# weiwei-ww/ML-VAE

Measured on AMD Instinct MI355X. Metric: spectrogram frames/sec + ELBO; 80-d log-mel B=256 at 1/2/4/8 MI355X, higher is better.
Workload: dtype bf16

## Files before the change

### include/mlvae.h

```cpp
#ifndef MLVAE_H
#define MLVAE_H
#include <stddef.h>
#ifdef __cplusplus
extern "C" {
#endif

const char* mlvae_last_error(void);
int mlvae_abi_version(void);
int mlvae_device_check(char* arch_out, int len);

size_t mlvae_gemm_workspace_size(int M, int N, int K);
int mlvae_gemm(int prec, int trans_a, int trans_b, int M, int N, int K, float alpha,
               const float* A, int lda, const float* B, int ldb, float beta, float* C, int ldc,
               const float* bias1, const float* bias2, int epi, const float* aux, int ldaux,
               int kshift_T, int kshift, float* ws, size_t ws_bytes, void* stream);

size_t mlvae_gemm_ex_workspace_size(int M, int N, int K);
int mlvae_gemm_ex(int trans_a, int trans_b, int M, int N, int K, float alpha, const void* A,
                  int a_bf16, int lda, const void* B, int b_bf16, int ldb, float beta, float* C,
                  int ldc, const float* bias1, const float* bias2, int epi, const float* aux,
                  int ldaux, int kshift_T, int kshift, float* ws, size_t ws_bytes, void* stream);
int mlvae_gemm_ex_drop(int trans_a, int trans_b, int M, int N, int K, float alpha,
                       const void* A, int a_bf16, int lda, const void* B, int b_bf16, int ldb,
                       float beta, float* C, int ldc, const float* bias1, const float* bias2,
                       int epi, const float* aux, int ldaux, int kshift_T, int kshift,
                       unsigned long long drop_seed, unsigned long long drop_offset, float drop_p,
                       float* ws, size_t ws_bytes, void* stream);
size_t mlvae_gemm_bf16_workspace_size(int M, int N, int K, int batch);
int mlvae_gemm_bf16_set_split_target(int workgroups);
int mlvae_gemm_bf16_set_variant(int var);
int mlvae_gemm_bf16(int trans_a, int trans_b, int M, int N, int K, int batch, const void* A,
                    int lda, long long a_bstride, const void* B, int ldb, long long b_bstride,
                    float* C, int ldc, long long c_bstride, float beta, const float* bias1,
                    const float* bias2, int epi, const float* aux, int ldaux, int kshift_T,
                    int kshift, int kshift_bstep, unsigned long long drop_seed,
                    unsigned long long drop_offset, float drop_p, float* ws, size_t ws_bytes,
                    void* stream);
int mlvae_cast_bf16(size_t n, const float* x, void* y, void* stream);
int mlvae_cast_bf16_t(int rows, int cols, const float* x, void* y, void* stream);

int mlvae_lstm_workspace_size(int B, int H, int prec, size_t* xbytes);
int mlvae_lstm_fwd(int prec, int B, int T, int H, const float* w_hh_fwd, const float* w_hh_rev,
                   float* gates, float* cells, float* y, void* xbuf, size_t xbytes, int* err,
                   void* stream);
int mlvae_lstm_bwd(int prec, int B, int T, int H, const float* w_hh_fwd, const float* w_hh_rev,
                   float* gates, const float* cells, const float* dy, void* xbuf, size_t xbytes,
                   int* err, void* stream);
int mlvae_lstm_fwd_ex(int prec, int B, int T, int H, const float* w_hh_fwd, const float* w_hh_rev,
                      float* gates, float* cells, float* y, void* y_bf16, void* xbuf,
                      size_t xbytes, int* err, void* stream);
int mlvae_lstm_bwd_ex(int prec, int B, int T, int H, const float* w_hh_fwd, const float* w_hh_rev,
                      float* gates, const float* cells, const float* dy, void* dg_bf16,
                      void* xbuf, size_t xbytes, int* err, void* stream);
int mlvae_lstm1_fwd(int prec, int B, int T, int H, const float* w_hh, float* gates, float* cells,
                    float* y, void* y_bf16, void* xbuf, size_t xbytes, int* err, void* stream);
int mlvae_lstm1_bwd(int prec, int B, int T, int H, const float* w_hh, float* gates,
                    const float* cells, const float* dy, void* dg_bf16, void* xbuf, size_t xbytes,
                    int* err, void* stream);
int mlvae_lstm_gates_fp16(int B, int H, int prec);
int mlvae_lstm_gates_fp16_t(int B, int T, int H, int prec);
int mlvae_lstm_fwd_ex2(int prec, int B, int T, int H, const float* w_hh_fwd, const float* w_hh_rev,
                       void* gates, int gates_fp16, float* cells, float* y, void* y_bf16,
                       void* y_drop_bf16, unsigned long long drop_seed,
                       unsigned long long drop_offset, float drop_p, void* xbuf, size_t xbytes,
                       int* err, void* stream);
int mlvae_lstm_bwd_ex2(int prec, int B, int T, int H, const float* w_hh_fwd, const float* w_hh_rev,
                       void* gates, int gates_fp16, const float* cells, const float* dy,
                       void* dg_bf16, float* dbias_rows, void* xbuf, size_t xbytes, int* err,
                       void* stream);
int mlvae_lstm_bwd_ex3(int prec, int B, int T, int H, const float* w_hh_fwd, const float* w_hh_rev,
                       void* gates, int gates_fp16, const float* cells, const void* dy, int dy_bf16,
                       void* dg_bf16, float* dbias_rows, void* xbuf, size_t xbytes, int* err,
                       void* stream);
int mlvae_lstm_fwd_fp8(int B, int T, int H, const float* w_hh_fwd, const float* w_hh_rev, void* gates,
                       float* cells, void* y_bf16, void* y_drop_bf16, void* y_drop_fp8, float x8_scale,
                       unsigned long long drop_seed, unsigned long long drop_offset, float drop_p,
                       void* xbuf, size_t xbytes, int* err, void* stream);
int mlvae_lstm_fwd_z(int B, int T, int H, const float* w_hh_fwd, const float* w_hh_rev, const void* z_bf16,
                     int ldz, int Z, const float* w_ih_fwd, const float* w_ih_rev, const float* b_ih_fwd,
                     const float* b_hh_fwd, const float* b_ih_rev, const float* b_hh_rev, void* gates,
                     float* cells, float* y, void* y_bf16, void* y_drop_bf16, void* y_drop_fp8, float x8_scale,
                     unsigned long long drop_seed, unsigned long long drop_offset, float drop_p, void* xbuf,
                     size_t xbytes, int* err, void* stream);
int mlvae_lstm_fwd_z2(int B, int T, int H, const float* w_hh_fwd, const float* w_hh_rev, const void* z_bf16,
                      int ldz, int Z, const float* w_ih_fwd, const float* w_ih_rev, const float* b_ih_fwd,
                      const float* b_hh_fwd, const float* b_ih_rev, const float* b_hh_rev, void* gates,
                      float* cells, float* y, void* y_bf16, int y_bf16_prev, void* y_drop_bf16, void* y_drop_fp8,
                      float x8_scale, unsigned long long drop_seed, unsigned long long drop_offset, float drop_p,
                      void* xbuf, size_t xbytes, int* err, void* stream);
int mlvae_lstm_bwd_fp8(int B, int T, int H, const float* w_hh_fwd, const float* w_hh_rev, void* gates,
                       const float* cells, const float* dy, void* dg_bf16, float* dbias_rows,
                       void* dg_fp8, const float* dg8_scale, unsigned* dg_amax, void* xbuf,
                       size_t xbytes, int* err, void* stream);
int mlvae_lstm_bwd_fp8_ex(int B, int T, int H, const float* w_hh_fwd, const float* w_hh_rev, void* gates,
                          const float* cells, const void* dy, int dy_bf16, void* dg_bf16,
                          float* dbias_rows, void* dg_fp8, const float* dg8_scale, unsigned* dg_amax,
                          void* xbuf, size_t xbytes, int* err, void* stream);
int mlvae_lstm_launch_workgroups(int B, int H, int prec, int fwd);
int mlvae_lstm_set_debug(void* buf);

int mlvae_phn_bce(int B, int T, int C, const float* logits, int ldl, const float* feat_lens,
                  const long long* phn, int L, const float* phn_lens, const float* boundary,
                  float* loss, const float* dloss, float* dlogits, int* err, void* stream);
int mlvae_boundary_fwd(size_t n, const float* za, const float* zb, const float* y, const float* u,
                       unsigned long long seed, unsigned long long offset, float* v, float* bce,
                       float* kld, void* stream);
int mlvae_boundary_bwd(size_t n, const float* za, const float* zb, const float* y, const float* u,
                       unsigned long long seed, unsigned long long offset, const float* dv,
                       const float* dbce, const float* dkld, float* dza, float* dzb, void* stream);

int mlvae_pi_sample(size_t n, const float* logits, const float* u, unsigned long long seed,
                    unsigned long long offset, int train, float* sampled_pi, void* stream);
int mlvae_pi_nll_fwd(size_t n, const float* logits, const int* labels, float* nll, int* err,
                     void* stream);
int mlvae_pi_nll_bwd(size_t n, const float* logits, const int* labels, const float* dnll,
                     float* dlogits, void* stream);

int mlvae_pi_sample_k(size_t n, int K, const float* logits, const float* u, unsigned long long seed,
                      unsigned long long offset, int train, float* sampled_pi, void* stream);
int mlvae_sfl_fwd(size_t n, int K, int F, int Z, const float* logits, const float* sampled_pi,
                  const float* recon, const float* kld, const float* pi_nll, const float* baseline,
                  float w_recon, float w_kld, float w_nll, float* reward, float* rif,
                  float* neg_entropy, float* baseline_loss, void* stream);
int mlvae_sfl_bwd(size_t n, int K, const float* logits, const float* sampled_pi, const float* reward,
// ... 73 lines not shown
                         float* partials, float* bias_ws, size_t bias_ws_bytes, float* db3m,
                         float* db3v, float* db2m, float* db2v, float* db1, int saved_bf16,
                         void* stream);
size_t mlvae_heads_wgrad_workspace_size(int B, int T, int F, int C);
int mlvae_heads_set_nt_mode(int mode);
int mlvae_heads_fused_ex2(int B, int T, int F, int C, int H2, int loss_type, int train,
                          const void* y_bf16, const void* w1_bf16, const void* w1t_bf16, const float* b1,
                          const float* w2m, const float* b2m, const float* w3m, const float* b3m,
                          const float* w2v, const float* b2v, const float* w3v, const float* b3v,
                          const float* x, const float* lens, const int* count, float rec_scale,
                          float* p1, float* p2m, float* p2v, float* mux, float* lvx, float* dmux,
                          float* dlvx, float* dp2m, float* dp2v, float* dp1, float* dy,
                          float* partials, float* bias_ws, size_t bias_ws_bytes, float* db3m,
                          float* db3v, float* db2m, float* db2v, float* db1, int saved_bf16,
                          float* wg_ws, size_t wg_ws_bytes, float* dw3m, float* dw3v, float* dw2m,
                          float* dw2v, void* stream);
int mlvae_heads_fused_ex3(int B, int T, int F, int C, int H2, int loss_type, int train,
                          const void* y_bf16, const void* w1_bf16, const void* w1t_bf16, const float* b1,
                          const float* w2m, const float* b2m, const float* w3m, const float* b3m,
                          const float* w2v, const float* b2v, const float* w3v, const float* b3v,
                          const float* x, const float* lens, const int* count, float rec_scale,
                          float* p1, float* p2m, float* p2v, float* mux, float* lvx, float* dmux,
                          float* dlvx, float* dp2m, float* dp2v, float* dp1, float* dy,
                          float* partials, float* bias_ws, size_t bias_ws_bytes, float* db3m,
                          float* db3v, float* db2m, float* db2v, float* db1, int saved_bf16,
                          float* wg_ws, size_t wg_ws_bytes, float* dw3m, float* dw3v, float* dw2m,
                          float* dw2v, const void* w1_split, void* stream);
int mlvae_bf16_split_rows(const float* src, int rows, int cols, int chunk, void* dst, void* stream);
int mlvae_skinny_proj(int M, int N, int K, const void* A, int lda, const void* B, int ldb,
                      const float* bias1, const float* bias2, float* C, int ldc, void* stream);
int mlvae_skinny_proj_ex(int M, int N, int K, const void* A, int lda, const void* B, int ldb,
                         const float* bias1, const float* bias2, void* C, int ldc, int c_fp16,
                         void* stream);
int mlvae_skinny_nt(int M, int N, int K, const void* A, int lda, const void* Bt, int ldb,
                    float* C, int ldc, void* stream);
size_t mlvae_skinny_tn_workspace_size(int M, int NB, int K);
int mlvae_skinny_tn(int M, int NB, int K, const void* A, int lda, const void* B, int ldb, int nw,
                    float* W, float* bias1, float* bias2, float* ws, size_t ws_bytes, void* stream);
int mlvae_skinny_nt_fp8(int M, int N, int K, const void* A8, int lda, const void* Bt, int ldb, float* C, int ldc,
                        const float* alpha, void* stream);
int mlvae_skinny_tn_fp8(int M, int NB, int K, const void* A8, int lda, const void* B, int ldb, int nw, float* W,
                        float* bias1, float* bias2, const float* alpha, float* ws, size_t ws_bytes, void* stream);
size_t mlvae_skinny_dzw_workspace_size(int M, int K8);
int mlvae_skinny_dzw(int M, int K8, const void* A, int lda, const void* Wt, int ldw, const void* zb, int ldz, int Z,
                     float* dZ, int lddz, float* W, float* bias1, float* bias2, float* ws, size_t ws_bytes,
                     void* stream);
int mlvae_encoder_supported(int F, int E, int Z);
int mlvae_encoder_partials_count(int B, int T);
size_t mlvae_encoder_workspace_size(int B, int T, int F, int E, int Z);
int mlvae_encoder_fwd(int B, int T, int F, int E, int Z, const float* x, const float* w0,
                      const float* b0, const float* w1, const float* b1, const float* wml,
                      const float* bml, const float* eps_in, unsigned long long seed,
                      unsigned long long offset, const float* lens, void* e1_bf16, void* e2_bf16,
                      float* ml, float* z, void* z_bf16, int z_ld, float* eps_out,
                      float* kl_partials, void* stream);
int mlvae_encoder_fwd_ex(int B, int T, int F, int E, int Z, const float* x, const float* w0,
                         const float* b0, const float* w1, const float* b1, const float* wml,
                         const float* bml, const float* eps_in, unsigned long long seed,
                         unsigned long long offset, const float* lens, void* e1_bf16, void* e2_bf16,
                         float* ml, float* z, void* z_bf16, int z_ld, float* eps_out,
                         float* kl_partials, int split, void* stream);
int mlvae_encoder_bwd(int B, int T, int F, int E, int Z, const float* dz, const float* ml,
                      const float* eps, const void* e1_bf16, const void* e2_bf16, const float* x,
                      const float* wml, const float* w1, const float* lens, const int* count,
                      float kl_scale, float* dwml, float* dbml, float* dw1, float* db1, float* dw0,
                      float* db0, float* ws, size_t ws_bytes, void* stream);
int mlvae_dp_scalars(int pack, float* hdr, float* loss3, int* err, void* stream);
int mlvae_elbo_finalize(const float* kl_partials, int nk, const float* rec_partials, int nr,
                        const float* lens, const int* count, int B, int T, int Z, int F,
                        float w_kl, float w_rec, float* out, void* stream);
int mlvae_count_frames(const float* lens, int B, int T, int* out, void* stream);
int mlvae_randn(size_t n, unsigned long long seed, unsigned long long offset, float* out,
                void* stream);
int mlvae_masked_mean(int B, int T, int C, const float* loss, const float* lens, int reduction,
                      float* out, void* stream);

int mlvae_norm_supported(int F);
int mlvae_norm_stats(int B, int T, int F, const float* x, const float* rel_lens, float* utt_stats,
                     float* sums, float eps, void* stream);
int mlvae_norm_update(int F, const float* sums, float* glob_mean, float* glob_std, int mode,
                      float w_old, float w_new, void* stream);
int mlvae_norm_apply(size_t rows, int F, const float* x, const float* glob_mean, const float* glob_std,
                     float* out, void* stream);

int mlvae_sumsq_partials_count(size_t n);
int mlvae_grad_sumsq(const float* grads, size_t n, double* partials, void* stream);
int mlvae_adam_step(float* params, float* exp_avg, float* exp_avg_sq, const float* grads,
                    size_t n, const double* partials, int nparts, const float* loss, int* step,
                    int* nonfinite, float lr, float beta1, float beta2, float eps,
                    float max_norm, float* norm_out, float* hyp_scratch, int advance,
                    void* stream);
int mlvae_adam_step_ex(float* params, float* exp_avg, float* exp_avg_sq, const float* grads,
                       size_t n, const double* partials, int nparts, const float* loss, int* step,
                       int* nonfinite, const int* err, int* err_skips, float lr, float beta1,
                       float beta2, float eps, float max_norm, float* norm_out, float* hyp_scratch,
                       int advance, void* stream);

int mlvae_clip_scale(float* grads, size_t n, const double* partials, int nparts, float max_norm,
                     float* norm_out, void* stream);

int mlvae_lrelu_bwd(size_t n, const float* dy, const float* y, float* dx, void* stream);
int mlvae_masked_mean_bwd(int B, int T, int C, const float* lens, int reduction, const float* g,
                          float* dloss, void* stream);

size_t mlvae_colsum_workspace_size(int N, int C);
int mlvae_colsum(int N, int C, const float* in, int ld, float* out, float* out2, float beta,
                 float* ws, size_t ws_bytes, void* stream);
int mlvae_colsum_ex(int N, int C, const void* in, int in_bf16, int ld, float* out, float* out2,
                    float beta, float* ws, size_t ws_bytes, void* stream);

int mlvae_dropout(size_t n, const float* x, float* y, const float* mask,
                  unsigned long long seed, float p, void* stream);
int mlvae_dropout_ex(size_t n, const float* x, float* y, void* y_bf16, const float* mask,
                     unsigned long long seed, unsigned long long offset, float p, void* stream);

int mlvae_gmm_latent_fwd(int rows, int N, int Z, const float* P, int ldp, const float* eps,
                         const float* expo, unsigned long long seed, unsigned long long offset,
                         float tau, float* z, float* kl, float* w, float* ysoft, void* stream);
int mlvae_gmm_latent_bwd(int rows, int N, int Z, const float* P, int ldp, const float* eps,
                         const float* ysoft, float tau, const float* dz, const float* dkl,
                         const float* dw, float* dP, int lddp, void* stream);
int mlvae_apply_weight_fwd(int rows, int N, int C, const float* x, int ldx, const float* w,
                           float* y, int ldy, void* stream);
int mlvae_apply_weight_bwd(int rows, int N, int C, const float* x, int ldx, const float* w,
                           const float* dy, int lddy, float* dx, int lddx, float* dw,
                           void* stream);

#ifdef __cplusplus
}
#endif
#endif
```

### ml-vae_amd/csrc/gemm_bf16.hip

```cpp
#include "common.h"

namespace {

constexpr int BM = 128, BN = 128, BK = 64, LDK = BK + 8;
constexpr int TILE_ELEMS = BM * LDK;
constexpr size_t LDS_BYTES = (size_t)2 * 2 * TILE_ELEMS * sizeof(short);

struct G2Args {
  int M, N, K;
  const void* A; int lda;
  const void* B; int ldb;
  float* C; int ldc;
  float alpha, beta;
  const float* bias1; const float* bias2;
  int epi;
  const float* aux; int ldaux;
  int kshiftT, kshift;
  int splits, kchunk;
  float* ws;
  unsigned long long dseed;
  unsigned long long doff;
  float dkeep, dscale;
};

// ... 317 lines not shown
  kc = (kc + BK - 1) / BK * BK;
  s = kc > 0 ? (K + kc - 1) / kc : 1;
  *splits = s < 1 ? 1 : s;
  *kchunk = kc > 0 ? kc : BK;
}

extern "C" size_t mlvae_gemm_ex_workspace_size(int M, int N, int K) {
  int s, kc;
  gemm2_plan(M, N, K, &s, &kc);
  return s > 1 ? (size_t)s * M * N * sizeof(float) : 0;
}

extern "C" int mlvae_gemm_ex_drop(int trans_a, int trans_b, int M, int N, int K, float alpha,
                                  const void* A, int a_bf16, int lda, const void* B, int b_bf16,
                                  int ldb, float beta, float* C, int ldc, const float* bias1,
                                  const float* bias2, int epi, const float* aux, int ldaux,
                                  int kshift_T, int kshift, unsigned long long drop_seed,
                                  unsigned long long drop_offset, float drop_p, float* ws,
                                  size_t ws_bytes, void* stream) {
  if (M < 0 || N < 0 || K < 0 || !C || (K > 0 && (!A || !B))) {
    mlvae_set_error("mlvae_gemm_ex: bad shape/ptr");
    return 1;
  }
  if (M == 0 || N == 0) return 0;
  if (epi == EPI_DLRELU && !aux) { mlvae_set_error("mlvae_gemm_ex: DLRELU needs aux"); return 1; }
  if (epi == EPI_DROPOUT && !(drop_p >= 0.f && drop_p < 1.f)) {
    mlvae_set_error("mlvae_gemm_ex: dropout p=%f out of range", drop_p);
    return 1;
  }
  if (epi < EPI_NONE || epi > EPI_DROPOUT) { mlvae_set_error("mlvae_gemm_ex: bad epilogue %d", epi); return 1; }
  if (kshift != 0 && (trans_b || kshift_T <= 0)) {
    mlvae_set_error("mlvae_gemm_ex: kshift needs trans_b = 0, T > 0");
    return 1;
  }
  const size_t ea = a_bf16 ? 2 : 4, eb = b_bf16 ? 2 : 4;
  const int va = (int)(16 / ea), vb = (int)(16 / eb);
  if (((uintptr_t)A % 16) || (lda % va) || ((uintptr_t)B % 16) || (ldb % vb)) {
    mlvae_set_error("mlvae_gemm_ex: operands need 16-byte aligned rows (lda %% %d, ldb %% %d)", va, vb);
    return 1;
  }
  G2Args g;
  g.M = M; g.N = N; g.K = K; g.A = A; g.lda = lda; g.B = B; g.ldb = ldb; g.C = C; g.ldc = ldc;
  g.alpha = alpha; g.beta = beta; g.bias1 = bias1; g.bias2 = bias2; g.epi = epi; g.aux = aux;
  g.ldaux = ldaux; g.kshiftT = kshift_T; g.kshift = kshift; g.ws = ws;
  g.dseed = drop_seed; g.doff = drop_offset; g.dkeep = 1.f - drop_p; g.dscale = 1.f / (1.f - drop_p);
  int s, kc;
  gemm2_plan(M, N, K, &s, &kc);
  if (s > 1 && (!ws || ws_bytes < (size_t)s * M * N * sizeof(float))) {
    s = 1;
    kc = ((K + BK - 1) / BK) * BK;
  }
  if (K == 0) { s = 1; kc = BK; }
  g.splits = s; g.kchunk = kc;
  hipStream_t st = (hipStream_t)stream;
  dim3 grid(((N + BN - 1) / BN) * ((M + BM - 1) / BM), 1, s);
  int rc;
  if (!trans_a && trans_b) rc = launch2<false, true>(g, grid, a_bf16, b_bf16, st);
  else if (!trans_a && !trans_b) rc = launch2<false, false>(g, grid, a_bf16, b_bf16, st);
  else if (trans_a && !trans_b) rc = launch2<true, false>(g, grid, a_bf16, b_bf16, st);
  else rc = launch2<true, true>(g, grid, a_bf16, b_bf16, st);
  if (rc) return rc;
  MLVAE_CHECK_LAUNCH();
  if (s > 1) {
    size_t MN = (size_t)M * N;
    int blocks = (int)((MN + 63) / 64);
    if (blocks > 4096) blocks = 4096;
    splitk_reduce2<<<blocks, 256, 0, st>>>(g);
    MLVAE_CHECK_LAUNCH();
  }
  return 0;
}

extern "C" int mlvae_gemm_ex(int trans_a, int trans_b, int M, int N, int K, float alpha,
                             const void* A, int a_bf16, int lda, const void* B, int b_bf16,
                             int ldb, float beta, float* C, int ldc, const float* bias1,
                             const float* bias2, int epi, const float* aux, int ldaux,
                             int kshift_T, int kshift, float* ws, size_t ws_bytes, void* stream) {
  if (epi == EPI_DROPOUT) { mlvae_set_error("mlvae_gemm_ex: dropout epilogue needs mlvae_gemm_ex_drop"); return 1; }
  return mlvae_gemm_ex_drop(trans_a, trans_b, M, N, K, alpha, A, a_bf16, lda, B, b_bf16, ldb, beta,
                            C, ldc, bias1, bias2, epi, aux, ldaux, kshift_T, kshift, 0ull, 0ull, 0.f, ws,
                            ws_bytes, stream);
}

__global__ __launch_bounds__(256) void cast_bf16_kernel(size_t n, const float* __restrict__ x,
                                                        unsigned short* __restrict__ y) {
  const size_t n4 = n / 4;
  for (size_t i = (size_t)blockIdx.x * 256 + threadIdx.x; i < n4; i += (size_t)gridDim.x * 256) {
    const f32x4 v = reinterpret_cast<const f32x4*>(x)[i];
    u32x2 o = {(unsigned)bf_bits(v[0]) | ((unsigned)bf_bits(v[1]) << 16),
               (unsigned)bf_bits(v[2]) | ((unsigned)bf_bits(v[3]) << 16)};
    reinterpret_cast<u32x2*>(y)[i] = o;
  }
  for (size_t i = n4 * 4 + (size_t)blockIdx.x * 256 + threadIdx.x; i < n; i += (size_t)gridDim.x * 256)
    y[i] = bf_bits(x[i]);
}

extern "C" int mlvae_cast_bf16(size_t n, const float* x, void* y, void* stream) {
  if (n == 0) return 0;
  if (!x || !y || ((uintptr_t)x % 16) || ((uintptr_t)y % 8)) {
    mlvae_set_error("mlvae_cast_bf16: needs 16-byte aligned x, 8-byte aligned y");
    return 1;
  }
  size_t blocks = (n / 4 + 255) / 256;
  if (blocks > 4096) blocks = 4096;
  if (blocks < 1) blocks = 1;
  cast_bf16_kernel<<<(unsigned)blocks, 256, 0, (hipStream_t)stream>>>(n, x,
                                                                       static_cast<unsigned short*>(y));
  MLVAE_CHECK_LAUNCH();
  return 0;
}

__global__ __launch_bounds__(256) void cast_bf16_t_kernel(int rows, int cols, const float* __restrict__ x,
                                                          unsigned short* __restrict__ y) {
  __shared__ float t[32][33];
  const int r0 = blockIdx.y * 32, c0 = blockIdx.x * 32;
  const int tx = threadIdx.x & 31, ty = threadIdx.x >> 5;
#pragma unroll
  for (int k = 0; k < 4; ++k) {
    const int r = r0 + ty + 8 * k, c = c0 + tx;
    t[ty + 8 * k][tx] = (r < rows && c < cols) ? x[(size_t)r * cols + c] : 0.f;
  }
  __syncthreads();
#pragma unroll
  for (int k = 0; k < 4; ++k) {
    const int c = c0 + ty + 8 * k, r = r0 + tx;
    if (c < cols && r < rows) y[(size_t)c * rows + r] = bf_bits(t[tx][ty + 8 * k]);
  }
}

extern "C" int mlvae_cast_bf16_t(int rows, int cols, const float* x, void* y, void* stream) {
  if (rows <= 0 || cols <= 0) return 0;
  if (!x || !y) { mlvae_set_error("mlvae_cast_bf16_t: null pointer"); return 1; }
  dim3 grid((cols + 31) / 32, (rows + 31) / 32);
  cast_bf16_t_kernel<<<grid, 256, 0, (hipStream_t)stream>>>(rows, cols, x, static_cast<unsigned short*>(y));
  MLVAE_CHECK_LAUNCH();
  return 0;
}
```

### ml-vae_amd/csrc/lstm.hip

```cpp
#include "common.h"
#include <stdlib.h>
#include <type_traits>

#include "lstm_common.h"

namespace {


template <int PREC, int HJ, int NL>
__global__ __launch_bounds__(320) void lstm_fwd_kernel(LstmArgs a) {
  typedef typename Elt<PREC>::T ET;
  constexpr int ROWS = 4 * HJ, MT = ROWS / 16;
  constexpr int KS = 4;
  constexpr int NRED = PREC == PREC_F32 ? 1 : 2;
  constexpr int KSTEP = PREC == PREC_F32 ? 16 : 32;
  constexpr int EPL = PREC == PREC_F32 ? 4 : 8;
  constexpr int GE = Elt<PREC>::GE;
  constexpr bool IOW = PREC == PREC_BF16 && HJ == 16;
  constexpr int GXS = 16 * 4 + 4, OUS = 16 * 8 + 4;
  extern __shared__ __attribute__((aligned(16))) char smem[];
  f32x4* red0 = reinterpret_cast<f32x4*>(smem);
  float* gxr = reinterpret_cast<float*>(smem + NRED * 4 * MT * 64 * 16);
  float* outr = gxr + 2 * 16 * GXS;
  __shared__ int abort_flag;
// ... 831 lines not shown
  return p;
}

int device_cus() {
  int dev = 0, cus = 256;
  if (hipGetDevice(&dev) != hipSuccess ||
      hipDeviceGetAttribute(&cus, hipDeviceAttributeMultiprocessorCount, dev) != hipSuccess)
    cus = 256;
  return cus;
}

int max_batch_per_launch(int H, bool fwd, int prec) {
  const int cus = device_cus();
  int hj = pick_hj(H, fwd, prec);
  int nj = hj ? H / hj : 1;
  int nb = cus / (2 * nj);
  return nb * BG;
}

template <int PREC, int HJ, int NL>
int launch_nl(bool fwd, const LstmArgs& a, const Plan& p, hipStream_t s) {
  dim3 grid(a.xcd_local ? 8 * a.NJ : a.ndir * a.NB * a.NJ);
  auto k = fwd ? lstm_fwd_kernel<PREC, HJ, NL> : lstm_bwd_kernel<PREC, HJ, NL>;
  const size_t lds = p.lds;
  if (hipFuncSetAttribute((const void*)k, hipFuncAttributeMaxDynamicSharedMemorySize, (int)lds) != hipSuccess) {
    mlvae_set_error("lstm: cannot reserve %zu B LDS", lds);
    return 2;
  }
  const int nthr = (fwd && PREC == PREC_BF16 && HJ == 16) ? 320 : 256;
  k<<<grid, nthr, lds, s>>>(a);
  MLVAE_CHECK_LAUNCH();
  return 0;
}

template <int PREC, int HJ>
int launch(bool fwd, const LstmArgs& a, const Plan& p, hipStream_t s) {
  constexpr int KSTEP = PREC == PREC_F32 ? 16 : 32;
  constexpr int KSF = 4;
  const int nl = fwd ? a.Kp / (KSF * KSTEP) : a.K4p / (4 * KSTEP);
  switch (nl) {
    case 1: return launch_nl<PREC, HJ, 1>(fwd, a, p, s);
    case 2: return launch_nl<PREC, HJ, 2>(fwd, a, p, s);
    case 4: return launch_nl<PREC, HJ, 4>(fwd, a, p, s);
    case 8: return launch_nl<PREC, HJ, 8>(fwd, a, p, s);
    case 16: return launch_nl<PREC, HJ, 16>(fwd, a, p, s);
    case 32: return launch_nl<PREC, HJ, 32>(fwd, a, p, s);
    default:
      mlvae_set_error("lstm: H=%d needs %d operand loads per wave (max 32)", a.H, nl);
      return 1;
  }
}

template <int NTW>
int launch_rs(const LstmArgs& a, const Plan& p, hipStream_t s) {
  dim3 grid(a.xcd_local ? 8 * a.NJ : a.ndir * a.NB * a.NJ);
  auto k = lstm_bwd_rs_kernel<NTW>;
  if (hipFuncSetAttribute((const void*)k, hipFuncAttributeMaxDynamicSharedMemorySize, (int)p.lds) != hipSuccess) {
    mlvae_set_error("lstm: cannot reserve %zu B LDS", p.lds);
    return 2;
  }
  k<<<grid, 256, p.lds, s>>>(a);
  MLVAE_CHECK_LAUNCH();
  return 0;
}

bool use_wide(int B, int H, int prec) {
  if (prec != PREC_BF16 || H <= 0 || H % 4) return false;
  const int bf = max_batch_per_launch(H, true, prec), bb = max_batch_per_launch(H, false, prec);
  (void)bf; (void)bb;
  if (g_dbg_mode & (1 << 20)) return false;
  return lstm_wide_workgroups(B, H, true) > 0 && lstm_wide_workgroups(B, H, false) > 0;
}

struct WideExtra {
  unsigned short* ydb = nullptr;
  float* dbias = nullptr;
  unsigned long long seed = 0, off = 0;
  float p = 0.f;
  WideFp8 f8;
  const unsigned short* dyb = nullptr;
  WideZ wz;
};

int run(bool fwd, int prec, int B, int T, int H, const float* W0, const float* W1, float* G,
        float* Cs, float* Y, void* xbuf, size_t xbytes, int* err, hipStream_t st,
        unsigned short* yb = nullptr, unsigned short* dgb = nullptr, int gates_fp16 = 0,
        const WideExtra& ex = WideExtra(), int ndir = 2) {
  if (B <= 0 || T <= 0) return 0;
  if (H <= 0 || H % 4 != 0) { mlvae_set_error("lstm: H=%d must be a positive multiple of 4", H); return 1; }
  if (prec != PREC_F32 && prec != PREC_BF16) { mlvae_set_error("lstm: bad prec %d", prec); return 1; }
  const bool wide = gates_fp16 != 0;
  if (ndir != 1 && ndir != 2) { mlvae_set_error("lstm: %d directions", ndir); return 1; }
  if (wide && ndir != 2) { mlvae_set_error("lstm: fp16 gates are bidirectional only"); return 1; }
  if (wide && !use_wide(B, H, prec)) {
    mlvae_set_error("lstm: B=%d H=%d prec=%d: fp16 gates only where mlvae_lstm_gates_fp16() = 1", B, H, prec);
    return 1;
  }
  if (wide) {
    if (!fwd && !dgb && !ex.f8.dg8) {
      mlvae_set_error("lstm: the wide-batch backward writes dG to dg_bf16 or (fp8 mode) dg_fp8 (both NULL)");
      return 1;
    }
    if (ex.ydb && !(ex.p >= 0.f && ex.p < 1.f)) { mlvae_set_error("lstm: dropout p=%g", ex.p); return 1; }
    return lstm_wide_run(fwd, B, T, H, W0, W1, G, Cs, Y, xbuf, xbytes, err, st, yb, dgb, ex.dbias, ex.ydb,
                         ex.seed, ex.off, ex.p, g_dbg, g_dbg_mode, ex.f8, ex.dyb, ex.wz);
  }
  if (ex.dyb) { mlvae_set_error("lstm: bf16 dY only on the wide-batch path (fp16 gates)"); return 1; }
  if (ex.ydb || ex.dbias || !Y) {
    mlvae_set_error("lstm: fused dropout / bias-gradient outputs, Y = NULL only on the wide-batch path");
    return 1;
  }
  if (!fwd && use_stepwise_bwd(H, prec)) return run_bwd_stepwise(B, T, H, ndir, W0, W1, G, Cs, Y, xbuf, xbytes, dgb, st);
  const int bmax = max_batch_per_launch(H, fwd, prec);
  if (bmax < BG) { mlvae_set_error("lstm: H=%d too large for one resident launch", H); return 1; }
  Plan full = make_plan(bmax < B ? bmax : B, H, prec, fwd);
  const size_t need_x = fwd ? full.xbytes_fwd : full.xbytes_bwd;
  if (!xbuf || xbytes < need_x || !err) {
    mlvae_set_error("lstm: exchange workspace too small (need %zu B)", need_x);
    return 1;
  }
  for (int b0 = 0; b0 < B; b0 += bmax) {
    const int bc = B - b0 < bmax ? B - b0 : bmax;
    Plan p = make_plan(bc, H, prec, fwd);
    LstmArgs a{};
    a.B = bc; a.T = T; a.H = H; a.NB = p.NB; a.NJ = p.NJ; a.HJ = p.HJ; a.Kp = p.Kp; a.K4p = p.K4p;
    a.W0 = W0; a.W1 = W1;
    const size_t gld = (size_t)4 * H * ndir, yld = (size_t)H * ndir;
    a.ndir = ndir;
    a.G = G + (size_t)b0 * T * gld;
    a.Cs = Cs + (size_t)b0 * T * yld;
    a.Y = Y + (size_t)b0 * T * yld;
    a.xbuf = xbuf; a.err = err; a.dbg = g_dbg; a.dbg_mode = g_dbg_mode;
    a.Yb = yb ? yb + (size_t)b0 * T * yld : nullptr;
    a.dGb = dgb ? dgb + (size_t)b0 * T * gld : nullptr;
    a.xcd_local = p.xcd && device_cus() == 256 && (fwd ? !(g_dbg_mode & 4) : (g_dbg_mode & 2));
    a.xtab = reinterpret_cast<unsigned*>(
        static_cast<char*>(xbuf) + (p.rs ? (size_t)2 * p.NB * NSLOT * p.NJ * p.NJ * 256 * sizeof(short)
                                         : (size_t)2 * p.NB * NSLOT * BG * p.Kp * (prec == PREC_F32 ? 4 : 2)));
    if (hipMemsetAsync(xbuf, 0, fwd ? p.xbytes_fwd : p.xbytes_bwd, st) != hipSuccess) {
      mlvae_set_error("lstm: memset failed");
      return 2;
    }
    int rc;
    if (p.rs) {
      rc = p.NJ == 8 ? launch_rs<2>(a, p, st) : p.NJ == 16 ? launch_rs<4>(a, p, st)
         : p.NJ == 32 ? launch_rs<8>(a, p, st) : launch_rs<16>(a, p, st);
    } else if (prec == PREC_F32) {
      rc = p.HJ == 16 ? launch<PREC_F32, 16>(fwd, a, p, st)
         : p.HJ == 8 ? launch<PREC_F32, 8>(fwd, a, p, st) : launch<PREC_F32, 4>(fwd, a, p, st);
    } else {
      rc = p.HJ == 32 ? launch<PREC_BF16, 32>(fwd, a, p, st)
         : p.HJ == 16 ? launch<PREC_BF16, 16>(fwd, a, p, st)
         : p.HJ == 8 ? launch<PREC_BF16, 8>(fwd, a, p, st) : launch<PREC_BF16, 4>(fwd, a, p, st);
    }
    if (rc) return rc;
  }
  return 0;
}

}

extern "C" int mlvae_lstm_workspace_size(int B, int H, int prec, size_t* xbytes) {
  if (H <= 0 || H % 4 != 0) { mlvae_set_error("lstm: H=%d must be a positive multiple of 4", H); return 1; }
  const int bf = max_batch_per_launch(H, true, prec), bb = max_batch_per_launch(H, false, prec);
  Plan pf = make_plan(bf < B ? bf : B, H, prec, true);
  Plan pb = make_plan(bb < B ? bb : B, H, prec, false);
  *xbytes = pf.xbytes_fwd > pb.xbytes_bwd ? pf.xbytes_fwd : pb.xbytes_bwd;
  if (use_stepwise_bwd(H, prec) && (size_t)2 * B * H * sizeof(float) > *xbytes)
    *xbytes = (size_t)2 * B * H * sizeof(float);
  if (prec == PREC_BF16) {
    const size_t wf = lstm_wide_xbytes(B, H, true), wb = lstm_wide_xbytes(B, H, false);
    if (wf > *xbytes) *xbytes = wf;
    if (wb > *xbytes) *xbytes = wb;
  }
  return 0;
}

extern "C" int mlvae_lstm_launch_workgroups(int B, int H, int prec, int fwd) {
  if (B <= 0 || H <= 0 || H % 4) return 0;
  const int bmax = max_batch_per_launch(H, fwd != 0, prec);
  if (use_wide(B, H, prec)) return lstm_wide_workgroups(B, H, fwd != 0);
  Plan p = make_plan(bmax < B ? bmax : B, H, prec, fwd != 0);
  return 2 * p.NB * p.NJ;
}

extern "C" int mlvae_lstm_gates_fp16(int B, int H, int prec) { return use_wide(B, H, prec) ? 1 : 0; }
extern "C" int mlvae_lstm_gates_fp16_t(int B, int T, int H, int prec) {
  return use_wide(B, H, prec) && lstm_wide_t_ok(T, H) ? 1 : 0;
}

extern "C" int mlvae_lstm_fwd_ex2(int prec, int B, int T, int H, const float* w_hh_fwd,
                                  const float* w_hh_rev, void* gates, int gates_fp16, float* cells,
                                  float* y, void* y_bf16, void* y_drop_bf16,
                                  unsigned long long drop_seed, unsigned long long drop_offset,
                                  float drop_p, void* xbuf, size_t xbytes, int* err, void* stream) {
  WideExtra ex;
  ex.ydb = static_cast<unsigned short*>(y_drop_bf16);
  ex.seed = drop_seed; ex.off = drop_offset; ex.p = drop_p;
  return run(true, prec, B, T, H, w_hh_fwd, w_hh_rev, static_cast<float*>(gates), cells, y, xbuf,
             xbytes, err, (hipStream_t)stream, static_cast<unsigned short*>(y_bf16), nullptr,
             gates_fp16, ex);
}

extern "C" int mlvae_lstm_fwd_fp8(int B, int T, int H, const float* w_hh_fwd, const float* w_hh_rev,
                                  void* gates, float* cells, void* y_bf16, void* y_drop_bf16,
                                  void* y_drop_fp8, float x8_scale, unsigned long long drop_seed,
                                  unsigned long long drop_offset, float drop_p, void* xbuf,
                                  size_t xbytes, int* err, void* stream) {
  if (!use_wide(B, H, PREC_BF16) || !y_drop_fp8 || !(x8_scale > 0.f)) {
    mlvae_set_error("lstm_fwd_fp8: wide-batch shapes with an e4m3 dropout output and a positive scale only");
    return 1;
  }
  WideExtra ex;
  ex.ydb = static_cast<unsigned short*>(y_drop_bf16);
  ex.seed = drop_seed; ex.off = drop_offset; ex.p = drop_p;
  ex.f8.y8 = static_cast<unsigned char*>(y_drop_fp8);
  ex.f8.x8scale = x8_scale;
  return run(true, PREC_BF16, B, T, H, w_hh_fwd, w_hh_rev, static_cast<float*>(gates), cells, nullptr,
             xbuf, xbytes, err, (hipStream_t)stream, static_cast<unsigned short*>(y_bf16), nullptr, 1, ex);
}
extern "C" int mlvae_lstm_fwd_z2(int B, int T, int H, const float* w_hh_fwd, const float* w_hh_rev,
                                 const void* z_bf16, int ldz, int Z, const float* w_ih_fwd,
                                 const float* w_ih_rev, const float* b_ih_fwd, const float* b_hh_fwd,
                                 const float* b_ih_rev, const float* b_hh_rev, void* gates, float* cells,
                                 float* y, void* y_bf16, int y_bf16_prev, void* y_drop_bf16, void* y_drop_fp8,
                                 float x8_scale, unsigned long long drop_seed, unsigned long long drop_offset,
                                 float drop_p, void* xbuf, size_t xbytes, int* err, void* stream) {
  if (Z != 32 || !z_bf16 || !use_wide(B, H, PREC_BF16) || (y_drop_fp8 && !(x8_scale > 0.f))) {
    mlvae_set_error("lstm_fwd_z: Z = 32 on wide-batch shapes; an e4m3 dropout output needs a scale");
    return 1;
  }
  WideExtra ex;
  ex.ydb = static_cast<unsigned short*>(y_drop_bf16);
  ex.seed = drop_seed; ex.off = drop_offset; ex.p = drop_p;
  ex.f8.y8 = static_cast<unsigned char*>(y_drop_fp8);
  ex.f8.x8scale = x8_scale;
  ex.wz.zb = static_cast<const unsigned short*>(z_bf16);
  ex.wz.ldz = ldz;
  ex.wz.w0 = w_ih_fwd; ex.wz.w1 = w_ih_rev;
  ex.wz.b[0] = b_ih_fwd; ex.wz.b[1] = b_hh_fwd; ex.wz.b[2] = b_ih_rev; ex.wz.b[3] = b_hh_rev;
  ex.wz.yb_prev = y_bf16 && y_bf16_prev ? 1 : 0;
  return run(true, PREC_BF16, B, T, H, w_hh_fwd, w_hh_rev, static_cast<float*>(gates), cells, y, xbuf, xbytes,
             err, (hipStream_t)stream, static_cast<unsigned short*>(y_bf16), nullptr, 1, ex);
}
// ... 126 lines not shown
```

### ml-vae_amd/csrc/lstm_common.h

```cpp
#pragma once
#include "common.h"
#include <type_traits>

#ifndef MLVAE_DIAG
#define MLVAE_DIAG 0
#endif
#define DMODE(a) (MLVAE_DIAG ? (a).dbg_mode : 0)
#define DPTR(a) (MLVAE_DIAG ? (a).dbg : (unsigned long long*)nullptr)

namespace {

constexpr int BG = 16;
constexpr int NSLOT = 4;
constexpr unsigned SPIN_LIMIT = 1u << 20;
constexpr int MIN_LDS = 82 * 1024;

struct LstmArgs {
  int B, T, H;
  int NB, NJ, HJ;
  int ndir;
  int Kp;
  int K4p;
  const float* W0;
  const float* W1;
  float* G;
  float* Cs;
  float* Y;
  void* xbuf;
  int* err;
  unsigned long long* dbg;
  int dbg_mode;
  int xcd_local;
  unsigned* xtab;
  unsigned short* Yb;
  unsigned short* dGb;
  float* dbias;
  unsigned short* Ydb;
  unsigned long long dseed, doff;
  float dkeep, dscale;
  unsigned char* Y8;
  float x8scale;
  unsigned char* dG8;
  const float* g8scale;
  unsigned* g8amax;
  const unsigned short* dYb;
  const unsigned short* Zb;
  int ldz;
  const float* Wz0;
  const float* Wz1;
  const float* bz[4];
  int yb_prev;
};

__device__ __forceinline__ unsigned xcc_id() {
  return __builtin_amdgcn_s_getreg((3 << 11) | (0 << 6) | 20) & 0xf;
}

__device__ bool group_on_one_xcd(unsigned* tab, int members, int me, int* scratch) {
  const int tid = threadIdx.x;
  const unsigned mine = xcc_id() + 1;
  if (tid == 0) { *scratch = 0; st_flag(tab + me, mine); }
  __syncthreads();
  if (tid < members) {
    unsigned v = 0, spins = 0;
    while ((v = ld_flag(tab + tid)) == 0 && ++spins < (1u << 16)) __builtin_amdgcn_s_sleep(2);
    if (v != mine) atomicOr(scratch, 1);
  }
  __syncthreads();
  return *scratch == 0;
}

#define STAMP(ph)                                                              \
  do {                                                                         \
    if (DPTR(a) && blockIdx.x == 0 && threadIdx.x == 0)                          \
      a.dbg[(size_t)s * 16 + (ph)] = __builtin_amdgcn_s_memtime();             \
  } while (0)
#define WSTAMP(slot)                                                           \
  do {                                                                         \
    if (DPTR(a) && blockIdx.x == 0 && (threadIdx.x & 63) == 0)                   \
      a.dbg[(size_t)s * 16 + (slot) + (threadIdx.x >> 6)] = __builtin_amdgcn_s_memtime(); \
  } while (0)

#define IOSTAMP(k)                                                             \
  do {                                                                         \
    if (DBG && DPTR(a) && (DMODE(a) & 16) && blockIdx.x == 0 && threadIdx.x == 256 && \
        (unsigned)(s - STW0) < (unsigned)STWN)                                 \
      stamp_lds[(s - STW0) * 16 + 8 + (k)] = __builtin_amdgcn_s_memtime();     \
  } while (0)
constexpr int STW0 = 64, STWN = 32;
#define LSTAMP_DECL                                                            \
  __shared__ unsigned long long stamp_lds[DBG ? STWN * 16 : 1];                \
  if (DBG && DPTR(a) && blockIdx.x == 0 && threadIdx.x == 0)                     \
    for (int i_ = 0; i_ < STWN * 16; ++i_) stamp_lds[i_] = 0
#define LSTAMP(ph)                                                             \
  do {                                                                         \
    if (DBG && DPTR(a) && blockIdx.x == 0 && threadIdx.x == 0 &&                        \
        (unsigned)(s - STW0) < (unsigned)STWN)                                 \
      stamp_lds[(s - STW0) * 16 + (ph)] = __builtin_amdgcn_s_memtime();        \
  } while (0)
#define LWSTAMP()                                                              \
  do {                                                                         \
    if (DBG && DPTR(a) && !(DMODE(a) & 16) && blockIdx.x == 0 && (threadIdx.x & 63) == 0 && \
        (unsigned)(s - STW0) < (unsigned)STWN)                                 \
      stamp_lds[(s - STW0) * 16 + 8 + (threadIdx.x >> 6)] = __builtin_amdgcn_s_memtime(); \
  } while (0)
#define LSTAMP_FLUSH()                                                         \
  do {                                                                         \
    if (DBG) __syncthreads();                                                  \
    if (DBG && DPTR(a) && blockIdx.x == 0 && threadIdx.x == 0)                   \
      for (int i_ = 0; i_ < STWN * 16; ++i_)                                   \
        a.dbg[(size_t)STW0 * 16 + i_] = stamp_lds[i_];                         \
  } while (0)

#define RTS_DECL                                                               \
  __shared__ unsigned long long rts_lds[DBG ? STWN * 16 : 1];                  \
  const bool rts_on = DBG && DPTR(a) && (DMODE(a) & 8);                        \
  if (rts_on)                                                                  \
    for (int i_ = threadIdx.x; i_ < STWN * 16; i_ += blockDim.x) rts_lds[i_] = 0
#define RTS(slot)                                                              \
  do {                                                                         \
    if (rts_on && (threadIdx.x & 63) == 0 && (unsigned)(s - STW0) < (unsigned)STWN) \
      rts_lds[(s - STW0) * 16 + (slot)] = __builtin_amdgcn_s_memrealtime();    \
  } while (0)
#define RTS_FLUSH()                                                            \
  do {                                                                         \
    if (DBG) __syncthreads();                                                  \
    if (rts_on)                                                                \
      for (int i_ = threadIdx.x; i_ < STWN * 16; i_ += blockDim.x)             \
        a.dbg[(size_t)a.T * 16 + (size_t)blockIdx.x * STWN * 16 + i_] = rts_lds[i_]; \
  } while (0)

__device__ __forceinline__ void stagger_start(int gid, int mode) {
  if (!(mode & (1 << 29)) || !((gid ^ (gid >> 3)) & 1)) return;
  for (int i = 0; i < ((mode >> 5) & 7); ++i) __builtin_amdgcn_s_sleep(16);
}

template <int PREC> struct Elt;
template <> struct Elt<PREC_F32> { typedef float T; static constexpr int GE = 2; };
template <> struct Elt<PREC_BF16> { typedef short T; static constexpr int GE = 4; };

__device__ __forceinline__ unsigned step_tag(int s) { return (unsigned)(((s >> 2) + 1) & 1); }
__device__ __forceinline__ unsigned step_tag_lg(int s, int lg) { return (unsigned)(((s >> lg) + 1) & 1); }

__device__ __forceinline__ unsigned long long pack_bf16(float v0, float v1, float v2, float v3,
                                                        unsigned tag) {
  const unsigned e0 = ((unsigned)(unsigned short)f2bf(v0) & ~1u) | tag;
  const unsigned lo = e0 | ((unsigned)(unsigned short)f2bf(v1) << 16);
  const unsigned hi = (unsigned)(unsigned short)f2bf(v2) | ((unsigned)(unsigned short)f2bf(v3) << 16);
  return ((unsigned long long)hi << 32) | lo;
}
__device__ __forceinline__ unsigned long long pack_f32(float v0, float v1, unsigned tag) {
  const unsigned e0 = (__float_as_uint(v0) & ~1u) | tag;
  return ((unsigned long long)__float_as_uint(v1) << 32) | e0;
}
__device__ __forceinline__ void st_granule(__amdgpu_buffer_rsrc_t r, unsigned byte_off,
                                           unsigned long long v) {
  u32x2 w = {(unsigned)v, (unsigned)(v >> 32)};
  __builtin_amdgcn_raw_buffer_store_b64(w, r, byte_off, 0, 16 );
}
__device__ __forceinline__ bool tags_ok(u32x4 v, unsigned tag, bool g0, bool g1) {
  return (!g0 || (v[0] & 1u) == tag) && (!g1 || (v[2] & 1u) == tag);
}

}

struct WideFp8 {
  unsigned char* y8 = nullptr;
  float x8scale = 0.f;
  unsigned char* dg8 = nullptr;
  const float* g8scale = nullptr;
  unsigned* g8amax = nullptr;
};
struct WideZ {
  const unsigned short* zb = nullptr;
  int ldz = 0;
  const float* w0 = nullptr;
  const float* w1 = nullptr;
  const float* b[4] = {nullptr, nullptr, nullptr, nullptr};
  int yb_prev = 0;
};
int lstm_wide_run(bool fwd, int B, int T, int H, const float* W0, const float* W1, float* G,
                  float* Cs, float* Y, void* xbuf, size_t xbytes, int* err, hipStream_t st,
                  unsigned short* yb, unsigned short* dgb, float* dbias, unsigned short* ydb,
                  unsigned long long dseed, unsigned long long doff, float dp,
                  unsigned long long* dbg, int dbg_mode, const WideFp8& f8 = WideFp8(),
                  const unsigned short* dyb = nullptr, const WideZ& wz = WideZ());
size_t lstm_wide_xbytes(int B, int H, bool fwd);
bool lstm_wide_t_ok(int T, int H);
int lstm_wide_workgroups(int B, int H, bool fwd);
```

### ml-vae_amd/csrc/lstm_wide.hip

```cpp
#include "lstm_common.h"
#include <stdlib.h>
#include <type_traits>

namespace {

constexpr int WW = 8;
constexpr int FWD_KLF = 4;
template <int TPW> constexpr int bptt_groups() { return 2; }
#ifndef NT_AUX
#define NT_AUX 2
#endif

__device__ __forceinline__ void publish(__amdgpu_buffer_rsrc_t r, unsigned byte_off,
                                        unsigned long long v, bool plain) {
  if (plain) {
    u32x2 w = {(unsigned)v, (unsigned)(v >> 32)};
    __builtin_amdgcn_raw_buffer_store_b64(w, r, byte_off, 0, 0);
  } else {
    st_granule(r, byte_off, v);
  }
}

__device__ __forceinline__ int swz(int utt, int slot) { return slot ^ (utt & 15); }

template <int TPW, int NKC, int OCC, bool DBG = false, bool AS = false, bool ZP = false, int NT = 1,
          bool W12 = false>
__global__ __launch_bounds__(W12 ? 768 : 512, W12 ? 1 : OCC) void lstm_fwd_wide_kernel(LstmArgs a) {
  static_assert(NT == 1 || (NT == 2 && AS && TPW == 1), "two N-tiles: the asymmetric TPW-1 split");
  static_assert(!W12 || (AS && TPW == 1), "12 waves: the asymmetric TPW-1 split");
  constexpr int NWV = W12 ? 12 : 8;
  constexpr int NPOLL = W12 ? 8 : 4;
  constexpr int IO0 = NWV - 4;
  constexpr int BGW = BG * NT;
  constexpr int HJ = WW * TPW * 4;
  constexpr int H = NKC * 32;
  constexpr int PL = NKC / NPOLL;
  constexpr int ROWB = H * 2;
  constexpr int HIMG = BGW * ROWB;
  constexpr int GXU = 4 * HJ + 8;
  constexpr int OUB = 4 * HJ * 2 + 2 * HJ * 4 + 16;
  constexpr int NC8 = BGW * HJ / 8;
  constexpr int KLF = ((TPW == 1 && !AS) || W12) ? 0 : FWD_KLF;
  constexpr int KR = NKC - KLF;
  constexpr int HB = 4;
  constexpr int NQ = 16 * 4 * HJ / 4;
  constexpr int QPT = NQ / 256;
  static_assert(NQ % 256 == 0, "io split");
  extern __shared__ __attribute__((aligned(16))) char smem[];
  LSTAMP_DECL;
  RTS_DECL;
  char* himg = smem;
  unsigned short* gxr = reinterpret_cast<unsigned short*>(smem + 2 * HIMG);
  char* outr = reinterpret_cast<char*>(gxr + 2 * BGW * GXU);
  bf16x8* wlds = reinterpret_cast<bf16x8*>(outr + 2 * BGW * OUB);
  unsigned* dbl = reinterpret_cast<unsigned*>(wlds + 8 * TPW * KLF * 64);
  __shared__ int abort_flag;

  const int ngroups = 2 * a.NB, gstride = (ngroups + 7) & ~7;
  const int gid = blockIdx.x % gstride, js = blockIdx.x / gstride;
  if (gid >= ngroups) return;
  const int dir = gid / a.NB, grp = gid % a.NB;
  const int T = a.T, j0 = js * HJ;
  const int tid = threadIdx.x, lane = tid & 63;
  const int nlg = (DMODE(a) & (1 << 24)) ? 2 : 1, nmask = (1 << nlg) - 1;
  const int wave = __builtin_amdgcn_readfirstlane(tid >> 6);
  const float* W = dir ? a.W1 : a.W0;
  const int bi = lane & 15, q = lane >> 4;
  bool valid[NT];
#pragma unroll
  for (int n = 0; n < NT; ++n) valid[n] = grp * BGW + 16 * n + bi < a.B;

  static_assert(!AS || TPW == 1, "asymmetric split: TPW 1 only");
  constexpr int TPP = W12 ? 1 : AS ? 2 : TPW;
  constexpr int TPI = AS ? 0 : TPW;
  static_assert(NPOLL * TPP + 4 * TPI == WW * TPW, "every tile owned once");
  auto load_w = [&](auto* wreg, int m0, int mt) {
    for (int t = 0; t < mt; ++t) {
      const int m = m0 + t;
      const float* wrow = W + (size_t)((bi & 3) * H + j0 + 4 * m + (bi >> 2)) * H;
#pragma unroll
      for (int kc = 0; kc < NKC; ++kc) {
        const f32x4 w0 = *reinterpret_cast<const f32x4*>(wrow + kc * 32 + 8 * q);
        const f32x4 w1 = *reinterpret_cast<const f32x4*>(wrow + kc * 32 + 8 * q + 4);
        bf16x8 v;
#pragma unroll
        for (int e = 0; e < 4; ++e) { v[e] = f2bf(w0[e]); v[4 + e] = f2bf(w1[e]); }
        if (kc < KR) wreg[t][kc < KR ? kc : 0] = v;
        else wlds[(m * KLF + (kc - KR)) * 64 + lane] = v;
      }
    }
  };
  __shared__ int placement;
  const bool same_xcd = group_on_one_xcd(a.xtab + gid * a.NJ, a.NJ, js, &placement) &&
                        !(DMODE(a) & 32768);
  if (tid == 0) abort_flag = 0;

  const size_t xslot = (size_t)BGW * H;
  short* xb = reinterpret_cast<short*>(a.xbuf) + (size_t)(dir * a.NB + grp) * NSLOT * xslot;
  auto xr = make_rsrc(xb, (unsigned)(NSLOT * xslot * sizeof(short)));

  const int iot = tid - 64 * IO0;
  const bool io = wave >= IO0;
  const int iow = wave - IO0;
  typedef __attribute__((address_space(3))) void* lds_ptr_t;
  unsigned short* G16 = reinterpret_cast<unsigned short*>(a.G);
  const auto rgx = make_rsrc(G16 + (size_t)grp * BGW * T * 8 * H, 0xffffffffu);
  const bool tmaj = (DMODE(a) & 1024) != 0;
  auto rowof = [&](int b_, int t_) -> size_t { return tmaj ? (size_t)t_ * a.B + b_ : (size_t)b_ * T + t_; };
  const auto rgx_abs = make_rsrc(G16, (unsigned)min((size_t)a.B * T * 8 * H * 2, (size_t)0xffffffffu));
  unsigned short* zr = gxr;
  const auto rz = make_rsrc(a.Zb, (unsigned)min((size_t)a.B * T * a.ldz * 2, (size_t)0x7fffffff));
  auto io_load = [&](int s_) {
    if (s_ >= T || (s_ > 0 && (DMODE(a) & 8192))) return;
    const int t_ = dir ? T - 1 - s_ : s_;
    if constexpr (ZP) {
      if (iow < NT) {
        const int u = iow * 16 + (lane >> 2), b = grp * BGW + u;
        const unsigned off = b < a.B ? (unsigned)((((size_t)b * T + t_) * a.ldz + 8 * (lane & 3)) * 2) : 0x80000000u;
        __builtin_amdgcn_raw_ptr_buffer_load_lds(rz, (lds_ptr_t)(zr + ((s_ & 1) * BGW + iow * 16) * 32), 16,
                                                 off, 0, 0, NT_AUX);
      }
      return;
    }
    constexpr int UPW = BGW / 4;
#pragma unroll
    for (int i = 0; i < UPW; ++i) {
      const int u = iow * UPW + i, b = grp * BGW + u;
      if (b >= a.B) continue;
      const int g = lane / (HJ / 8), uu = (lane % (HJ / 8)) * 8;
      const unsigned off = tmaj ? (unsigned)((((size_t)t_ * a.B + b) * 8 * H + dir * 4 * H + g * H + j0 + uu) * 2)
                                : (unsigned)((((size_t)u * T + t_) * 8 * H + dir * 4 * H + g * H + j0 + uu) * 2);
      const auto rs = tmaj ? rgx_abs : rgx;
      unsigned short* dst = gxr + (s_ & 1) * BGW * GXU + u * GXU;
      if (lane < HJ / 2) __builtin_amdgcn_raw_ptr_buffer_load_lds(rs, (lds_ptr_t)dst, 16, off, 0, 0, NT_AUX);
    }
  };
  auto drop_bits = [&](int s_, int c8) -> unsigned {
    const int u = c8 / (HJ / 8), uu = (c8 % (HJ / 8)) * 8;
    const int t_ = dir ? T - 1 - s_ : s_;
    const size_t o = ((size_t)(grp * BGW + u) * T + t_) * 2 * H + dir * H + j0 + uu;
// ... 303 lines not shown
              for (int t = 0; t < MT; ++t) {
                const int u0 = j0 + 4 * (m0 + t);
                publish(xr, ((unsigned)((s & nmask) * xslot) + ((u0 >> 3) * BGW + 16 * n + bi) * 8 + (u0 & 7)) * sizeof(short),
                        gr[t][n], same_xcd);
              }
          }
        } else if (q == 0) {
          const int u0 = j0 + 4 * TPW * wave;
          const unsigned cell = (unsigned)((s & nmask) * xslot) + ((u0 >> 3) * 16 + bi) * 8 + (u0 & 7);
          if constexpr (TPW == 2) {
            const u32x4 v = {(unsigned)gr[0][0], (unsigned)(gr[0][0] >> 32), (unsigned)gr[1][0], (unsigned)(gr[1][0] >> 32)};
            if (same_xcd) __builtin_amdgcn_raw_buffer_store_b128(v, xr, cell * sizeof(short), 0, 0);
            else st_sc1_b128(xr, cell * sizeof(short), v);
          } else {
            publish(xr, cell * sizeof(short), gr[0][0], same_xcd);
          }
        }
      }
      LSTAMP(4);
      RTS(wave);
      IOSTAMP(5);
      if (!IO && (DMODE(a) & (1 << 23))) {
        asm volatile("s_waitcnt vmcnt(0)" ::: "memory");
        LSTAMP(5);
      }
      if (IO && !PURE_IO && late_dma_s) io_load(s + 1);
      if (IO && !PURE_IO && s > 0) io_store(s - 1);
      IOSTAMP(6);
#pragma unroll
      for (int n = 0; n < NT; ++n) {
        char* ob = outr + ((s & 1) * BGW + 16 * n + bi) * OUB;
        unsigned short* og = reinterpret_cast<unsigned short*>(ob);
        float* of = reinterpret_cast<float*>(ob + 8 * HJ);
#pragma unroll
        for (int t = 0; t < MT; ++t) {
          const int u = 4 * (m0 + t) + q;
          og[u] = f2h(gates[t][n][0]); og[HJ + u] = f2h(gates[t][n][1]);
          og[2 * HJ + u] = f2h(gates[t][n][2]); og[3 * HJ + u] = f2h(gates[t][n][3]);
          of[u] = c[t][n]; of[HJ + u] = hvals[t][n];
        }
      }
      LSTAMP(6);
      if (!IO && want_drop && tid < NC8 && (!late_bits || s + 1 == T)) dbl[(s & 1) * NC8 + tid] = drop_bits(s, tid);
      LSTAMP(7);
    }
    __syncthreads();
    if (IO) io_store(T - 1);
  };
  if (io) run(std::true_type{});
  else run(std::false_type{});
  LSTAMP_FLUSH();
  RTS_FLUSH();
}

template <int TPW, int NKC, int OCC, bool F8 = false, bool DYB = false, bool DBG = false>
__global__ __launch_bounds__(512, OCC) void lstm_bwd_wide_kernel(LstmArgs a) {
  constexpr int HJ = 32 * TPW;
  constexpr int H = NKC * 32;
  constexpr int NJ = H / HJ;
  constexpr int NTW = NKC / 4;
  constexpr int KC = 4 * HJ / 32;
  constexpr int KLB = TPW == 1 ? 0 : KC / 4;
  constexpr int KR = KC - KLB;
  constexpr int BKB = TPW == 1 ? 4 : 1;
  constexpr int ROWB = 4 * HJ * 2;
  constexpr int AIMG = 16 * ROWB;
  constexpr int NPL = NJ / 8;
  constexpr int CPG = 2 * HJ / 64;
  static_assert(NPL >= 1 && CPG >= 1 && NPL * CPG == 2, "two 16-byte partial loads per lane");
  extern __shared__ __attribute__((aligned(16))) char smem[];
  LSTAMP_DECL;
  RTS_DECL;
  char* aimg = smem;
  bf16x8* wlds = reinterpret_cast<bf16x8*>(smem + 2 * AIMG);
  constexpr int CG_B = 4 * HJ * 2 + 16;
  constexpr int CF_B = HJ * 4 + 32;
  constexpr int CD_B = DYB ? HJ * 2 + 32 : CF_B;
  static_assert(((CG_B + CF_B + CD_B) / 4) % 8 == 4 || ((CG_B + CF_B + CD_B) / 4) % 64 == 20,
                "conflict-free staged rows");
  constexpr int CUTT = CG_B + CF_B + CD_B;
  char* cst = smem + 2 * AIMG + (size_t)8 * NTW * KLB * 64 * 16;
  __shared__ int abort_flag;

  const int ngroups = 2 * a.NB, gstride = (ngroups + 7) & ~7;
  const int gid = blockIdx.x % gstride, js = blockIdx.x / gstride;
  if (gid >= ngroups) return;
  const int dir = gid / a.NB, grp = gid % a.NB;
  const int T = a.T, j0 = js * HJ;
  const int tid = threadIdx.x, lane = tid & 63;
  const int nlg = (DMODE(a) & (1 << 24)) ? 2 : 1, nmask = (1 << nlg) - 1;
  const int wave = __builtin_amdgcn_readfirstlane(tid >> 6);
  const float* W = dir ? a.W1 : a.W0;
  const int bi = lane & 15, q = lane >> 4;

  bf16x8 wreg[NTW][KR];
  static_assert(KLB > 0 || KR == KC, "");
#pragma unroll
  for (int nt = 0; nt < NTW; ++nt) {
    const int n = (wave * NTW + nt) * 16 + bi;
#pragma unroll
    for (int kc = 0; kc < KC; ++kc) {
      bf16x8 v;
#pragma unroll
      for (int e = 0; e < 8; ++e) {
        const int k = kc * 32 + 8 * q + e;
        v[e] = f2bf(W[(size_t)((k / HJ) * H + j0 + (k % HJ)) * H + n]);
      }
      if (kc < KR) wreg[nt][kc < KR ? kc : 0] = v;
      else wlds[((wave * NTW + nt) * KLB + (kc - KR)) * 64 + lane] = v;
    }
  }
  __shared__ int placement;
  const bool same_xcd = group_on_one_xcd(a.xtab + gid * NJ, NJ, js, &placement) &&
                        !(DMODE(a) & 32768);
  if (tid == 0) abort_flag = 0;
  if (DBG && DPTR(a) && (DMODE(a) & 8) && tid == 0) a.dbg[blockIdx.x] = same_xcd ? 1 : 2;
  __syncthreads();

  const size_t xslot = (size_t)NJ * NJ * HJ * 16;
  short* xb = reinterpret_cast<short*>(a.xbuf) + (size_t)(dir * a.NB + grp) * NSLOT * xslot;
  auto xr = make_rsrc(xb, (unsigned)(NSLOT * xslot * sizeof(short)));

  auto rs_perm = [](int g) { return g ^ ((g & 4) ? 3 : 0); };
  const int arow = rs_perm(js / NPL);
  const int gq = tid >> 3, pg = lane & 7;
  int uc[CPG], cu[CPG];
  bool bv[CPG];
#pragma unroll
  for (int ci = 0; ci < CPG; ++ci) {
    const int cb = gq * CPG + ci;
    uc[ci] = cb >> 1;
    cu[ci] = (cb & 1) * 8 + rs_perm(pg);
    bv[ci] = grp * BG + cu[ci] < a.B;
  }
  constexpr int NGC = 16 * 4 * HJ / 8, NFC = 16 * HJ / 4, NDC = DYB ? 16 * HJ / 8 : NFC;
  constexpr int NCH = NGC + NFC + NDC;
  constexpr int CPT = (NCH + 511) / 512;
  static_assert(DYB || NCH % 512 == 0, "whole chunks per thread");
  static_assert(NGC % 64 == 0 && NFC % 64 == 0 && NDC % 64 == 0, "chunk kinds change at whole waves");
  const size_t gbase = (size_t)grp * BG * T;
  const auto rG = make_rsrc(reinterpret_cast<const unsigned short*>(a.G) + gbase * 8 * H, 0xffffffffu);
  const auto rC = make_rsrc(a.Cs + gbase * 2 * H, 0xffffffffu);
  const auto rY = DYB ? make_rsrc(a.dYb + gbase * 2 * H, 0xffffffffu) : make_rsrc(a.Y + gbase * 2 * H, 0xffffffffu);
  u32x4 creg[CPT];
  auto chunk_lds = [&](int c) -> int {
    if (c < NGC) {
      const int u = c / (4 * HJ / 8), k = c % (4 * HJ / 8);
      return u * CUTT + k * 16;
    }
    const int f = c - NGC;
    if (f < NFC) {
      const int u = f / (HJ / 4), k = f % (HJ / 4);
      return u * CUTT + CG_B + k * 16;
    }
    const int r = f - NFC, upr = DYB ? HJ / 8 : HJ / 4;
    return (r / upr) * CUTT + CG_B + CF_B + (r % upr) * 16;
  };
  const int ulast = a.B - 1 - grp * BG;
  auto load_cell = [&](int s_) {
    const int sc = s_ < T ? s_ : T - 1;
    const int t_ = dir ? sc : T - 1 - sc;
    const int tp_ = dir ? t_ + 1 : t_ - 1;
    const int tpc = tp_ < 0 ? 0 : (tp_ >= T ? T - 1 : tp_);
#pragma unroll
    for (int i = 0; i < CPT; ++i) {
      const int cw0 = wave * 64 + 512 * i;
// ... 340 lines not shown
    if (2 * nb2 * (H / 32) <= cus) {
      p.nt = 2; p.tpw = 1; p.HJ = 32; p.NJ = H / 32; p.NB = nb2; p.ok = true;
    }
  }
  if (!p.ok)
  for (int tpw = 1; tpw <= 2; ++tpw) {
    if (fwd && tpw * p.nkc * 4 > 128) break;
    p.NB = (B + BG - 1) / BG;
    const int hj = 32 * tpw, nj = H / hj;
    if (!fwd && (nj < 8 || nj % 8)) continue;
    if (2 * p.NB * nj <= cus) {
      p.tpw = tpw; p.HJ = hj; p.NJ = nj; p.ok = true;
      break;
    }
  }
  if (!p.ok) return p;
  if (fwd && p.tpw == 1) p.w12 = !(mode & 2048);
  p.lds = wide_lds(H, p.HJ, fwd, p.nt);
  if (fwd) p.xbytes = (size_t)2 * p.NB * NSLOT * BG * p.nt * H * 2;
  else p.xbytes = (size_t)2 * p.NB * NSLOT * p.NJ * p.NJ * p.HJ * 16 * 2;
  if (p.lds < (size_t)MIN_LDS) p.lds = MIN_LDS;
  p.xtab_off = p.xbytes;
  p.xbytes += (size_t)2 * p.NB * p.NJ * sizeof(unsigned);
  return p;
}

template <int TPW, int NKC, int OCC>
int launch_wide(bool fwd, const LstmArgs& a, const WidePlan& p, hipStream_t s) {
  const bool dbg = a.dbg != nullptr;
  constexpr bool AS1 = TPW == 1;
  const bool zp = a.Zb != nullptr;
  auto k = (fwd && p.w12)
               ? (p.nt == 2 ? (dbg ? lstm_fwd_wide_kernel<1, NKC, OCC, true, true, false, 2, true>
                                   : zp ? lstm_fwd_wide_kernel<1, NKC, OCC, false, true, true, 2, true>
                                        : lstm_fwd_wide_kernel<1, NKC, OCC, false, true, false, 2, true>)
                            : (dbg ? lstm_fwd_wide_kernel<1, NKC, OCC, true, true, false, 1, true>
                                   : zp ? lstm_fwd_wide_kernel<1, NKC, OCC, false, true, true, 1, true>
                                        : lstm_fwd_wide_kernel<1, NKC, OCC, false, true, false, 1, true>))
         : (fwd && p.nt == 2)
               ? (dbg ? lstm_fwd_wide_kernel<1, NKC, OCC, true, true, false, 2>
                      : zp ? lstm_fwd_wide_kernel<1, NKC, OCC, false, true, true, 2>
                           : lstm_fwd_wide_kernel<1, NKC, OCC, false, true, false, 2>)
         : fwd ? (dbg ? lstm_fwd_wide_kernel<TPW, NKC, OCC, true, AS1>
                      : zp ? lstm_fwd_wide_kernel<TPW, NKC, OCC, false, AS1, true>
                           : lstm_fwd_wide_kernel<TPW, NKC, OCC, false, AS1>)
               : (a.g8amax ? (a.dYb ? lstm_bwd_wide_kernel<TPW, NKC, OCC, true, true>
                                    : lstm_bwd_wide_kernel<TPW, NKC, OCC, true, false>)
                           : (a.dYb ? (dbg ? lstm_bwd_wide_kernel<TPW, NKC, OCC, false, true, true>
                                           : lstm_bwd_wide_kernel<TPW, NKC, OCC, false, true>)
                                    : (dbg ? lstm_bwd_wide_kernel<TPW, NKC, OCC, false, false, true>
                                           : lstm_bwd_wide_kernel<TPW, NKC, OCC, false>)));
  if (hipFuncSetAttribute((const void*)k, hipFuncAttributeMaxDynamicSharedMemorySize, (int)p.lds) != hipSuccess) {
    mlvae_set_error("lstm_wide: cannot reserve %zu B LDS", p.lds);
    return 2;
  }
  k<<<dim3(((2 * p.NB + 7) & ~7) * p.NJ), (fwd && p.w12) ? 768 : 512, p.lds, s>>>(a);
  MLVAE_CHECK_LAUNCH();
  return 0;
}

}

bool lstm_wide_t_ok(int T, int H) {
  return (size_t)2 * BG * T * 8 * H * 2 <= 0xffffffffull && (size_t)2 * BG * T * 2 * H * 4 <= 0xffffffffull;
}

int lstm_wide_workgroups(int B, int H, bool fwd) {
  WidePlan p = wide_plan(B, H, fwd);
  if (!p.ok) return 0;
  return 2 * p.NB * p.NJ;
}

size_t lstm_wide_xbytes(int B, int H, bool fwd) {
  WidePlan p = wide_plan(B, H, fwd), q = wide_plan(B, H, fwd, 512);
  if (!p.ok) return 0;
  return p.xbytes > q.xbytes ? p.xbytes : q.xbytes;
}

int lstm_wide_run(bool fwd, int B, int T, int H, const float* W0, const float* W1, float* G,
                  float* Cs, float* Y, void* xbuf, size_t xbytes, int* err, hipStream_t st,
                  unsigned short* yb, unsigned short* dgb, float* dbias, unsigned short* ydb,
                  unsigned long long dseed, unsigned long long doff, float dp,
                  unsigned long long* dbg, int dbg_mode, const WideFp8& f8, const unsigned short* dyb,
                  const WideZ& wz) {
  WidePlan p = wide_plan(B, H, fwd, dbg_mode);
  if (!p.ok) return -1;
  if (!lstm_wide_t_ok(T, H)) {
    mlvae_set_error("lstm_wide: T=%d too long for the wide kernels' 32-bit batch-group addressing at H=%d "
                    "(mlvae_lstm_gates_fp16_t(B, T, H, prec) = 0: pass fp32 gates)", T, H);
    return 1;
  }
  if (!xbuf || xbytes < p.xbytes || !err) {
    mlvae_set_error("lstm_wide: exchange workspace too small (need %zu B)", p.xbytes);
    return 1;
  }
  LstmArgs a{};
  a.ndir = 2;
  a.B = B; a.T = T; a.H = H; a.NB = p.NB; a.NJ = p.NJ; a.HJ = p.HJ; a.Kp = H; a.K4p = 4 * H;
  a.W0 = W0; a.W1 = W1; a.G = G; a.Cs = Cs; a.Y = Y; a.xbuf = xbuf; a.err = err;
  a.dbg = dbg; a.dbg_mode = dbg_mode; a.xcd_local = 0; a.Yb = yb; a.dGb = dgb;
  a.dbias = dbias; a.Ydb = ydb; a.dseed = dseed; a.doff = doff; a.dkeep = 1.f - dp;
  a.Y8 = f8.y8; a.x8scale = f8.x8scale; a.dG8 = f8.dg8; a.g8scale = f8.g8scale; a.g8amax = f8.g8amax;
  a.dYb = fwd ? nullptr : dyb;
  if (wz.zb && dbg) a.dbg = dbg = nullptr;
  if (wz.zb) {
    if (!fwd || !wz.w0 || !wz.w1 || !wz.b[0] || !wz.b[1] || !wz.b[2] || !wz.b[3] ||
        wz.ldz < 32 || wz.ldz % 8 || ((uintptr_t)wz.zb % 16)) {
      mlvae_set_error("lstm_wide: the fused z projection needs the forward, "
                      "both W_ih and all four biases, a 16-byte aligned z with ldz >= 32, ldz %% 8 == 0");
      return 1;
    }
    a.Zb = wz.zb; a.ldz = wz.ldz; a.Wz0 = wz.w0; a.Wz1 = wz.w1; a.yb_prev = wz.yb_prev;
    for (int i = 0; i < 4; ++i) a.bz[i] = wz.b[i];
  }
  if (a.Y8 && (!fwd || !(a.x8scale > 0.f) || !(dp >= 0.f && dp < 1.f))) {
    mlvae_set_error("lstm_wide: the e4m3 dropout(h) output needs the forward, a positive scale and 0 <= p < 1");
    return 1;
  }
  if (a.dG8 && (!a.g8scale || !a.g8amax)) {
    mlvae_set_error("lstm_wide: the fp8 dG copy needs its scale and amax words");
    return 1;
  }
  a.dscale = dp < 1.f ? 1.f / (1.f - dp) : 0.f;
  a.xtab = reinterpret_cast<unsigned*>(static_cast<char*>(xbuf) + p.xtab_off);
  if (hipMemsetAsync(xbuf, 0, p.xbytes, st) != hipSuccess) {
    mlvae_set_error("lstm_wide: memset failed");
    return 2;
  }
  return p.tpw == 2 ? launch_wide<2, 16, 2>(fwd, a, p, st) : launch_wide<1, 16, 2>(fwd, a, p, st);
}
```

### ml-vae_amd/csrc/norm.hip

```cpp
#include "common.h"

namespace {

constexpr int NT = 256;

__device__ __forceinline__ int norm_frames(float rel, int T) {
  const float n = rintf(rel * (float)T);
  return n <= 0.f ? 0 : (n >= (float)T ? T : (int)n);
}

__global__ __launch_bounds__(NT) void norm_stats_kernel(int T, int F, const float* __restrict__ x,
                                                        const float* __restrict__ lens,
                                                        float* __restrict__ stats, float eps) {
  extern __shared__ f32x4 red[];
  const int b = blockIdx.x, FQ = F / 4, RL = NT / FQ;
  const int q = threadIdx.x % FQ, rl = threadIdx.x / FQ;
  const int n = norm_frames(lens[b], T);
  const f32x4* xb = reinterpret_cast<const f32x4*>(x + (size_t)b * T * F);
  const bool act = rl < RL;
  f32x4 s = {0.f, 0.f, 0.f, 0.f};
  if (act) {
    int r = rl;
    for (; r + 3 * RL < n; r += 4 * RL) {
      const f32x4 a0 = xb[(size_t)r * FQ + q], a1 = xb[(size_t)(r + RL) * FQ + q];
      const f32x4 a2 = xb[(size_t)(r + 2 * RL) * FQ + q], a3 = xb[(size_t)(r + 3 * RL) * FQ + q];
      s += a0; s += a1; s += a2; s += a3;
    }
    for (; r < n; r += RL) s += xb[(size_t)r * FQ + q];
    red[rl * FQ + q] = s;
  }
  __syncthreads();
  f32x4 mean = {0.f, 0.f, 0.f, 0.f};
  if (n > 0) {
    f32x4 t = red[q];
    for (int i = 1; i < RL; ++i) t += red[i * FQ + q];
    mean = t / (float)n;
  }
  __syncthreads();
  f32x4 v = {0.f, 0.f, 0.f, 0.f};
  if (act) {
    int r = rl;
    for (; r + 3 * RL < n; r += 4 * RL) {
      const f32x4 d0 = xb[(size_t)r * FQ + q] - mean, d1 = xb[(size_t)(r + RL) * FQ + q] - mean;
      const f32x4 d2 = xb[(size_t)(r + 2 * RL) * FQ + q] - mean, d3 = xb[(size_t)(r + 3 * RL) * FQ + q] - mean;
      v += d0 * d0; v += d1 * d1; v += d2 * d2; v += d3 * d3;
    }
    for (; r < n; r += RL) {
      const f32x4 d = xb[(size_t)r * FQ + q] - mean;
      v += d * d;
    }
    red[rl * FQ + q] = v;
  }
  __syncthreads();
  if (rl == 0) {
    f32x4 t = red[q];
    for (int i = 1; i < RL; ++i) t += red[i * FQ + q];
    f32x4 sd;
#pragma unroll
    for (int e = 0; e < 4; ++e) {
      const float var = t[e] / (float)(n - 1);
      const float st = sqrtf(var);
      sd[e] = n > 0 ? (st < eps ? eps : st) : 0.f;
    }
    float* o = stats + (size_t)b * 2 * F;
    *reinterpret_cast<f32x4*>(o + 4 * q) = mean;
    *reinterpret_cast<f32x4*>(o + F + 4 * q) = sd;
  }
}

__global__ __launch_bounds__(NT) void norm_sums_kernel(int B, int T, int F, const float* __restrict__ lens,
                                                       const float* __restrict__ stats,
                                                       float* __restrict__ sums) {
  __shared__ float red[4][64];
  const int c = threadIdx.x & 63, lb = threadIdx.x >> 6, f = blockIdx.x * 64 + c;
  float s = 0.f;
  if (f <= 2 * F) {
    int b = lb;
    for (; b + 12 < B; b += 16) {
      float v[4], m[4];
#pragma unroll
      for (int i = 0; i < 4; ++i) {
        m[i] = norm_frames(lens[b + 4 * i], T) > 0 ? 1.f : 0.f;
        v[i] = f < 2 * F ? stats[(size_t)(b + 4 * i) * 2 * F + f] : 1.f;
      }
#pragma unroll
      for (int i = 0; i < 4; ++i) s += m[i] * v[i];
    }
    for (; b < B; b += 4)
      if (norm_frames(lens[b], T) > 0) s += f < 2 * F ? stats[(size_t)b * 2 * F + f] : 1.f;
  }
  red[lb][c] = s;
  __syncthreads();
  if (lb == 0 && f <= 2 * F) sums[f] = ((red[0][c] + red[1][c]) + red[2][c]) + red[3][c];
}

__global__ __launch_bounds__(NT) void norm_update_kernel(int F, const float* __restrict__ sums,
                                                         float* __restrict__ gmean, float* __restrict__ gstd,
                                                         int mode, float w1, float w) {
  const float cnt = sums[2 * F] > 0.f ? sums[2 * F] : 1.f;
  for (int f = threadIdx.x; f < F; f += NT) {
    const float cm = sums[f] / cnt, cs = sums[F + f] / cnt;
    if (mode == 1) { gmean[f] = cm; gstd[f] = cs; }
    else if (mode == 2) { gmean[f] = w1 * gmean[f] + w * cm; gstd[f] = w1 * gstd[f] + w * cs; }
  }
}

__global__ __launch_bounds__(NT) void norm_apply_kernel(size_t nq, int FQ, const f32x4* __restrict__ x,
                                                        const float* __restrict__ gmean,
                                                        const float* __restrict__ gstd,
                                                        f32x4* __restrict__ out) {
  for (size_t i = (size_t)blockIdx.x * NT + threadIdx.x; i < nq; i += (size_t)gridDim.x * NT) {
    const int q = (int)(i % FQ);
    const f32x4 m = *reinterpret_cast<const f32x4*>(gmean + 4 * q);
    const f32x4 s = *reinterpret_cast<const f32x4*>(gstd + 4 * q);
    out[i] = (x[i] - m) / s;
  }
}

}

extern "C" int mlvae_norm_supported(int F) { return F > 0 && F % 4 == 0 && F / 4 <= NT; }

extern "C" int mlvae_norm_stats(int B, int T, int F, const float* x, const float* rel_lens,
                                float* utt_stats, float* sums, float eps, void* stream) {
  if (!mlvae_norm_supported(F) || B <= 0 || T <= 0) {
    mlvae_set_error("norm_stats: B=%d T=%d F=%d unsupported (F %% 4 == 0, F <= 1024)", B, T, F);
    return 1;
  }
  if (((uintptr_t)x | (uintptr_t)utt_stats) & 15) {
    mlvae_set_error("norm_stats: x / utt_stats must be 16-byte aligned");
    return 1;
  }
  hipStream_t s = (hipStream_t)stream;
  const int FQ = F / 4, RL = NT / FQ;
  norm_stats_kernel<<<B, NT, (size_t)RL * FQ * sizeof(f32x4), s>>>(T, F, x, rel_lens, utt_stats, eps);
  norm_sums_kernel<<<(2 * F + 1 + 63) / 64, NT, 0, s>>>(B, T, F, rel_lens, utt_stats, sums);
  MLVAE_CHECK_LAUNCH();
  return 0;
}

extern "C" int mlvae_norm_update(int F, const float* sums, float* glob_mean, float* glob_std, int mode,
                                 float w_old, float w_new, void* stream) {
  if (mode < 0 || mode > 2) { mlvae_set_error("norm_update: mode %d", mode); return 1; }
  if (mode == 0) return 0;
  norm_update_kernel<<<1, NT, 0, (hipStream_t)stream>>>(F, sums, glob_mean, glob_std, mode, w_old, w_new);
  MLVAE_CHECK_LAUNCH();
  return 0;
}

extern "C" int mlvae_norm_apply(size_t rows, int F, const float* x, const float* glob_mean,
                                const float* glob_std, float* out, void* stream) {
  if (!mlvae_norm_supported(F)) { mlvae_set_error("norm_apply: F=%d unsupported", F); return 1; }
  if (((uintptr_t)x | (uintptr_t)out | (uintptr_t)glob_mean | (uintptr_t)glob_std) & 15) {
    mlvae_set_error("norm_apply: buffers must be 16-byte aligned");
    return 1;
  }
  const size_t nq = rows * (size_t)(F / 4);
  size_t g = (nq + NT - 1) / NT;
  if (g > 4096) g = 4096;
  if (g < 1) g = 1;
  norm_apply_kernel<<<(unsigned)g, NT, 0, (hipStream_t)stream>>>(
      nq, F / 4, reinterpret_cast<const f32x4*>(x), glob_mean, glob_std, reinterpret_cast<f32x4*>(out));
  MLVAE_CHECK_LAUNCH();
  return 0;
}
```

### ml-vae_amd/csrc/optim.hip

```cpp
#include "common.h"

namespace {

__global__ __launch_bounds__(256) void sumsq_kernel(const float* __restrict__ g, size_t n,
                                                    double* __restrict__ partials) {
  __shared__ double sm[4];
  double acc = 0.0;
  const size_t n4 = n / 4;
  const f32x4* g4 = reinterpret_cast<const f32x4*>(g);
  for (size_t i = (size_t)blockIdx.x * 256 + threadIdx.x; i < n4; i += (size_t)gridDim.x * 256) {
    f32x4 v = g4[i];
    acc += (double)v[0] * v[0] + (double)v[1] * v[1] + (double)v[2] * v[2] + (double)v[3] * v[3];
  }
  if (blockIdx.x == 0)
    for (size_t i = n4 * 4 + threadIdx.x; i < n; i += 256) acc += (double)g[i] * g[i];
  acc = wave_sum_d(acc);
  if ((threadIdx.x & 63) == 0) sm[threadIdx.x >> 6] = acc;
  __syncthreads();
  if (threadIdx.x == 0) partials[blockIdx.x] = sm[0] + sm[1] + sm[2] + sm[3];
}

struct AdamArgs {
  float* p; float* m; float* v; const float* g;
  size_t n;
  const float* hyp;
  float b1, b2, eps;
};

__global__ __launch_bounds__(256) void adam_prologue(const double* partials, int nparts,
                                                     const float* loss, const int* step, float lr,
                                                     float b1, float b2, float max_norm,
                                                     float* hyp, float* norm_out, const int* err) {
  __shared__ double red[256];
  double a = 0.0;
  for (int i = threadIdx.x; i < nparts; i += 256) a += partials[i];
  red[threadIdx.x] = a;
  __syncthreads();
  for (int o = 128; o > 0; o >>= 1) {
    if ((int)threadIdx.x < o) red[threadIdx.x] += red[threadIdx.x + o];
    __syncthreads();
  }
  if (threadIdx.x != 0) return;
  const float total = (float)sqrt(red[0]);
  float coef = max_norm / (total + 1e-6f);
  coef = coef < 1.f ? coef : 1.f;
  if (!(total == total)) coef = total;
  const int t = *step + 1;
  const double bc1 = 1.0 - pow((double)b1, (double)t);
  const double bc2 = 1.0 - pow((double)b2, (double)t);
  hyp[0] = coef;
  hyp[1] = ((loss && !isfinite(*loss)) || (err && *err != 0)) ? 1.f : 0.f;
  hyp[2] = (float)((double)lr / bc1);
  hyp[3] = (float)sqrt(bc2);
  if (norm_out) *norm_out = total;
}

__global__ __launch_bounds__(256) void adam_kernel(AdamArgs a) {
  if (a.hyp[1] != 0.f) return;
  const float coef = a.hyp[0], step_size = a.hyp[2], bc2s = a.hyp[3];
  const float w1 = 1.f - a.b1, w2 = 1.f - a.b2;
  const size_t n4 = a.n / 4;
  f32x4* p4 = reinterpret_cast<f32x4*>(a.p);
  f32x4* m4 = reinterpret_cast<f32x4*>(a.m);
  f32x4* v4 = reinterpret_cast<f32x4*>(a.v);
  const f32x4* g4 = reinterpret_cast<const f32x4*>(a.g);
  for (size_t i = (size_t)blockIdx.x * 256 + threadIdx.x; i < n4; i += (size_t)gridDim.x * 256) {
    f32x4 g = g4[i] * coef, m = m4[i], v = v4[i], p = p4[i];
#pragma unroll
    for (int e = 0; e < 4; ++e) {
      m[e] = m[e] + w1 * (g[e] - m[e]);
      v[e] = v[e] * a.b2 + w2 * g[e] * g[e];
      const float denom = sqrtf(v[e]) / bc2s + a.eps;
      p[e] = p[e] + (-step_size) * (m[e] / denom);
    }
    p4[i] = p; m4[i] = m; v4[i] = v;
  }
  if (blockIdx.x == 0) {
    for (size_t i = n4 * 4 + threadIdx.x; i < a.n; i += 256) {
      const float g = a.g[i] * coef;
      float m = a.m[i], v = a.v[i];
      m = m + w1 * (g - m);
      v = v * a.b2 + w2 * g * g;
      a.p[i] = a.p[i] + (-step_size) * (m / (sqrtf(v) / bc2s + a.eps));
      a.m[i] = m; a.v[i] = v;
    }
  }
}

__global__ void step_counter_kernel(const float* loss, int* step, int* nonfinite, const int* err,
                                    int* err_skips) {
  if (threadIdx.x || blockIdx.x) return;
  if (err && *err != 0) { if (err_skips) *err_skips += 1; }
  else if (loss && !isfinite(*loss)) { if (nonfinite) *nonfinite += 1; }
  else *step += 1;
}

__global__ __launch_bounds__(256) void clip_scale_kernel(float* __restrict__ g, size_t n,
                                                         const double* __restrict__ partials,
                                                         int nparts, float max_norm,
                                                         float* norm_out) {
  __shared__ double red[256];
  double a = 0.0;
  for (int i = threadIdx.x; i < nparts; i += 256) a += partials[i];
  red[threadIdx.x] = a;
  __syncthreads();
  for (int o = 128; o > 0; o >>= 1) {
    if ((int)threadIdx.x < o) red[threadIdx.x] += red[threadIdx.x + o];
    __syncthreads();
  }
  const float total = (float)sqrt(red[0]);
  float coef = max_norm / (total + 1e-6f);
  coef = coef < 1.f ? coef : 1.f;
  if (!(total == total)) coef = total;
  if (blockIdx.x == 0 && threadIdx.x == 0 && norm_out) *norm_out = total;
  for (size_t i = (size_t)blockIdx.x * 256 + threadIdx.x; i < n; i += (size_t)gridDim.x * 256)
    g[i] *= coef;
}

template <bool BF>
__device__ __forceinline__ f32x4 load4(const void* in, size_t off) {
  if constexpr (BF) {
    const u32x2 v = *reinterpret_cast<const u32x2*>(static_cast<const unsigned short*>(in) + off);
    return f32x4{__uint_as_float(v[0] << 16), __uint_as_float(v[0] & 0xffff0000u),
                 __uint_as_float(v[1] << 16), __uint_as_float(v[1] & 0xffff0000u)};
  } else {
    return *reinterpret_cast<const f32x4*>(static_cast<const float*>(in) + off);
  }
}
template <bool BF>
__device__ __forceinline__ float load1(const void* in, size_t off) {
  if constexpr (BF) return __uint_as_float((unsigned)static_cast<const unsigned short*>(in)[off] << 16);
  else return static_cast<const float*>(in)[off];
}

template <bool BF>
__global__ __launch_bounds__(256) void colsum_partial(int N, int C, const void* __restrict__ in,
                                                      int ld, int rows_per, int vec,
                                                      float* __restrict__ part) {
  __shared__ f32x4 red[16][16];
  const int cq = threadIdx.x & 15, rl = threadIdx.x >> 4;
  const int c = blockIdx.x * 64 + cq * 4;
  const int r0 = blockIdx.y * rows_per, r1 = min(N, r0 + rows_per);
  f32x4 acc = {0.f, 0.f, 0.f, 0.f};
  if (c < C) {
    if (vec && c + 3 < C) {
      for (int rb = r0 + rl; rb < r1; rb += 256) {
        f32x4 blk = {0.f, 0.f, 0.f, 0.f};
        const int re = min(r1, rb + 256);
        for (int r = rb; r < re; r += 16) blk += load4<BF>(in, (size_t)r * ld + c);
        acc += blk;
      }
    } else {
      for (int r = r0 + rl; r < r1; r += 16)
        for (int e = 0; e < 4; ++e)
          if (c + e < C) acc[e] += load1<BF>(in, (size_t)r * ld + c + e);
    }
  }
  red[rl][cq] = acc;
  __syncthreads();
  if (threadIdx.x < 64) {
    const int q = threadIdx.x >> 2, e = threadIdx.x & 3;
    float s = 0.f;
    for (int i = 0; i < 16; ++i) s += red[i][q][e];
    const int cc = blockIdx.x * 64 + threadIdx.x;
    if (cc < C) part[(size_t)blockIdx.y * C + cc] = s;
  }
}

__global__ __launch_bounds__(256) void colsum_final(int C, int R, const float* __restrict__ part,
                                                    float* __restrict__ out, float* __restrict__ out2,
                                                    float beta) {
  const int c = blockIdx.x * 256 + threadIdx.x;
  if (c >= C) return;
  float s = 0.f;
  for (int r0 = 0; r0 < R; r0 += 16) {
    float b = 0.f;
    const int r1 = min(R, r0 + 16);
// ... 7 lines not shown
static int colsum_chunks(int N, int C) {
  const int cb = (C + 63) / 64;
  int R = (1024 + cb - 1) / cb;
  const int rmax = (N + 63) / 64;
  if (R > rmax) R = rmax;
  if (R > 256) R = 256;
  if (R < 1) R = 1;
  return R;
}

__global__ __launch_bounds__(256) void dropout_kernel(size_t n, const float* __restrict__ x,
                                                      float* __restrict__ y,
                                                      unsigned short* __restrict__ ybf,
                                                      const float* __restrict__ mask,
                                                      unsigned long long seed,
                                                      unsigned long long qoff, float p, bool vec) {
  const float keep = 1.f - p, scale = 1.f / keep;
  const size_t nq = (n + 3) / 4;
  const unsigned long long dk = drop_key(seed);
  for (size_t q = (size_t)blockIdx.x * 256 + threadIdx.x; q < nq; q += (size_t)gridDim.x * 256) {
    unsigned long long r = 0;
    if (!mask) r = drop_quad(dk, qoff + q);
    if (vec && q * 4 + 3 < n) {
      const f32x4 xv = *reinterpret_cast<const f32x4*>(x + q * 4);
      f32x4 v;
#pragma unroll
      for (int e = 0; e < 4; ++e) v[e] = xv[e] * (mask ? mask[q * 4 + e] : drop_elem_scale(r, e, keep, scale));
      if (y) *reinterpret_cast<f32x4*>(y + q * 4) = v;
      if (ybf) *reinterpret_cast<bf16x4*>(ybf + q * 4) = bf16x4{f2bf(v[0]), f2bf(v[1]), f2bf(v[2]), f2bf(v[3])};
      continue;
    }
#pragma unroll
    for (int e = 0; e < 4; ++e) {
      const size_t i = q * 4 + e;
      if (i >= n) break;
      const float m = mask ? mask[i] : drop_elem_scale(r, e, keep, scale);
      const float v = x[i] * m;
      if (y) y[i] = v;
      if (ybf) ybf[i] = (unsigned short)f2bf(v);
    }
  }
}

int grid_for(size_t total, int cap) {
  size_t g = (total + 255) / 256;
  if (g > (size_t)cap) g = cap;
  if (g < 1) g = 1;
  return (int)g;
}

}

extern "C" int mlvae_sumsq_partials_count(size_t n) { return grid_for(n / 4 + 1, 1024); }

extern "C" int mlvae_grad_sumsq(const float* g, size_t n, double* partials, void* stream) {
  if (((uintptr_t)g & 15) != 0) { mlvae_set_error("grad_sumsq: grads must be 16-byte aligned"); return 1; }
  sumsq_kernel<<<mlvae_sumsq_partials_count(n), 256, 0, (hipStream_t)stream>>>(g, n, partials);
  MLVAE_CHECK_LAUNCH();
  return 0;
}

extern "C" int mlvae_adam_step_ex(float* params, float* exp_avg, float* exp_avg_sq, const float* grads,
                                  size_t n, const double* partials, int nparts, const float* loss,
                                  int* step, int* nonfinite, const int* err, int* err_skips, float lr,
                                  float beta1, float beta2, float eps, float max_norm, float* norm_out,
                                  float* hyp, int advance, void* stream) {
  if (!hyp || (((uintptr_t)params | (uintptr_t)exp_avg | (uintptr_t)exp_avg_sq | (uintptr_t)grads) & 15)) {
    mlvae_set_error("adam_step: needs hyp scratch and 16-byte aligned buffers");
    return 1;
  }
  hipStream_t s = (hipStream_t)stream;
  if (advance >= 0)
    adam_prologue<<<1, 256, 0, s>>>(partials, nparts, loss, step, lr, beta1, beta2, max_norm, hyp,
                                    norm_out, err);
  AdamArgs a;
  a.p = params; a.m = exp_avg; a.v = exp_avg_sq; a.g = grads; a.n = n; a.hyp = hyp;
  a.b1 = beta1; a.b2 = beta2; a.eps = eps;
  adam_kernel<<<grid_for(n / 4 + 1, 2048), 256, 0, s>>>(a);
  if (advance > 0) step_counter_kernel<<<1, 64, 0, s>>>(loss, step, nonfinite, err, err_skips);
  MLVAE_CHECK_LAUNCH();
  return 0;
}

extern "C" int mlvae_adam_step(float* params, float* exp_avg, float* exp_avg_sq, const float* grads,
                               size_t n, const double* partials, int nparts, const float* loss,
                               int* step, int* nonfinite, float lr, float beta1, float beta2,
                               float eps, float max_norm, float* norm_out, float* hyp,
                               int advance, void* stream) {
  return mlvae_adam_step_ex(params, exp_avg, exp_avg_sq, grads, n, partials, nparts, loss, step,
                            nonfinite, nullptr, nullptr, lr, beta1, beta2, eps, max_norm, norm_out,
                            hyp, advance, stream);
}

extern "C" int mlvae_clip_scale(float* g, size_t n, const double* partials, int nparts,
                                float max_norm, float* norm_out, void* stream) {
  if (n == 0) return 0;
  clip_scale_kernel<<<grid_for(n, 512), 256, 0, (hipStream_t)stream>>>(g, n, partials, nparts,
                                                                       max_norm, norm_out);
  MLVAE_CHECK_LAUNCH();
  return 0;
}

extern "C" size_t mlvae_colsum_workspace_size(int N, int C) {
  return (size_t)colsum_chunks(N, C) * C * sizeof(float);
}

extern "C" int mlvae_colsum_ex(int N, int C, const void* in, int in_bf16, int ld, float* out,
                               float* out2, float beta, float* ws, size_t ws_bytes, void* stream) {
  if (C == 0) return 0;
  const int R = colsum_chunks(N, C);
  if (!ws || ws_bytes < (size_t)R * C * sizeof(float)) { mlvae_set_error("colsum: workspace too small"); return 1; }
  const int rows_per = (N + R - 1) / R;
  const int vec = in_bf16 ? ((((uintptr_t)in & 7) == 0) && (ld % 4 == 0))
                          : ((((uintptr_t)in & 15) == 0) && (ld % 4 == 0));
  hipStream_t s = (hipStream_t)stream;
  if (in_bf16) colsum_partial<true><<<dim3((C + 63) / 64, R), 256, 0, s>>>(N, C, in, ld, rows_per, vec, ws);
  else colsum_partial<false><<<dim3((C + 63) / 64, R), 256, 0, s>>>(N, C, in, ld, rows_per, vec, ws);
  colsum_final<<<(C + 255) / 256, 256, 0, s>>>(C, R, ws, out, out2, beta);
  MLVAE_CHECK_LAUNCH();
  return 0;
}

extern "C" int mlvae_colsum(int N, int C, const float* in, int ld, float* out, float* out2,
                            float beta, float* ws, size_t ws_bytes, void* stream) {
  return mlvae_colsum_ex(N, C, in, 0, ld, out, out2, beta, ws, ws_bytes, stream);
}

extern "C" int mlvae_dropout_ex(size_t n, const float* x, float* y, void* y_bf16,
                                const float* mask, unsigned long long seed,
                                unsigned long long offset, float p, void* stream) {
  if (p < 0.f || p >= 1.f) { mlvae_set_error("dropout: p=%f out of range", p); return 1; }
  if (offset % 4) { mlvae_set_error("dropout: element offset %llu not a multiple of 4", offset); return 1; }
  if (!y && !y_bf16) { mlvae_set_error("dropout: no output"); return 1; }
  const bool vec = ((uintptr_t)x % 16) == 0 && ((uintptr_t)y % 16) == 0 && ((uintptr_t)y_bf16 % 8) == 0;
  dropout_kernel<<<grid_for(n, 2048), 256, 0, (hipStream_t)stream>>>(
      n, x, y, static_cast<unsigned short*>(y_bf16), mask, seed, offset / 4, p, vec);
  MLVAE_CHECK_LAUNCH();
  return 0;
}

extern "C" int mlvae_dropout(size_t n, const float* x, float* y, const float* mask,
                             unsigned long long seed, float p, void* stream) {
  return mlvae_dropout_ex(n, x, y, nullptr, mask, seed, 0ull, p, stream);
}

__global__ void dp_scalars_kernel(int pack, float* hdr, float* loss3, int* err) {
  if (threadIdx.x || blockIdx.x) return;
  if (pack) {
    hdr[0] = loss3[0]; hdr[1] = loss3[1]; hdr[2] = loss3[2];
    hdr[3] = *err != 0 ? 1.f : 0.f;
  } else {
    loss3[0] = hdr[0]; loss3[1] = hdr[1]; loss3[2] = hdr[2];
    if (hdr[3] > 0.f && *err == 0) *err = 1;
  }
}
extern "C" int mlvae_dp_scalars(int pack, float* hdr, float* loss3, int* err, void* stream) {
  if (!hdr || !loss3 || !err) { mlvae_set_error("dp_scalars: null pointer"); return 1; }
  dp_scalars_kernel<<<1, 64, 0, (hipStream_t)stream>>>(pack, hdr, loss3, err);
  MLVAE_CHECK_LAUNCH();
  return 0;
}
```

### ml-vae_amd/mlvae_hip/_lib.py

```python
import ctypes as C
import os

_HERE = os.path.dirname(os.path.abspath(__file__))
LIB_PATH = os.environ.get("MLVAE_LIB_PATH") or os.path.join(_HERE, "libmlvae.so")

P = C.c_void_p
I = C.c_int
F = C.c_float
SZ = C.c_size_t
U64 = C.c_ulonglong

_SIGS = {
    "mlvae_last_error": [],
    "mlvae_abi_version": [],
    "mlvae_device_check": [C.c_char_p, I],
    "mlvae_gemm_workspace_size": [I, I, I],
    "mlvae_gemm": [I, I, I, I, I, I, F, P, I, P, I, F, P, I, P, P, I, P, I, I, I, P, SZ, P],
    "mlvae_gemm_ex_workspace_size": [I, I, I],
    "mlvae_gemm_ex": [I, I, I, I, I, F, P, I, I, P, I, I, F, P, I, P, P, I, P, I, I, I, P, SZ, P],
    "mlvae_gemm_ex_drop": [I, I, I, I, I, F, P, I, I, P, I, I, F, P, I, P, P, I, P, I, I, I, U64, U64,
                           F, P, SZ, P],
    "mlvae_cast_bf16": [SZ, P, P, P],
    "mlvae_cast_bf16_t": [I, I, P, P, P],
    "mlvae_gemm_bf16_workspace_size": [I, I, I, I],
    "mlvae_gemm_bf16_set_split_target": [I],
    "mlvae_gemm_bf16_set_variant": [I],
    "mlvae_gemm_bf16": [I, I, I, I, I, I, P, I, C.c_longlong, P, I, C.c_longlong, P, I, C.c_longlong,
                        F, P, P, I, P, I, I, I, I, U64, U64, F, P, SZ, P],
    "mlvae_lstm_workspace_size": [I, I, I, C.POINTER(SZ)],
    "mlvae_lstm_fwd": [I, I, I, I, P, P, P, P, P, P, SZ, P, P],
    "mlvae_lstm_bwd": [I, I, I, I, P, P, P, P, P, P, SZ, P, P],
    "mlvae_lstm_fwd_ex": [I, I, I, I, P, P, P, P, P, P, P, SZ, P, P],
    "mlvae_lstm_bwd_ex": [I, I, I, I, P, P, P, P, P, P, P, SZ, P, P],
    "mlvae_viterbi_workspace_size": [I, I, I],
    "mlvae_viterbi_md": [I, I, I, I, P, I, P, P, P, P, P, P, F, P, SZ, P, P, P, P, P, P],
    "mlvae_phn_bce": [I, I, I, P, I, P, P, I, P, P, P, P, P, P, P],
    "mlvae_gemm_fp8": [I, I, I, P, I, P, I, P, I, P, P, P, I, P],
    "mlvae_fp8_scale_workspace_size": [],
    "mlvae_fp8_scale": [SZ, P, F, P, P, SZ, P],
    "mlvae_cast_fp8": [SZ, P, I, P, F, P, P],
    "mlvae_conv1d_supported": [I, I, I],
    "mlvae_conv1d_fwd": [I, I, I, I, I, P, I, P, P, I, P, I, P],
    "mlvae_conv1d_dgrad": [I, I, I, I, I, P, I, P, P, I, P, I, P],
    "mlvae_conv1d_wgrad_workspace_size": [I, I, I, I, I],
    "mlvae_conv1d_wgrad": [I, I, I, I, I, P, I, P, I, P, P, P, SZ, P],
    "mlvae_boundary_fwd": [SZ, P, P, P, P, U64, U64, P, P, P, P],
    "mlvae_boundary_bwd": [SZ, P, P, P, P, U64, U64, P, P, P, P, P, P],
    "mlvae_pi_sample": [SZ, P, P, U64, U64, I, P, P],
    "mlvae_pi_nll_fwd": [SZ, P, P, P, P, P],
    "mlvae_pi_nll_bwd": [SZ, P, P, P, P, P],
    "mlvae_pi_sample_k": [SZ, I, P, P, U64, U64, I, P, P],
    "mlvae_sfl_fwd": [SZ, I, I, I, P, P, P, P, P, P, F, F, F, P, P, P, P, P],
    "mlvae_sfl_bwd": [SZ, I, P, P, P, P, P, P, P, P, P, P],
    "mlvae_lstm1_fwd": [I, I, I, I, P, P, P, P, P, P, SZ, P, P],
    "mlvae_lstm1_bwd": [I, I, I, I, P, P, P, P, P, P, SZ, P, P],
    "mlvae_lstm_gates_fp16": [I, I, I],
    "mlvae_lstm_gates_fp16_t": [I, I, I, I],
    "mlvae_lstm_fwd_ex2": [I, I, I, I, P, P, P, I, P, P, P, P, U64, U64, F, P, SZ, P, P],
    "mlvae_lstm_bwd_ex2": [I, I, I, I, P, P, P, I, P, P, P, P, P, SZ, P, P],
    "mlvae_lstm_bwd_ex3": [I, I, I, I, P, P, P, I, P, P, I, P, P, P, SZ, P, P],
    "mlvae_elbo_partials_count": [I, I, I],
    "mlvae_heads_partials_count": [I, I],
    "mlvae_heads_supported": [I, I, I],
    "mlvae_heads_fused": [I, I, I, I, I, I, I, P, P, P, P, P, P, P, P, P, P, P, P, P, P, P, F,
                          P, P, P, P, P, P, P, P, P, P, P, P, P],
    "mlvae_heads_bias_workspace_size": [I, I, I, I],
    "mlvae_heads_fused_ex": [I, I, I, I, I, I, I, P, P, P, P, P, P, P, P, P, P, P, P, P, P, P, F,
                             P, P, P, P, P, P, P, P, P, P, P, P, P, SZ, P, P, P, P, P, I, P],
    "mlvae_heads_fused_ex2": [I, I, I, I, I, I, I, P, P, P, P, P, P, P, P, P, P, P, P, P, P, P, F,
                              P, P, P, P, P, P, P, P, P, P, P, P, P, SZ, P, P, P, P, P, I,
                              P, SZ, P, P, P, P, P],
    "mlvae_heads_fused_ex3": [I, I, I, I, I, I, I, P, P, P, P, P, P, P, P, P, P, P, P, P, P, P, F,
                              P, P, P, P, P, P, P, P, P, P, P, P, P, SZ, P, P, P, P, P, I,
                              P, SZ, P, P, P, P, P, P],
    "mlvae_bf16_split_rows": [P, I, I, I, P, P],
    "mlvae_dp_scalars": [I, P, P, P, P],
    "mlvae_heads_wgrad_workspace_size": [I, I, I, I],
    "mlvae_heads_set_nt_mode": [I],
    "mlvae_skinny_proj": [I, I, I, P, I, P, I, P, P, P, I, P],
    "mlvae_skinny_proj_ex": [I, I, I, P, I, P, I, P, P, P, I, I, P],
    "mlvae_skinny_nt": [I, I, I, P, I, P, I, P, I, P],
    "mlvae_skinny_tn_workspace_size": [I, I, I],
    "mlvae_skinny_tn": [I, I, I, P, I, P, I, I, P, P, P, P, SZ, P],
    "mlvae_skinny_nt_fp8": [I, I, I, P, I, P, I, P, I, P, P],
    "mlvae_skinny_tn_fp8": [I, I, I, P, I, P, I, I, P, P, P, P, P, SZ, P],
    "mlvae_skinny_dzw": [I, I, P, I, P, I, P, I, I, P, I, P, P, P, P, SZ, P],
    "mlvae_skinny_dzw_workspace_size": [I, I],
    "mlvae_encoder_supported": [I, I, I],
    "mlvae_encoder_partials_count": [I, I],
    "mlvae_encoder_workspace_size": [I, I, I, I, I],
    "mlvae_encoder_fwd": [I, I, I, I, I, P, P, P, P, P, P, P, P, U64, U64, P, P, P, P, P, P, I, P, P, P],
    "mlvae_encoder_fwd_ex": [I, I, I, I, I, P, P, P, P, P, P, P, P, U64, U64, P, P, P, P, P, P, I, P, P, I, P],
    "mlvae_encoder_bwd": [I, I, I, I, I, P, P, P, P, P, P, P, P, P, P, F, P, P, P, P, P, P, P, SZ, P],
    "mlvae_reparam_kl_fwd": [I, I, I, P, I, P, P, P, P, P, P],
    "mlvae_reparam_kl_bwd": [I, I, I, P, I, P, P, P, P, P, F, P, I, P],
    "mlvae_recon": [I, I, I, I, P, I, P, I, P, I, P, P, P, P, P, F, P, P, P],
    "mlvae_elbo_finalize": [P, I, P, I, P, P, I, I, I, I, F, F, P, P],
    "mlvae_masked_mean": [I, I, I, P, P, I, P, P],
    "mlvae_count_frames": [P, I, I, P, P],
    "mlvae_randn": [SZ, U64, U64, P, P],
    "mlvae_sumsq_partials_count": [SZ],
    "mlvae_grad_sumsq": [P, SZ, P, P],
    "mlvae_adam_step": [P, P, P, P, SZ, P, I, P, P, P, F, F, F, F, F, P, P, I, P],
    "mlvae_adam_step_ex": [P, P, P, P, SZ, P, I, P, P, P, P, P, F, F, F, F, F, P, P, I, P],
    "mlvae_colsum_workspace_size": [I, I],
    "mlvae_colsum": [I, I, P, I, P, P, F, P, SZ, P],
    "mlvae_colsum_ex": [I, I, P, I, I, P, P, F, P, SZ, P],
    "mlvae_dropout": [SZ, P, P, P, U64, F, P],
    "mlvae_dropout_ex": [SZ, P, P, P, P, U64, U64, F, P],
    "mlvae_lrelu_bwd": [SZ, P, P, P, P],
    "mlvae_clip_scale": [P, SZ, P, I, F, P, P],
    "mlvae_masked_mean_bwd": [I, I, I, P, I, P, P, P],
    "mlvae_gmm_latent_fwd": [I, I, I, P, I, P, P, U64, U64, F, P, P, P, P, P],
    "mlvae_gmm_latent_bwd": [I, I, I, P, I, P, P, F, P, P, P, P, I, P],
    "mlvae_apply_weight_fwd": [I, I, I, P, I, P, P, I, P],
    "mlvae_apply_weight_bwd": [I, I, I, P, I, P, P, I, P, I, P, P],
    "mlvae_lstm_launch_workgroups": [I, I, I, I],
    "mlvae_lstm_set_debug": [P],
    "mlvae_lstm_set_debug_mode": [I],
    "mlvae_lstm_fwd_fp8": [I, I, I, P, P, P, P, P, P, P, F, U64, U64, F, P, SZ, P, P],
    "mlvae_lstm_fwd_z": [I, I, I, P, P, P, I, I, P, P, P, P, P, P, P, P, P, P, P, P, F, U64, U64, F, P, SZ, P, P],
    "mlvae_lstm_fwd_z2": [I, I, I, P, P, P, I, I, P, P, P, P, P, P, P, P, P, P, I, P, P, F, U64, U64, F, P, SZ, P, P],
    "mlvae_lstm_bwd_fp8": [I, I, I, P, P, P, P, P, P, P, P, P, P, P, SZ, P, P],
    "mlvae_lstm_bwd_fp8_ex": [I, I, I, P, P, P, P, P, I, P, P, P, P, P, P, SZ, P, P],
    "mlvae_fp8_delayed_scale": [P, P, P, F, P, P],
    "mlvae_gemm_fp8_ex": [I, I, I, P, I, P, I, P, I, P, P, P, I, U64, U64, F, P],
    "mlvae_gemm_fp8_tn_workspace_size": [I, I, I],
    "mlvae_gemm_fp8_tn": [I, I, I, P, I, P, I, P, I, P, P, SZ, P],
    "mlvae_gemm_fp8_tn_ex_workspace_size": [I, I, I, I],
    "mlvae_gemm_fp8_tn_ex": [I, I, I, I, P, I, C.c_longlong, P, I, C.c_longlong, P, I, C.c_longlong, P, I, I, I,
                             P, SZ, P],
    "mlvae_norm_supported": [I],
    "mlvae_norm_stats": [I, I, I, P, P, P, P, F, P],
    "mlvae_norm_update": [I, P, P, P, I, F, F, P],
    "mlvae_norm_apply": [SZ, I, P, P, P, P, P],
}
_RESTYPE = {
    "mlvae_last_error": C.c_char_p,
    "mlvae_conv1d_wgrad_workspace_size": SZ,
    "mlvae_skinny_dzw_workspace_size": SZ,
    "mlvae_fp8_scale_workspace_size": SZ,
    "mlvae_gemm_fp8_tn_workspace_size": SZ,
    "mlvae_gemm_fp8_tn_ex_workspace_size": SZ,
    "mlvae_gemm_workspace_size": SZ,
    "mlvae_gemm_ex_workspace_size": SZ,
    "mlvae_colsum_workspace_size": SZ,
    "mlvae_gemm_bf16_workspace_size": SZ,
    "mlvae_skinny_tn_workspace_size": SZ,
    "mlvae_encoder_workspace_size": SZ,
    "mlvae_viterbi_workspace_size": SZ,
    "mlvae_heads_bias_workspace_size": SZ,
    "mlvae_heads_wgrad_workspace_size": SZ,
}

_lib = None


class MlvaeError(RuntimeError):
    pass


def lib():
    global _lib
    if _lib is None:
        import torch
        if not os.path.exists(LIB_PATH):
            raise MlvaeError(
                f"{LIB_PATH} is missing: build it with `python -m mlvae_hip.build` "
                "(or __graft_entry__.build()); there is no CPU fallback")
        h = C.CDLL(LIB_PATH)
        ab = "MLVAE_LIB_PATH" in os.environ
        for name, args in _SIGS.items():
            if ab and not hasattr(h, name):
                continue
            fn = getattr(h, name)
            fn.argtypes = args
            fn.restype = _RESTYPE.get(name, I)
        _lib = h
        mode = os.environ.get("MLVAE_LSTM_DEBUG_MODE")
        if mode:
            h.mlvae_lstm_set_debug_mode(int(mode))
    return _lib


def exported_symbols():
    return list(_SIGS.keys())


def last_error():
    return lib().mlvae_last_error().decode(errors="replace")


def check(rc, what=""):
    if rc != 0:
        raise MlvaeError(f"{what or 'mlvae'} failed (status {rc}): {last_error()}")
    return rc


def device_check():
    buf = C.create_string_buffer(64)
    rc = lib().mlvae_device_check(buf, 64)
    return rc, buf.value.decode()


_cus = None


def device_cus():
    global _cus
    if _cus is None:
        import torch
        _cus = torch.cuda.get_device_properties(torch.cuda.current_device()).multi_processor_count
    return _cus
```

### ml-vae_amd/mlvae_hip/engine.py

```python
import contextlib
import math
from collections import OrderedDict
from dataclasses import dataclass
from functools import partial

import torch

from . import _lib
from ._lib import check, lib

PREC = {"fp32": 0, "bf16": 1}
LOSS = {"likelihood": 0, "mse": 1}
EPI_NONE, EPI_LRELU, EPI_DLRELU, EPI_DROPOUT = 0, 1, 2, 3
EPI_OUT_F16 = 16
EPI_OUT_BF16 = 32
G8_MARGIN = 2.0


def x8_scale(p):
    s, lim = 1.0, 448.0 * (1.0 - p)
    while s * 2.0 <= lim:
        s *= 2.0
    return s

# ... 157 lines not shown
        self.E1 = empty(N, E, **f)
        self.E2 = empty(N, E, **f)
        self.ML = empty(N, 2 * Z, **f)
        self.Zs = empty(N, Z, **f)
        self.eps = empty(N, Z, **f)
        self.g16 = bool(lib().mlvae_lstm_gates_fp16_t(B, T, H, PREC[cfg.prec]))
        self.G = [empty(N, 8 * H, dtype=torch.float16 if self.g16 else torch.float32) for _ in range(L)]
        self.NBG = (B + 15) // 16
        self.dbias_rows = [empty(self.NBG, 8 * H, **f) if self.g16 else None for _ in range(L)]
        self.Cs = [empty(N, 2 * H, **f) for _ in range(L)]
        self.Y = [empty(N, 2 * H, **f) for _ in range(L)]
        self.Yd = [empty(N, 2 * H, **f) if cfg.dropout > 0 else None for _ in range(L - 1)]
        self.bf = cfg.prec == "bf16"
        b16 = dict(dtype=torch.bfloat16)
        self.Yb = [empty(N, 2 * H, **b16) for _ in range(L)] if self.bf else None
        self.Ydb = ([empty(N, 2 * H, **b16) if cfg.dropout > 0 else None for _ in range(L - 1)]
                    if self.bf else None)
        self.dGb = [empty(N, 8 * H, **b16) for _ in range(L)] if self.bf else None
        self.enc_fused = self.bf and enc_fused
        self.ZA = Z + 16 if self.enc_fused else Z
        self.Zb = empty(N, self.ZA, **b16) if self.bf else None
        f8 = self.bf and cfg.fp8
        self.X8 = {li: empty(N, 2 * H, dtype=torch.uint8) for li in range(1, L)} if f8 else None
        self.dG8 = {li: empty(N, 8 * H, dtype=torch.uint8) for li in range(0 if f8_l0 else 1, L)} if f8 else None
        self.H8 = {li: empty(N, 2 * H, dtype=torch.uint8) for li in range(0 if f8_l0 else 1, L)} if f8 else None
        self.E1b = empty(N, E, **b16) if self.enc_fused else None
        self.E2b = empty(N, E, **b16) if self.enc_fused else None
        if self.bf:
            self.Yd = [None] * (L - 1)
        self.P1 = empty(N, 2 * C, **f)
        self.P2m = empty(N, C, **f)
        self.P2v = empty(N, C, **f)
        self.MUX = empty(N, F, **f)
        self.LVX = empty(N, F, **f)
        self.dMUX = empty(N, F, **f)
        self.dLVX = empty(N, F, **f)
        self.dP2m = empty(N, C, **f)
        self.dP2v = empty(N, C, **f)
        self.dP1 = empty(N, 2 * C, **f)
        self.heads_bws = empty(lib().mlvae_heads_bias_workspace_size(B, T, F, C) // 4 + 1, **f) \
            if self.bf else None
        nwg = lib().mlvae_heads_wgrad_workspace_size(B, T, F, C) if self.bf else 0
        self.heads_wgws = empty(nwg // 4 + 1, **f) if nwg else None
        self.dY = [empty(N, 2 * H, **f) for _ in range(L)]
        self.dZs = empty(N, Z, **f)
        self.dML = empty(N, 2 * Z, **f)
        self.dE2 = empty(N, E, **f)
        self.dE1 = empty(N, E, **f)
        l = lib()
        self.nk = l.mlvae_elbo_partials_count(B, T, Z)
        self.nr = l.mlvae_elbo_partials_count(B, T, F)
        self.pk = empty(self.nk, **f)
        self.pr = empty(self.nr, **f)
        self.nh = l.mlvae_heads_partials_count(B, T)
        self.ph = empty(self.nh, **f)
        self.nke = l.mlvae_encoder_partials_count(B, T) if self.enc_fused else 0
        self.pke = empty(max(self.nke, 1), **f)
        ewb = l.mlvae_encoder_workspace_size(B, T, F, E, Z) if self.enc_fused else 0
        self.enc_ws = empty(ewb // 4 + 1, **f)
        self.conv_ws = ([empty(l.mlvae_conv1d_wgrad_workspace_size(B, T, cin, E, cfg.enc_conv) // 4 + 1, **f)
                         for cin in (F, E)] if cfg.enc_conv else None)
        self.loss = torch.zeros(3, device=device, dtype=torch.float32)
        self.count = torch.zeros(1, device=device, dtype=torch.int32)
        shapes = [(N, E, F), (N, E, E), (N, 2 * Z, E), (N, 2 * C, 2 * H), (N, C, C), (N, F, C),
                  (F, C, N), (C, C, N), (2 * C, 2 * H, N), (2 * Z, E, N), (E, E, N), (E, F, N),
                  (N, 2 * H, 8 * H), (N, Z, 8 * H), (4 * H, H, N)]
        for li in range(L):
            din = Z if li == 0 else 2 * H
            shapes += [(N, 8 * H, din), (8 * H, din, N)]
        ws = max(max(l.mlvae_gemm_workspace_size(m, n, k), l.mlvae_gemm_ex_workspace_size(m, n, k),
                     l.mlvae_gemm_bf16_workspace_size(m, n, k, 1))
                 for m, n, k in shapes)
        ws = max(ws, l.mlvae_gemm_bf16_workspace_size(4 * H, H, N, 2))
        if self.enc_fused:
            ws = max(ws, l.mlvae_skinny_tn_workspace_size(8 * H, self.ZA, N))
            if Z == 32 and (8 * H) % 256 == 0:
                ws = max(ws, l.mlvae_skinny_dzw_workspace_size(N, 8 * H))
        cs = max(l.mlvae_colsum_workspace_size(N, c) for c in (F, C, 2 * C, 8 * H, 2 * Z, E))
        self.gws = empty(max(ws, cs, 16) // 4 + 1, **f)
        self.gws_side = empty(max(ws, cs, 16) // 4 + 1, **f)
        self.gws_bytes = self.gws.numel() * 4
        xb = _lib.SZ()
        check(l.mlvae_lstm_workspace_size(B, H, PREC[cfg.prec], _lib.C.byref(xb)), "lstm_workspace_size")
        self.xbuf = empty(max(xb.value, 16), dtype=torch.uint8)
        self.reset_step()

    def reset_step(self):
        self.x = self.lens = None
        self.eps_used = None
        self.kl_parts = None
        self.layer_in = []
        self.rnn_out = self.rnn_out_bf = None
        self.heads_fused = False
        self.heads_bias = False
        self.heads_wgrad = False
        self.dy_bf16 = {li: False for li in range(self.L)}
        self.x8_fused = {}
        self.ydb_skipped = {}
        self.yb_prev = {}
        self.f8hh = {}
        self.drop_seed = {}
        self.masks = {}


def _aligned(ptr, ld, bf):
    return ptr is not None and ptr % 16 == 0 and ld % (8 if bf else 4) == 0


def _pb(t, off=0):
    return t.data_ptr() + 2 * off


def _p(t, off=0):
    return t.data_ptr() + 4 * off


def _pg(t, off=0):
    return None if t is None else _p(t, off)


def _pgb(t, off=0):
    return None if t is None else _pb(t, off)


class VAEEngine:

    def __init__(self, cfg, device="cuda", params=None, seed=123456):
        self.cfg = cfg.check()
        self.device = torch.device(device)
        if self.device.type != "cuda":
            raise RuntimeError("VAEEngine runs on the HIP device only (no CPU fallback)")
        lib()
        self.layout = ParamLayout(cfg)
        n = self.layout.total
        f = dict(device=self.device, dtype=torch.float32)
        self.flat = torch.zeros(n, **f)
        self._grad_ext = torch.zeros(4 + n, **f)
        self.grad = self._grad_ext[4:]
        self.exp_avg = torch.zeros(n, **f)
        self.exp_avg_sq = torch.zeros(n, **f)
        self.step_ctr = torch.zeros(1, device=self.device, dtype=torch.int32)
        self.nonfinite_ctr = torch.zeros(1, device=self.device, dtype=torch.int32)
        self.grad_norm = torch.zeros(1, **f)
        self.hyp = torch.zeros(4, **f)
        self.err = torch.zeros(1, device=self.device, dtype=torch.int32)
        self.err_skips = torch.zeros(1, device=self.device, dtype=torch.int32)
        self._nonfinite_seen = 0
        self.flat_bf = torch.empty(n, device=self.device, dtype=torch.bfloat16) if cfg.prec == "bf16" else None
        self.wih_t = {}
        self.fused_heads = (cfg.prec == "bf16" and bool(lib().mlvae_heads_supported(cfg.C, cfg.F, 2 * cfg.H)))
        self.w1_t = (torch.empty(2 * cfg.C * 2 * cfg.H, device=self.device, dtype=torch.bfloat16)
                     if self.fused_heads else None)
        self.w1_split = (torch.empty(2 * cfg.C * 4 * cfg.H, device=self.device, dtype=torch.bfloat16)
                         if self.fused_heads else None)
        self.fused_encoder = (cfg.prec == "bf16" and not cfg.enc_conv and
                              bool(lib().mlvae_encoder_supported(cfg.F, cfg.E, cfg.Z)))
        if cfg.prec == "bf16":
            for li in range(1, cfg.L):
                self.wih_t[li] = torch.empty(2 * cfg.H * 8 * cfg.H, device=self.device, dtype=torch.bfloat16)
            if self.fused_encoder:
                self.wih_t[0] = torch.empty(cfg.Z * 8 * cfg.H, device=self.device, dtype=torch.bfloat16)
        up, every = (range(1, cfg.L), range(cfg.L)) if cfg.fp8 else ((), ())
        self.w8 = {li: torch.empty(8 * cfg.H * 2 * cfg.H, device=self.device, dtype=torch.uint8) for li in up}
        self.w8s = {li: torch.zeros(2, device=self.device) for li in up}
        self.w8t = {li: torch.empty(2 * cfg.H * 8 * cfg.H, device=self.device, dtype=torch.uint8) for li in up}
        self.g8 = {li: torch.zeros(2, device=self.device) for li in every}
        self.g8_amax = {li: torch.zeros(2, device=self.device, dtype=torch.int32) for li in every}
        self.g8w = {li: torch.zeros(2, device=self.device) for li in every}
        self.one1 = torch.ones(1, device=self.device) if cfg.fp8 else None
        self.x8s = torch.tensor([x8_scale(cfg.dropout)], device=self.device) if cfg.fp8 else None
        self.f8ws = (torch.empty(lib().mlvae_fp8_scale_workspace_size() // 4 + 1, device=self.device)
                     if cfg.fp8 else None)
        self.g8_ready = False
        self.g8_par = 0
        self.nparts = lib().mlvae_sumsq_partials_count(n)
        self.sq_parts = torch.zeros(self.nparts, device=self.device, dtype=torch.float64)
        self.seed = seed
        self.rng_step = 0
        self._work = {}
        self._T = 0
        self._pool = _Pool(self.device)
        self.force_overlap = None
        self.overlap = True
        self.split_overlap = 128
        self.split_tail = 160
        self.side_stream = torch.cuda.Stream(self.device)
        self._on_side = False
        self.kernel_timers = None
        self.process_group = None
        self.world = 1
        self.rank = 0
        self.global_offset = 0
        self.bucket_allreduce = True
        self.comm_stream = None
        self._ar_pending = False
        self.ar_split = self.layout.offsets[f"decoder.rnn.weight_ih_l{cfg.L - 1}"]
        if params is not None:
            self.load_reference_params(params)

    dy_bf16 = property(lambda self: self.cfg.prec == "bf16")
    zproj = property(lambda self: True)
    heads_wgrad = property(lambda self: True)

    def view(self, name, buf=None):
        buf = self.flat if buf is None else buf
        o = self.layout.offsets[name]
        return buf[o:o + self.layout.numel(name)].view(self.layout.shapes[name])

    def named_parameters(self):
        return OrderedDict((k, self.view(k)) for k in self.layout.shapes)

    def named_grads(self):
        return OrderedDict((k, self.view(k, self.grad)) for k in self.layout.shapes)

    @classmethod
    def from_modules(cls, encoder, decoder, device="cuda", prec="fp32", kld_weight=1e-3,
                     recon_weight=1.0, lr=1e-3, betas=(0.9, 0.999), eps=1e-8,
                     max_grad_norm=5.0, seed=123456, fp8=False):
        heads = decoder.mean_fc.linear_plan()
        if hasattr(encoder, "conv"):
            c0 = encoder.conv[0].conv_plan()[0][0]
            F, E, kconv = c0.in_channels, c0.out_channels, c0.kernel_size[0]
        else:
            lin0 = encoder.fc[0].linear_plan()[0][0]
            F, E, kconv = lin0.in_features, lin0.out_features, 0
        cfg = VAEConfig(F=F, E=E, enc_conv=kconv,
                        Z=encoder.mean_fc.out_features, H=decoder.rnn.hidden_size,
# ... 10 lines not shown
            for n, p in mod.named_parameters():
                p.data = eng.view(pre + n)
                p.grad = eng.view(pre + n, eng.grad)
        return eng

    def init_default(self, seed=None):
        g = torch.Generator(device=self.device).manual_seed(self.seed if seed is None else seed)
        with torch.no_grad():
            for name, shp in self.layout.shapes.items():
                if ".rnn." in name:
                    bound = 1.0 / math.sqrt(self.cfg.H)
                else:
                    wshape = self.layout.shapes[name[:-4] + "weight"] if name.endswith("bias") else shp
                    bound = 1.0 / math.sqrt(math.prod(wshape[1:]))
                v = self.view(name)
                v.uniform_(-bound, bound, generator=g)
        return self

    def load_reference_params(self, params):
        with torch.no_grad():
            for k, v in params.items():
                self.view(k).copy_(torch.as_tensor(v, dtype=torch.float32))

    def _ptr(self, name, buf=None):
        return _p(self.flat if buf is None else buf, self.layout.offsets[name])

    def _gp(self, name):
        return self._ptr(name, self.grad)

    def _wb(self, name):
        if self.flat_bf is None:
            return None
        return _pb(self.flat_bf, self.layout.offsets[name])

    def _fp8_whh(self, w, li, shifted=False):
        H, N, T = self.cfg.H, w.N, w.T
        l = lib()
        st = self._stream()
        check(l.mlvae_cast_fp8(N * 2 * H, _pb(w.Yb[li]), 1, None, x8_scale(self.cfg.dropout), w.H8[li].data_ptr(),
                               st), "cast_fp8")
        check(l.mlvae_gemm_fp8_tn_ex(4 * H, H, N, 2, w.dG8[li].data_ptr(), 8 * H, 4 * H, w.H8[li].data_ptr(), 2 * H, H,
                                     self._gp(f"decoder.rnn.weight_hh_l{li}"), H, 4 * H * H, _p(self.g8w[li], 1),
                                     0 if shifted else T, 0 if shifted else -1, 0 if shifted else 2,
                                     _p(self._ws(w)), w.gws_bytes, st), "gemm_fp8_tn_ex")

    def _whh_bf16(self, w, li, dG_bf, preshifted):
        H, N, T = self.cfg.H, w.N, w.T
        Yb = w.Yb[li]
        ld, lh = 8 * H, 2 * H
        C = self._gp(f"decoder.rnn.weight_hh_l{li}")
        if preshifted:
            self._fast(w, 1, 0, 4 * H, H, N, _pb(dG_bf), ld, _pb(Yb), lh, C, H, batch=2, a_bs=4 * H, b_bs=H,
                       c_bs=4 * H * H)
            return
        nb = N // T
        if nb > 1:
            ca0, cb0 = T * ld, (T - 1) * lh
            self._fast(w, 1, 0, 4 * H, H, nb - 1, _pb(dG_bf, ca0), T * ld, _pb(Yb, cb0), T * lh, C, H, batch=2,
                       a_bs=(T - 1) * ld + 4 * H - ca0, b_bs=T * lh + H - cb0, c_bs=4 * H * H)
        self._fast(w, 1, 0, 4 * H, H, N - 1, _pb(dG_bf, ld), ld, _pb(Yb), lh, C, H, batch=2,
                   a_bs=4 * H - ld, b_bs=lh + H, c_bs=4 * H * H, beta=-1.0 if nb > 1 else 0.0)

    def _dzw_path(self, N):
        cfg = self.cfg
        return bool(cfg.Z == 32 and (8 * cfg.H) % 256 == 0 and N >= 65536)

    def _f8_layer0(self, N):
        cfg = self.cfg
        return bool(cfg.fp8 and self.fused_encoder
                    and not self._dzw_path(N) and N >= 4096 and (8 * cfg.H) % 256 == 0 and cfg.H % 16 == 0)

    def work(self, B, T):
        key = (B, T)
        if key not in self._work:
            self._work = {key: _Work(self.cfg, B, T, self.device,
                                     enc_fused=self.fused_encoder, pool=self._pool, f8_l0=self._f8_layer0(B * T))}
        return self._work[key]

    def _stream(self):
        if self._on_side:
            return self.side_stream.cuda_stream
        return torch.cuda.current_stream(self.device).cuda_stream

    def _ws(self, w):
        return w.gws_side if self._on_side else w.gws

    def _mm(self, w, ta, tb, M, N, K, A, lda, B, ldb, C, ldc, A_bf=None, B_bf=None, bias1=None,
            bias2=None, epi=0, aux=None, ldaux=0, kshift_T=0, kshift=0, beta=0.0, drop_seed=None):
        if self.cfg.prec == "bf16":
            a, abf = (A_bf, 1) if A_bf is not None else (A, 0)
            b, bbf = (B_bf, 1) if B_bf is not None else (B, 0)
            if _aligned(a, lda, abf) and _aligned(b, ldb, bbf):
                ws = self._ws(w)
                if drop_seed is not None:
                    check(lib().mlvae_gemm_ex_drop(ta, tb, M, N, K, 1.0, a, abf, lda, b, bbf, ldb, beta,
                                                   C, ldc, bias1, bias2, EPI_DROPOUT, aux, ldaux,
                                                   kshift_T, kshift, drop_seed, self._drop_off,
                                                   self.cfg.dropout,
                                                   _p(ws), w.gws_bytes, self._stream()),
                          "mlvae_gemm_ex_drop")
                    return True
                check(lib().mlvae_gemm_ex(ta, tb, M, N, K, 1.0, a, abf, lda, b, bbf, ldb, beta, C,
                                          ldc, bias1, bias2, epi, aux, ldaux, kshift_T, kshift,
                                          _p(ws), w.gws_bytes, self._stream()), "mlvae_gemm_ex")
                return False
        if A is None or B is None:
            raise RuntimeError("GEMM operand exists only as bf16 but is not 16-byte aligned")
        check(lib().mlvae_gemm(PREC[self.cfg.prec], ta, tb, M, N, K, 1.0, A, lda, B, ldb, beta, C,
                               ldc, bias1, bias2, epi, aux, ldaux, kshift_T, kshift,
                               _p(self._ws(w)), w.gws_bytes, self._stream()), "mlvae_gemm")
        return False

    def _fast(self, w, ta, tb, M, N, K, A_bf, lda, B_bf, ldb, C, ldc, batch=1, a_bs=0, b_bs=0,
              c_bs=0, bias1=None, bias2=None, drop_seed=None, out_f16=False, out_bf16=False, beta=0.0):
        epi, p = (EPI_DROPOUT, self.cfg.dropout) if drop_seed is not None else (EPI_NONE, 0.0)
        if out_f16:
            epi |= EPI_OUT_F16
        if out_bf16:
            epi |= EPI_OUT_BF16
        check(lib().mlvae_gemm_bf16(ta, tb, M, N, K, batch, A_bf, lda, a_bs, B_bf, ldb, b_bs, C, ldc,
                                    c_bs, beta, bias1, bias2, epi, None, 0, 0, 0, 0,
                                    drop_seed or 0, self._drop_off, p, _p(self._ws(w)), w.gws_bytes,
                                    self._stream()), "mlvae_gemm_bf16")

    def _colsum(self, w, N, Cn, src, ld, out, out2=None):
        check(lib().mlvae_colsum(N, Cn, src, ld, out, out2, 0.0, _p(self._ws(w)), w.gws_bytes,
                                 self._stream()), "mlvae_colsum")

    def _side(self, fn, ev=None):
        if not self.overlap:
            return fn()
        if ev is None:
            ev = self._mark()
        self.side_stream.wait_event(ev)
        self._on_side = True
        try:
            fn()
        finally:
            self._on_side = False

    def _mark(self):
        ev = torch.cuda.Event()
        ev.record(torch.cuda.current_stream(self.device))
        return ev

    def _defer_side(self, pending, fn):
        if not self.overlap:
            return fn()
        pending.append((fn, self._mark()))

    def _flush_side(self, pending):
        for fn, ev in pending:
            self._side(fn, ev)
        pending.clear()

    @contextlib.contextmanager
    def _timed(self, name):
        on = self.kernel_timers is not None and not self._on_side
        if on:
            a = torch.cuda.Event(enable_timing=True)
            a.record(torch.cuda.current_stream(self.device))
        yield
        if on:
            b = torch.cuda.Event(enable_timing=True)
            b.record(torch.cuda.current_stream(self.device))
            self.kernel_timers.setdefault(name, []).append((a, b))

    def _join_side(self):
        if self.overlap:
            ev = torch.cuda.Event()
            ev.record(self.side_stream)
            torch.cuda.current_stream(self.device).wait_event(ev)

    def forward(self, x, lens, eps=None, train=False, dropout_masks=None, need_grad_inputs=False):
        cfg = self.cfg
        B, T, Fdim = x.shape
        if Fdim != cfg.F:
            raise ValueError(f"feature dim {Fdim} != input_size {cfg.F}")
        x = x.contiguous()
        if x.data_ptr() % 16:
            x = x.clone()
        lens = lens.to(device=self.device, dtype=torch.float32).contiguous()
        w = self.work(B, T)
        w.reset_step()
        w.x, w.lens = x, lens
        self._T = T
        if self.world > 1:
            self.global_offset = self.rank * B
        prep_ev = self._prep_weights(B, train)
        count = self._global_count(w) if self.world > 1 else None
        self._encode(w, eps)
        layer_in = (w.Zs, (w.Zb if w.bf else None), cfg.Z, w.ZA)
        for li in range(cfg.L):
            if li == 1 and prep_ev is not None:
                torch.cuda.current_stream(self.device).wait_event(prep_ev)
                prep_ev = None
            w.layer_in.append(layer_in)
            zproj = self._input_projection(w, li)
            layer_in = self._recurrence_fwd(w, li, zproj, train, dropout_masks)
        if prep_ev is not None:
            torch.cuda.current_stream(self.device).wait_event(prep_ev)
        w.rnn_out = w.Y[cfg.L - 1]
        w.rnn_out_bf = w.Yb[cfg.L - 1] if w.bf else None
        w.heads_fused = self.fused_heads and w.bf
        recon_parts, n = (self._heads_fused if w.heads_fused else self._heads_unfused)(w, train, count)
        w_kl, w_rec = self.loss_weights()
        check(lib().mlvae_elbo_finalize(_p(w.kl_parts[0]), w.kl_parts[1], _p(recon_parts), n, _p(lens), count, B, T,
                                        cfg.Z, cfg.F, w_kl, w_rec, _p(w.loss), self._stream()), "elbo_finalize")
        return w

    def _prep_weights(self, B, train):
        if self.flat_bf is None:
            return None
        check(lib().mlvae_cast_bf16(self.layout.total, _p(self.flat), _pb(self.flat_bf), self._stream()), "cast_bf16")
        if self._full_chip(B):
            self._weight_prep(train)
            return None
        self._on_side = True
        self.side_stream.wait_event(self._mark())
        try:
            self._weight_prep(train)
        finally:
            self._on_side = False
        prep_ev = torch.cuda.Event()
        prep_ev.record(self.side_stream)
        return prep_ev

    def _weight_prep(self, train):
        cfg, l, s = self.cfg, lib(), self._stream()
        if train and self.w1_t is not None:
            check(l.mlvae_cast_bf16_t(2 * cfg.C, 2 * cfg.H, self._ptr("decoder.mean_fc.blocks.0.weight"),
                                      _pb(self.w1_t), s), "cast_bf16_t")
        if train:
            for li, dst in self.wih_t.items():
                check(l.mlvae_cast_bf16_t(8 * cfg.H, cfg.Z if li == 0 else 2 * cfg.H,
                                          self._ptr(f"decoder.rnn.weight_ih_l{li}"), _pb(dst), s), "cast_bf16_t")
        n = 8 * cfg.H * 2 * cfg.H
        for li in self.w8:
            wih = self._ptr(f"decoder.rnn.weight_ih_l{li}")
            check(l.mlvae_fp8_scale(n, wih, x8_scale(cfg.dropout), _p(self.w8s[li]), _p(self.f8ws),
                                    self.f8ws.numel() * 4, s), "fp8_scale")
            check(l.mlvae_cast_fp8(n, wih, 0, _p(self.w8s[li]), 0.0, self.w8[li].data_ptr(), s), "cast_fp8")
            if train and li in self.wih_t:
                check(l.mlvae_cast_fp8(n, _pb(self.wih_t[li]), 1, _p(self.w8s[li]), 0.0,
                                       self.w8t[li].data_ptr(), s), "cast_fp8")

    def _encode(self, w, eps):
        cfg = self.cfg
        B, T, N, E, Z, Fd = w.B, w.T, w.N, cfg.E, cfg.Z, cfg.F
        l, s = lib(), self._stream()
        X, lens, wb = _p(w.x), w.lens, self._wb
        eps_off = self._eps_offset(T) + self.rng_step * (1 << 40)
        eps_t = None if eps is None else eps.to(self.device, torch.float32).contiguous().view(N, Z)
        w.eps_used = w.eps if eps_t is None else eps_t
        if w.enc_fused:
            ep = lambda n: self._ptr(f"encoder.{n}")
            with self._timed("encoder_fwd"):
                check(l.mlvae_encoder_fwd_ex(B, T, Fd, E, Z, X, ep("fc.0.blocks.0.weight"), ep("fc.0.blocks.0.bias"),
                                           ep("fc.0.blocks.2.weight"), ep("fc.0.blocks.2.bias"),
                                           ep("mean_fc.weight"), ep("mean_fc.bias"),
                                           None if eps_t is None else _p(eps_t), self.seed, eps_off, _p(lens),
                                           _pb(w.E1b), _pb(w.E2b), _p(w.ML), _p(w.Zs), _pb(w.Zb), w.ZA,
                                           _p(w.eps) if eps_t is None else None, _p(w.pke), 1,
                                           s), "encoder_fwd")
            w.kl_parts = (w.pke, w.nke)
            return
        if eps_t is None:
            check(l.mlvae_randn(N * Z, self.seed, eps_off, _p(w.eps), s), "mlvae_randn")
        ep = cfg.enc_prefix
        if cfg.enc_conv:
            K = cfg.enc_conv
            with self._timed("conv_fwd"):
                check(l.mlvae_conv1d_fwd(B, T, Fd, E, K, X, Fd, self._ptr(f"{ep}.0.weight"),
                                         self._ptr(f"{ep}.0.bias"), 1, _p(w.E1), E, s), "conv1d_fwd")
                check(l.mlvae_conv1d_fwd(B, T, E, E, K, _p(w.E1), E, self._ptr(f"{ep}.2.weight"),
                                         self._ptr(f"{ep}.2.bias"), 1, _p(w.E2), E, s), "conv1d_fwd")
        else:
            self._mm(w, 0, 1, N, E, Fd, X, Fd, self._ptr(f"{ep}.0.weight"), Fd,
                     _p(w.E1), E, B_bf=wb(f"{ep}.0.weight"),
                     bias1=self._ptr(f"{ep}.0.bias"), epi=EPI_LRELU)
            self._mm(w, 0, 1, N, E, E, _p(w.E1), E, self._ptr(f"{ep}.2.weight"), E,
                     _p(w.E2), E, B_bf=wb(f"{ep}.2.weight"),
                     bias1=self._ptr(f"{ep}.2.bias"), epi=EPI_LRELU)
        self._mm(w, 0, 1, N, 2 * Z, E, _p(w.E2), E, self._ptr("encoder.mean_fc.weight"), E,
                 _p(w.ML), 2 * Z, B_bf=wb("encoder.mean_fc.weight"), bias1=self._ptr("encoder.mean_fc.bias"))
        check(l.mlvae_reparam_kl_fwd(B, T, Z, _p(w.ML), 2 * Z, _p(w.eps_used), _p(lens), _p(w.Zs),
                                     None, _p(w.pk), s), "reparam_kl_fwd")
        if w.bf:
            check(l.mlvae_cast_bf16(N * Z, _p(w.Zs), _pb(w.Zb), s), "cast_bf16")
        w.kl_parts = (w.pk, w.nk)

    def _input_projection(self, w, li):
        cfg = self.cfg
        N, H = w.N, cfg.H
        l, s, wb = lib(), self._stream(), self._wb
        xin, xin_bf, din, ldx = w.layer_in[li]
        W, b_ih, b_hh = (self._ptr(f"decoder.rnn.{n}_l{li}") for n in ("weight_ih", "bias_ih", "bias_hh"))
        if li == 0 and w.bf and w.g16 and din == 32 and ldx % 8 == 0 and xin_bf is not None:
            return True
        if w.bf and din <= 32 and din % 8 == 0:
            check(l.mlvae_skinny_proj_ex(N, 8 * H, din, _pb(xin_bf), ldx, wb(f"decoder.rnn.weight_ih_l{li}"), din,
                                         b_ih, b_hh, _p(w.G[li]), 8 * H, int(w.g16), s), "skinny_proj")
        elif w.bf and cfg.fp8 and li > 0 and din % 16 == 0 and ldx == din:
            xs = x8_scale(cfg.dropout)
            with self._timed(f"proj_l{li}"):
                if not w.x8_fused[li]:
                    check(l.mlvae_cast_fp8(N * din, _pb(xin_bf), 1, None, xs, w.X8[li].data_ptr(), s), "cast_fp8")
                check(l.mlvae_gemm_fp8(N, 8 * H, din, w.X8[li].data_ptr(), din, self.w8[li].data_ptr(), din,
                                       _p(w.G[li]), 8 * H, _p(self.w8s[li], 1), b_ih, b_hh,
                                       EPI_OUT_F16 if w.g16 else EPI_NONE, s), "gemm_fp8")
        elif w.bf and din % 8 == 0:
            with self._timed(f"proj_l{li}"):
                self._fast(w, 0, 1, N, 8 * H, din, _pb(xin_bf), ldx, wb(f"decoder.rnn.weight_ih_l{li}"),
                           din, _p(w.G[li]), 8 * H, bias1=b_ih, bias2=b_hh, out_f16=w.g16)
        else:
            if w.g16:
                raise RuntimeError("fp16 gate buffer needs a bf16 layer input with din % 8 == 0")
            self._mm(w, 0, 1, N, 8 * H, din, _pg(xin), din, W, din, _p(w.G[li]), 8 * H,
                     A_bf=_pgb(xin_bf), B_bf=wb(f"decoder.rnn.weight_ih_l{li}"), bias1=b_ih, bias2=b_hh)
        return False

    def _recurrence_fwd(self, w, li, zproj, train, dropout_masks):
        cfg = self.cfg
        B, T, N, H = w.B, w.T, w.N, cfg.H
        l, s = lib(), self._stream()
        _, xin_bf, din, ldx = w.layer_in[li]
        W_hh, W_hh_r = self._ptr(f"decoder.rnn.weight_hh_l{li}"), self._ptr(f"decoder.rnn.weight_hh_l{li}_reverse")
        drop = li < cfg.L - 1 and train and cfg.dropout > 0
        fuse_drop = w.g16 and drop and dropout_masks is None
        need_y = (not w.g16 or (drop and not fuse_drop) or
                  (li == cfg.L - 1 and not (self.fused_heads and w.bf)))
        seed = self._drop_seed(li) if fuse_drop else 0
        x8_fused = bool(cfg.fp8 and fuse_drop and not need_y and (li + 1) in w.X8 and 2 * H % 16 == 0)
        x8_ptr = w.X8[li + 1].data_ptr() if x8_fused else None
        w.x8_fused[li + 1] = x8_fused
        skip_ydb = bool(x8_fused and self.g8_ready
                        and l.mlvae_gemm_fp8_tn_workspace_size(8 * H, 2 * H, N) <= w.gws_bytes)
        w.ydb_skipped[li + 1] = skip_ydb
        ydb_arg = None if skip_ydb else (_pb(w.Ydb[li]) if fuse_drop else None)
        yb_prev = bool(zproj and fuse_drop)
        w.yb_prev[li] = yb_prev
        with self._timed("lstm_fwd"):
            if zproj:
                rp = lambda n: self._ptr(f"decoder.rnn.{n}")
                check(l.mlvae_lstm_fwd_z2(B, T, H, W_hh, W_hh_r, _pb(xin_bf), ldx, din,
                                          rp("weight_ih_l0"), rp("weight_ih_l0_reverse"),
                                          rp("bias_ih_l0"), rp("bias_hh_l0"), rp("bias_ih_l0_reverse"),
                                          rp("bias_hh_l0_reverse"), _p(w.G[li]), _p(w.Cs[li]),
                                          _p(w.Y[li]) if need_y else None, _pb(w.Yb[li]), int(yb_prev),
                                          ydb_arg, x8_ptr, x8_scale(cfg.dropout) if x8_fused else 0.0, seed,
                                          self._drop_off, cfg.dropout if fuse_drop else 0.0,
                                          _p(w.xbuf), w.xbuf.numel(), _p(self.err), s), "lstm_fwd_z2")
            elif x8_fused:
                check(l.mlvae_lstm_fwd_fp8(B, T, H, W_hh, W_hh_r, _p(w.G[li]), _p(w.Cs[li]), _pb(w.Yb[li]),
                                           ydb_arg, x8_ptr, x8_scale(cfg.dropout), seed, self._drop_off, cfg.dropout,
                                           _p(w.xbuf), w.xbuf.numel(), _p(self.err), s), "lstm_fwd_fp8")
            else:
                check(l.mlvae_lstm_fwd_ex2(PREC[cfg.prec], B, T, H, W_hh, W_hh_r, _p(w.G[li]), int(w.g16),
                                           _p(w.Cs[li]), _p(w.Y[li]) if need_y else None, _pgb(w.Yb[li] if w.bf else None),
                                           _pb(w.Ydb[li]) if fuse_drop else None, seed, self._drop_off,
                                           cfg.dropout if fuse_drop else 0.0,
                                           _p(w.xbuf), w.xbuf.numel(), _p(self.err), s), "lstm_fwd")
        if not drop:
            return w.Y[li], (w.Yb[li] if w.bf else None), 2 * H, 2 * H
        if fuse_drop:
            w.drop_seed[li] = (seed, None)
        else:
            self._dropout(w, li, w.Y[li], w.Yd[li], dropout_masks)
        return w.Yd[li], (w.Ydb[li] if w.bf else None), 2 * H, 2 * H

    def _heads_fused(self, w, train, count):
        cfg = self.cfg
        B, T, H, C, Fd = w.B, w.T, cfg.H, cfg.C, cfg.F
        l, s, wb = lib(), self._stream(), self._wb
        lt = LOSS[cfg.loss_type]
        _, w_rec = self.loss_weights()
        hp = lambda name: self._ptr(f"decoder.{name}")
        hg = lambda name: self._gp(f"decoder.{name}")
        w.heads_bias = bool(train)
        w.dy_bf16[cfg.L - 1] = bool(w.heads_bias and w.g16)
        bias_args = (_p(w.heads_bws), w.heads_bws.numel() * 4, hg("mean_fc.blocks.4.bias"),
                     hg("log_var_fc.blocks.4.bias"), hg("mean_fc.blocks.2.bias"),
                     hg("log_var_fc.blocks.2.bias"), hg("mean_fc.blocks.0.bias")) \
            if w.heads_bias else (None, 0, None, None, None, None, None)
        w.heads_wgrad = bool(w.heads_bias and w.heads_wgws is not None)
        mse_h = lt == 1
        wg_args = (_p(w.heads_wgws), w.heads_wgws.numel() * 4, hg("mean_fc.blocks.4.weight"),
                   None if mse_h else hg("log_var_fc.blocks.4.weight"), hg("mean_fc.blocks.2.weight"),
                   None if mse_h else hg("log_var_fc.blocks.2.weight")) \
            if w.heads_wgrad else (None, 0, None, None, None, None)
        if train:
            check(l.mlvae_bf16_split_rows(hp("mean_fc.blocks.0.weight"), 2 * C, 2 * H, 64, _pb(self.w1_split), s),
                  "bf16_split_rows")
        with self._timed("heads"):
            check(l.mlvae_heads_fused_ex3(
              B, T, Fd, C, 2 * H, lt, 1 if train else 0, _pb(w.rnn_out_bf), wb("decoder.mean_fc.blocks.0.weight"),
              _pb(self.w1_t) if train else None, hp("mean_fc.blocks.0.bias"),
              hp("mean_fc.blocks.2.weight"), hp("mean_fc.blocks.2.bias"),
              hp("mean_fc.blocks.4.weight"), hp("mean_fc.blocks.4.bias"),
              hp("log_var_fc.blocks.2.weight"), hp("log_var_fc.blocks.2.bias"),
              hp("log_var_fc.blocks.4.weight"), hp("log_var_fc.blocks.4.bias"),
              _p(w.x), _p(w.lens), count, w_rec, _p(w.P1), _p(w.P2m), _p(w.P2v), _p(w.MUX), _p(w.LVX),
              _p(w.dMUX) if train else None, _p(w.dLVX) if (train and lt == 0) else None,
              _p(w.dP2m) if train else None, _p(w.dP2v) if train else None,
              _p(w.dP1) if train else None, _p(w.dY[cfg.L - 1]) if train else None,
              _p(w.ph), *bias_args, (3 if w.dy_bf16[cfg.L - 1] else 1) if w.heads_bias else 0,
              *wg_args, _pb(self.w1_split) if train else None, s), "heads_fused")
        return w.ph, w.nh

    def _heads_unfused(self, w, train, count):
        cfg = self.cfg
        B, T, N, H, C, Fd = w.B, w.T, w.N, cfg.H, cfg.C, cfg.F
        l, s, wb = lib(), self._stream(), self._wb
        lt = LOSS[cfg.loss_type]
        _, w_rec = self.loss_weights()
        self._mm(w, 0, 1, N, 2 * C, 2 * H, _p(w.rnn_out), 2 * H, self._ptr("decoder.mean_fc.blocks.0.weight"),
                 2 * H, _p(w.P1), 2 * C, A_bf=_pgb(w.rnn_out_bf), B_bf=wb("decoder.mean_fc.blocks.0.weight"),
                 bias1=self._ptr("decoder.mean_fc.blocks.0.bias"), epi=EPI_LRELU)
        for hd, P2, out in (("mean_fc", w.P2m, w.MUX), ("log_var_fc", w.P2v, w.LVX)):
            off = 0 if hd == "mean_fc" else C
            self._mm(w, 0, 1, N, C, C, _p(w.P1, off), 2 * C,
                     self._ptr(f"decoder.{hd}.blocks.2.weight"), C, _p(P2), C,
                     B_bf=wb(f"decoder.{hd}.blocks.2.weight"),
                     bias1=self._ptr(f"decoder.{hd}.blocks.2.bias"), epi=EPI_LRELU)
            self._mm(w, 0, 1, N, Fd, C, _p(P2), C, self._ptr(f"decoder.{hd}.blocks.4.weight"), C,
                     _p(out), Fd, B_bf=wb(f"decoder.{hd}.blocks.4.weight"),
                     bias1=self._ptr(f"decoder.{hd}.blocks.4.bias"))
        dmux = _p(w.dMUX) if train else None
        dlvx = _p(w.dLVX) if (train and lt == 0) else None
        check(l.mlvae_recon(B, T, Fd, lt, _p(w.MUX), Fd, _p(w.LVX), Fd, _p(w.x), Fd, _p(w.lens), count,
                            None, _p(w.pr), None, w_rec, dmux, dlvx, s), "recon")
        return w.pr, w.nr

    def loss_weights(self):
        return float(self.cfg.kld_weight), float(self.cfg.recon_weight)

    def _eps_offset(self, T):
        return self.global_offset * T * self.cfg.Z

    @property
    def _drop_off(self):
        return self.global_offset * self._T * 2 * self.cfg.H

    def _drop_seed(self, li):
        return (self.seed * 1000003 + self.rng_step * 131 + li) & ((1 << 63) - 1)
# ... 54 lines not shown
        N, H, C, Fd = w.N, cfg.H, cfg.C, cfg.F
        wb = self._wb
        fused = w.heads_fused
        side = partial(self._defer_side, pending) if fused else self._side
        mse = cfg.loss_type == "mse"
        heads = [("mean_fc", w.P2m, w.dMUX, w.dP2m, 0)]
        if not mse:
            heads.append(("log_var_fc", w.P2v, w.dLVX, w.dP2v, C))
        for hd, P2, dOut, dP2, off in heads:
            W3, W2 = f"decoder.{hd}.blocks.4", f"decoder.{hd}.blocks.2"
            if not w.heads_wgrad:
                side(partial(self._heads_wg, w, W3, Fd, dOut, P2, 0, C))
            if not fused:
                self._mm(w, 0, 0, N, C, Fd, _p(dOut), Fd, self._ptr(f"{W3}.weight"), C, _p(dP2), C,
                         B_bf=wb(f"{W3}.weight"), epi=EPI_DLRELU, aux=_p(P2), ldaux=C)
            if not w.heads_wgrad:
                side(partial(self._heads_wg, w, W2, C, dP2, w.P1, off, 2 * C))
            if not fused:
                self._mm(w, 0, 0, N, C, C, _p(dP2), C, self._ptr(f"{W2}.weight"), C, _p(w.dP1, off), 2 * C,
                         B_bf=wb(f"{W2}.weight"), epi=EPI_DLRELU, aux=_p(w.P1, off), ldaux=2 * C)
        K1 = C if mse else 2 * C
        side(partial(self._heads_wg1, w, K1))
        if not fused:
            self._mm(w, 0, 0, N, 2 * H, K1, _p(w.dP1), 2 * C, self._ptr("decoder.mean_fc.blocks.0.weight"),
                     2 * H, _p(w.dY[cfg.L - 1]), 2 * H, B_bf=wb("decoder.mean_fc.blocks.0.weight"))

    def _heads_wg(self, w, name, M, dy, x, off, ldx):
        N, C = w.N, self.cfg.C
        if w.heads_fused:
            self._mm(w, 1, 0, M, C, N, None, M, None, ldx, self._gp(f"{name}.weight"), C,
                     A_bf=_p(dy), B_bf=_pb(x, off))
        else:
            self._mm(w, 1, 0, M, C, N, _p(dy), M, _p(x, off), ldx, self._gp(f"{name}.weight"), C)
            self._colsum(w, N, M, _p(dy), M, self._gp(f"{name}.bias"))

    def _heads_wg1(self, w, K1):
        N, H, C = w.N, self.cfg.H, self.cfg.C
        R_bf = _pb(w.rnn_out_bf) if w.bf else None
        if w.heads_fused:
            self._fast(w, 1, 0, K1, 2 * H, N, _p(w.dP1), 2 * C, R_bf, 2 * H,
                       self._gp("decoder.mean_fc.blocks.0.weight"), 2 * H)
            return
        self._mm(w, 1, 0, K1, 2 * H, N, _p(w.dP1), 2 * C, _p(w.rnn_out), 2 * H,
                 self._gp("decoder.mean_fc.blocks.0.weight"), 2 * H, B_bf=R_bf)
        self._colsum(w, N, K1, _p(w.dP1), 2 * C, self._gp("decoder.mean_fc.blocks.0.bias"))

    def _lstm_layer_bwd(self, w, li, pending, split_target):
        cfg = self.cfg
        N, H = w.N, cfg.H
        l = lib()
        _, _, din, ldx = w.layer_in[li]
        f8 = bool(cfg.fp8 and w.g16 and li in w.dG8)
        f8_dgrad = f8 and self.g8_ready
        f8w = bool(f8_dgrad and li in w.X8 and ldx == din and din % 16 == 0
                   and l.mlvae_gemm_fp8_tn_workspace_size(8 * H, din, N) <= w.gws_bytes)
        f8hh = bool(f8w and li in w.H8
                    and H % 16 == 0 and l.mlvae_gemm_fp8_tn_ex_workspace_size(4 * H, H, N, 2) <= w.gws_bytes)
        f8l0 = bool(li == 0 and f8_dgrad and w.enc_fused and 0 in w.H8
                    and l.mlvae_gemm_fp8_tn_ex_workspace_size(4 * H, H, N, 2) <= w.gws_bytes
                    and l.mlvae_skinny_tn_workspace_size(8 * H, w.ZA, N) <= w.gws_bytes)
        if li == 0:
            f8hh = f8l0
        w.f8hh[li] = f8hh
        self._bptt(w, li, f8, f8_dgrad, f8hh)
        self._flush_side(pending)
        if w.ydb_skipped.get(li) and not f8w:
            raise RuntimeError(f"layer {li}: the forward skipped the bf16 dropout(h) the bf16 weight gradient reads")
        wgl = partial(self._lstm_wgrads, w, li, split_target, f8w, f8hh)
        if li == 0:
            self._defer_side(pending, wgl)
        self._dgrad(w, li, f8_dgrad, f8hh)
        self._flush_side(pending)
        if li > 0:
            self._defer_side(pending, wgl)
        return f8

    def _bptt(self, w, li, f8, f8_dgrad, f8hh):
        cfg = self.cfg
        B, T, H = w.B, w.T, cfg.H
        l, s = lib(), self._stream()
        W_hh, W_hh_r = self._ptr(f"decoder.rnn.weight_hh_l{li}"), self._ptr(f"decoder.rnn.weight_hh_l{li}_reverse")
        dGb = w.dGb[li] if w.bf else None
        dyb = w.dy_bf16[li]
        with self._timed("lstm_bwd"):
            rows = w.dbias_rows[li] if (w.g16 and not (li == 0 and w.enc_fused)) else None
            if f8:
                par = self.g8_par
                am = self.g8_amax[li].data_ptr()
                if f8_dgrad:
                    check(l.mlvae_fp8_delayed_scale(am + 4 * (1 - par), None, _p(self.x8s), G8_MARGIN,
                                                    _p(self.g8w[li]), s), "fp8_delayed_scale")
                other = self.one1 if li == 0 else self.w8s[li]
                check(l.mlvae_fp8_delayed_scale(am + 4 * (1 - par), am + 4 * par, _p(other), G8_MARGIN,
                                                _p(self.g8[li]), s), "fp8_delayed_scale")
                check(l.mlvae_lstm_bwd_fp8_ex(B, T, H, W_hh, W_hh_r, _p(w.G[li]),
                                           _p(w.Cs[li]), _p(w.dY[li]), int(dyb), None if f8hh else _pb(dGb),
                                           _pg(rows), w.dG8[li].data_ptr() if f8_dgrad else None, _p(self.g8[li]),
                                           am + 4 * par, _p(w.xbuf), w.xbuf.numel(), _p(self.err), s),
                      "lstm_bwd_fp8")
            else:
                check(l.mlvae_lstm_bwd_ex3(PREC[cfg.prec], B, T, H, W_hh, W_hh_r, _p(w.G[li]),
                                           int(w.g16), _p(w.Cs[li]), _p(w.dY[li]), int(dyb), _pgb(dGb), _pg(rows),
                                           _p(w.xbuf), w.xbuf.numel(), _p(self.err), s), "lstm_bwd")

    def _lstm_wgrads(self, w, li, split_target, f8w, f8hh):
        prev = lib().mlvae_gemm_bf16_set_split_target(split_target)
        try:
            self._wgrad_layer(w, li, f8w, f8hh)
        finally:
            lib().mlvae_gemm_bf16_set_split_target(prev)

    def _wgrad_hh(self, w, li, f8hh):
        pre = w.yb_prev[li]
        with self._timed(f"wgrad_hh_l{li}"):
            if f8hh:
                self._fp8_whh(w, li, shifted=pre)
            else:
                self._whh_bf16(w, li, w.dGb[li], pre)

    def _wgrad_layer(self, w, li, f8w, f8hh):
        if li == 0 and w.enc_fused:
            self._wgrad_hh(w, 0, f8hh)
            return
        N, T, H, gp = w.N, w.T, self.cfg.H, self._gp
        xin, xin_bf, din, ldx = w.layer_in[li]
        dG, dG_bf = (None, w.dGb[li]) if w.bf else (w.G[li], None)
        Ybl = w.Yb[li] if w.bf else None
        if dG_bf is not None and xin_bf is not None and din % 8 == 0 and H % 8 == 0:
            with self._timed(f"wgrad_ih_l{li}"):
                if f8w:
                    check(lib().mlvae_gemm_fp8_tn(8 * H, din, N, w.dG8[li].data_ptr(), 8 * H, w.X8[li].data_ptr(),
                                                  din, gp(f"decoder.rnn.weight_ih_l{li}"), din,
                                                  _p(self.g8w[li], 1), _p(self._ws(w)), w.gws_bytes, self._stream()),
                          "gemm_fp8_tn")
                else:
                    self._fast(w, 1, 0, 8 * H, din, N, _pb(dG_bf), 8 * H, _pb(xin_bf), ldx,
                               gp(f"decoder.rnn.weight_ih_l{li}"), din)
            self._wgrad_hh(w, li, f8hh)
        else:
            self._mm(w, 1, 0, 8 * H, din, N, _pg(dG), 8 * H, _pg(xin), din,
                     gp(f"decoder.rnn.weight_ih_l{li}"), din, A_bf=_pgb(dG_bf), B_bf=_pgb(xin_bf))
            self._mm(w, 1, 0, 4 * H, H, N, _pg(dG), 8 * H, _p(w.Y[li]), 2 * H,
                     gp(f"decoder.rnn.weight_hh_l{li}"), H, A_bf=_pgb(dG_bf), B_bf=_pgb(Ybl),
                     kshift_T=T, kshift=-1)
            self._mm(w, 1, 0, 4 * H, H, N, _pg(dG, 4 * H), 8 * H, _p(w.Y[li], H), 2 * H,
                     gp(f"decoder.rnn.weight_hh_l{li}_reverse"), H, A_bf=_pgb(dG_bf, 4 * H),
                     B_bf=_pgb(Ybl, H), kshift_T=T, kshift=1)
        if w.g16:
            self._colsum(w, w.NBG, 8 * H, _p(w.dbias_rows[li]), 8 * H,
                         gp(f"decoder.rnn.bias_ih_l{li}"), gp(f"decoder.rnn.bias_hh_l{li}"))
        elif dG_bf is not None:
            check(lib().mlvae_colsum_ex(N, 8 * H, _pb(dG_bf), 1, 8 * H, gp(f"decoder.rnn.bias_ih_l{li}"),
                                        gp(f"decoder.rnn.bias_hh_l{li}"), 0.0, _p(self._ws(w)), w.gws_bytes,
                                        self._stream()), "colsum")
        else:
            self._colsum(w, N, 8 * H, _p(dG), 8 * H, gp(f"decoder.rnn.bias_ih_l{li}"),
                         gp(f"decoder.rnn.bias_hh_l{li}"))

    def _dgrad(self, w, li, f8_dgrad, f8hh):
        cfg = self.cfg
        N, Z, H = w.N, cfg.Z, cfg.H
        l, s, gp, wb = lib(), self._stream(), self._gp, self._wb
        dG, dG_bf = (None, w.dGb[li]) if w.bf else (w.G[li], None)
        if li == 0 and w.enc_fused:
            if self._dzw_path(N) and w.ZA >= 48:
                check(l.mlvae_skinny_dzw(N, 8 * H, _pb(dG_bf), 8 * H, _pb(self.wih_t[0]), 8 * H, _pb(w.Zb),
                                         w.ZA, Z, _p(w.dZs), Z, gp("decoder.rnn.weight_ih_l0"),
                                         gp("decoder.rnn.bias_ih_l0"), gp("decoder.rnn.bias_hh_l0"),
                                         _p(w.gws), w.gws_bytes, s), "skinny_dzw")
            elif f8hh:
                check(l.mlvae_skinny_nt_fp8(N, Z, 8 * H, w.dG8[0].data_ptr(), 8 * H, _pb(self.wih_t[0]), 8 * H,
                                            _p(w.dZs), Z, _p(self.g8[0], 1), s), "skinny_nt_fp8")
            else:
                check(l.mlvae_skinny_nt(N, Z, 8 * H, _pb(dG_bf), 8 * H, _pb(self.wih_t[0]), 8 * H,
                                        _p(w.dZs), Z, s), "skinny_nt")
            return
        xin, _, din, _ = w.layer_in[li]
        dx = w.dZs if li == 0 else w.dY[li - 1]
        drop = li > 0 and xin is not w.Y[li - 1]
        seed, mask_ptr = w.drop_seed[li - 1] if drop else (None, None)
        drop_fused = drop and mask_ptr is None
        dyb = bool(w.g16 and w.heads_fused and (drop_fused or not drop))
        if f8_dgrad:
            epi8 = EPI_DROPOUT if drop_fused else EPI_NONE
            if dyb:
                w.dy_bf16[li - 1] = True
# ... 2 lines not shown
                                          8 * H, _p(dx), din, _p(self.g8[li], 1), None, None,
                                          epi8 | (EPI_OUT_BF16 if dyb else 0),
                                          (seed or 0) if epi8 else 0, self._drop_off, cfg.dropout, s),
                      "gemm_fp8_ex")
        elif dG_bf is not None and li in self.wih_t and din >= 256:
            if dyb:
                w.dy_bf16[li - 1] = True
            with self._timed(f"dgrad_l{li}"):
                self._fast(w, 0, 1, N, din, 8 * H, _pb(dG_bf), 8 * H, _pb(self.wih_t[li]), 8 * H,
                           _p(dx), din, drop_seed=seed if drop_fused else None, out_bf16=dyb)
        else:
            drop_fused = self._mm(w, 0, 0, N, din, 8 * H, _pg(dG), 8 * H,
                                  self._ptr(f"decoder.rnn.weight_ih_l{li}"), din, _p(dx), din,
                                  A_bf=_pgb(dG_bf), B_bf=wb(f"decoder.rnn.weight_ih_l{li}"),
                                  drop_seed=seed if drop_fused else None)
        if drop and not drop_fused:
            check(l.mlvae_dropout_ex(dx.numel(), _p(dx), _p(dx), None, mask_ptr, seed, self._drop_off,
                                     cfg.dropout, s), "dropout_bwd")

    def _encoder_bwd_fused(self, w, count, w_kl):
        cfg = self.cfg
        B, T, N, E, Z, H, Fd = w.B, w.T, w.N, cfg.E, cfg.Z, cfg.H, cfg.F
        l, s, gp = lib(), self._stream(), self._gp
        ep = lambda n: self._ptr(f"encoder.{n}")
        ge = lambda n: gp(f"encoder.{n}")
        with self._timed("encoder_bwd"):
            check(l.mlvae_encoder_bwd(B, T, Fd, E, Z, _p(w.dZs), _p(w.ML), _p(w.eps_used), _pb(w.E1b),
                                    _pb(w.E2b), _p(w.x), ep("mean_fc.weight"), ep("fc.0.blocks.2.weight"),
                                    _p(w.lens), count, w_kl, ge("mean_fc.weight"), ge("mean_fc.bias"),
                                    ge("fc.0.blocks.2.weight"), ge("fc.0.blocks.2.bias"),
                                    ge("fc.0.blocks.0.weight"), ge("fc.0.blocks.0.bias"), _p(w.enc_ws),
                                    w.enc_ws.numel() * 4, s), "encoder_bwd")
        if w.f8hh[0]:
            check(l.mlvae_skinny_tn_fp8(8 * H, w.ZA, N, w.dG8[0].data_ptr(), 8 * H, _pb(w.Zb), w.ZA, Z,
                                        gp("decoder.rnn.weight_ih_l0"), gp("decoder.rnn.bias_ih_l0"),
                                        gp("decoder.rnn.bias_hh_l0"), _p(self.g8[0], 1), _p(w.gws), w.gws_bytes,
                                        s), "skinny_tn_fp8")
        elif not (self._dzw_path(N) and w.ZA >= 48):
            check(l.mlvae_skinny_tn(8 * H, w.ZA, N, _pb(w.dGb[0]), 8 * H, _pb(w.Zb), w.ZA, Z,
                                    gp("decoder.rnn.weight_ih_l0"), gp("decoder.rnn.bias_ih_l0"),
                                    gp("decoder.rnn.bias_hh_l0"), _p(w.gws), w.gws_bytes, s), "skinny_tn")

    def _encoder_bwd(self, w, count, w_kl):
        cfg = self.cfg
        B, T, N, E, Z, Fd = w.B, w.T, w.N, cfg.E, cfg.Z, cfg.F
        l, s, wb = lib(), self._stream(), self._wb
        check(l.mlvae_reparam_kl_bwd(B, T, Z, _p(w.ML), 2 * Z, _p(w.eps_used), _p(w.lens), count,
                                     _p(w.dZs), None, w_kl, _p(w.dML), 2 * Z, s), "reparam_kl_bwd")
        self._side(partial(self._wgrad_fc, w, 2 * Z, E, w.dML, w.E2, "encoder.mean_fc"))
        self._mm(w, 0, 0, N, E, 2 * Z, _p(w.dML), 2 * Z, self._ptr("encoder.mean_fc.weight"), E,
                 _p(w.dE2), E, B_bf=wb("encoder.mean_fc.weight"), epi=EPI_DLRELU, aux=_p(w.E2), ldaux=E)
        ep = cfg.enc_prefix
        if cfg.enc_conv:
            K = cfg.enc_conv
            self._side(partial(self._wgrad_conv, w, E, w.dE2, _p(w.E1), 2, w.conv_ws[1]))
            with self._timed("conv_bwd"):
                check(l.mlvae_conv1d_dgrad(B, T, E, E, K, _p(w.dE2), E, self._ptr(f"{ep}.2.weight"), _p(w.E1),
                                           E, _p(w.dE1), E, s), "conv1d_dgrad")
                self._wgrad_conv(w, Fd, w.dE1, _p(w.x), 0, w.conv_ws[0])
            return
        self._side(partial(self._wgrad_fc, w, E, E, w.dE2, w.E1, f"{ep}.2"))
        self._mm(w, 0, 0, N, E, E, _p(w.dE2), E, self._ptr(f"{ep}.2.weight"), E,
                 _p(w.dE1), E, B_bf=wb(f"{ep}.2.weight"), epi=EPI_DLRELU,
                 aux=_p(w.E1), ldaux=E)
        self._wgrad_fc(w, E, Fd, w.dE1, w.x, f"{ep}.0")

    def _wgrad_fc(self, w, M, K, dy, xin, name):
        self._mm(w, 1, 0, M, K, w.N, _p(dy), M, _p(xin), K, self._gp(f"{name}.weight"), K)
        self._colsum(w, w.N, M, _p(dy), M, self._gp(f"{name}.bias"))

    def _wgrad_conv(self, w, cin, dy, xin, name, ws):
        cfg = self.cfg
        ep, E = cfg.enc_prefix, cfg.E
        check(lib().mlvae_conv1d_wgrad(w.B, w.T, cin, E, cfg.enc_conv, _p(dy), E, xin, cin,
                                       self._gp(f"{ep}.{name}.weight"), self._gp(f"{ep}.{name}.bias"),
                                       _p(ws), ws.numel() * 4, self._stream()), "conv1d_wgrad")

    def optimizer_step(self, w):
        cfg, l, s = self.cfg, lib(), self._stream()
        if self.world > 1:
            self._allreduce_grads(w)
        check(l.mlvae_grad_sumsq(_p(self.grad), self.layout.total, self.sq_parts.data_ptr(), s), "sumsq")
        b1, b2 = cfg.betas
        check(l.mlvae_adam_step_ex(_p(self.flat), _p(self.exp_avg), _p(self.exp_avg_sq), _p(self.grad),
                                   self.layout.total, self.sq_parts.data_ptr(), self.nparts,
                                   _p(w.loss, 2), self.step_ctr.data_ptr(), self.nonfinite_ctr.data_ptr(),
                                   self.err.data_ptr(), self.err_skips.data_ptr(),
                                   cfg.lr, b1, b2, cfg.adam_eps, cfg.max_grad_norm,
                                   _p(self.grad_norm), _p(self.hyp), 1, s), "adam")

    def _start_suffix_allreduce(self):
        from . import dist as mdist
        if self.comm_stream is None:
            self.comm_stream = torch.cuda.Stream(self.device)
        self.comm_stream.wait_stream(torch.cuda.current_stream(self.device))
        if self.overlap:
            self.comm_stream.wait_stream(self.side_stream)
        with torch.cuda.stream(self.comm_stream):
            mdist.allreduce_grad_bucket(self.grad[self.ar_split:], self.process_group)
        self._ar_pending = True

    def _allreduce_grads(self, w):
        from . import dist as mdist
        l, s = lib(), self._stream()
        hdr = self._grad_ext
        check(l.mlvae_dp_scalars(1, _p(hdr), _p(w.loss), self.err.data_ptr(), s), "dp_scalars")
        if self._ar_pending:
            torch.cuda.current_stream(self.device).wait_stream(self.comm_stream)
            mdist.allreduce_grad_bucket(hdr[:4 + self.ar_split], self.process_group)
            self._ar_pending = False
        else:
            mdist.allreduce_grad_bucket(hdr, self.process_group)
        check(l.mlvae_dp_scalars(0, _p(hdr), _p(w.loss), self.err.data_ptr(), s), "dp_scalars")

    def normalise(self, x, lens, norm, epoch=0):
        B, T, F = x.shape
        l, s = lib(), self._stream()
        if not l.mlvae_norm_supported(F):
            raise ValueError(f"input normalisation kernels need F % 4 == 0 (F={F})")
        x = x.contiguous()
        if x.data_ptr() % 16:
            x = x.clone()
        lens = lens.to(device=self.device, dtype=torch.float32).contiguous()
        utt = self._pool("norm_utt", (B, 2 * F))
        sums = self._pool("norm_sums", (2 * F + 4,))
        out = self._pool("norm_x", (B, T, F))
        with self._timed("norm"):
            check(l.mlvae_norm_stats(B, T, F, _p(x), _p(lens), _p(utt), _p(sums), float(norm.eps), s),
                  "norm_stats")
            if norm.training and self.world > 1:
                from . import dist as mdist
                mdist.allreduce_loss(sums[:2 * F + 1], self.process_group)
            gm, gs = norm.glob_mean, norm.glob_std
            fresh = gm.numel() == 0
            if fresh:
                gm = torch.zeros(F, device=self.device)
                gs = torch.zeros(F, device=self.device)
            elif gm.device != self.device or gm.dtype != torch.float32 or not gm.is_contiguous() \
                    or gm.data_ptr() % 16 or gs.data_ptr() % 16:
                gm = gm.to(self.device, torch.float32).contiguous().clone()
                gs = gs.to(self.device, torch.float32).contiguous().clone()
            norm.glob_mean, norm.glob_std = gm, gs
            mode, w_old, w_new = (1 if fresh else 0), 0.0, 0.0
            if norm.training:
                if norm.count == 0:
                    mode = 1
                elif epoch < norm.update_until_epoch:
                    wt = norm.avg_factor if norm.avg_factor is not None else 1.0 / (norm.count + 1)
                    mode, w_old, w_new = 2, 1 - wt, wt
                norm.count += 1
            check(l.mlvae_norm_update(F, _p(sums), _p(gm), _p(gs), mode, w_old, w_new, s), "norm_update")
            check(l.mlvae_norm_apply(B * T, F, _p(x), _p(gm), _p(gs), _p(out), s), "norm_apply")
        return out

    def train_step(self, x, lens, eps=None, dropout_masks=None, normalizer=None, epoch=0):
        if normalizer is not None:
            x = self.normalise(x, lens, normalizer, epoch)
        w = self.forward(x, lens, eps=eps, train=True, dropout_masks=dropout_masks)
        self.backward(w)
        self.optimizer_step(w)
        self.rng_step += 1
        return w.loss

    def eval_step(self, x, lens, eps=None, normalizer=None, epoch=0):
        if normalizer is not None:
            x = self.normalise(x, lens, normalizer, epoch)
        w = self.forward(x, lens, eps=eps, train=False)
        if self.world > 1:
            from . import dist as mdist
            mdist.allreduce_loss(w.loss, self.process_group)
        self.rng_step += 1
        return w.loss

    def check_errors(self):
        if int(self.err.item()) != 0:
            raise RuntimeError("LSTM recurrence hand-off timed out (err word set): the outputs "
                               "of the affected steps are undefined; their optimizer updates were "
                               f"skipped ({int(self.err_skips.item())} steps)")

    def check_health(self, nonfinite_patience=3, where=""):
        self.check_errors()
        ctr = int(self.nonfinite_ctr.item())
        new = ctr - self._nonfinite_seen
        self._nonfinite_seen = ctr
        if new > nonfinite_patience:
            raise ValueError(f"Loss is not finite and patience is exhausted ({new} non-finite "
                             f"steps skipped{where}, patience {nonfinite_patience})")
        return new
```

Before: 13.90 million.

## Fuse weight prep, norm update/apply, adam step and LSTM exchange clearing into fewer launches

Batches the bf16 weight casts and transposed casts into a single multi-segment weight_prep kernel. It also fuses the normalizer's global-stat update with the apply pass and switches to a fused Adam step that uses a ticket counter. LSTM exchange buffers are now zeroed for the next call inside the recurrent kernel itself, so the per-call hipMemsetAsync goes away. The aim is to cut kernel launch and memset overhead per training step, at the cost of more complex state (a thread-local hand-off and a clean flag) that could go stale after errors.

```diff
diff --git a/include/mlvae.h b/include/mlvae.h
--- a/include/mlvae.h
+++ b/include/mlvae.h
@@ -38,8 +38,10 @@
                     void* stream);
 int mlvae_cast_bf16(size_t n, const float* x, void* y, void* stream);
 int mlvae_cast_bf16_t(int rows, int cols, const float* x, void* y, void* stream);
+int mlvae_weight_prep(int nseg, const long long* desc, void* stream);
 
 int mlvae_lstm_workspace_size(int B, int H, int prec, size_t* xbytes);
+int mlvae_lstm_exchange_next(int xbuf_is_zero, void* clear, size_t clear_bytes);
 int mlvae_lstm_fwd(int prec, int B, int T, int H, const float* w_hh_fwd, const float* w_hh_rev,
                    float* gates, float* cells, float* y, void* xbuf, size_t xbytes, int* err,
                    void* stream);
@@ -279,6 +281,9 @@
                       float w_old, float w_new, void* stream);
 int mlvae_norm_apply(size_t rows, int F, const float* x, const float* glob_mean, const float* glob_std,
                      float* out, void* stream);
+int mlvae_norm_update_apply(size_t rows, int F, const float* x, const float* sums, const float* glob_mean,
+                            const float* glob_std, float* glob_mean_out, float* glob_std_out, int mode,
+                            float w_old, float w_new, float* out, void* stream);
 
 int mlvae_sumsq_partials_count(size_t n);
 int mlvae_grad_sumsq(const float* grads, size_t n, double* partials, void* stream);
@@ -293,6 +298,12 @@
                        float beta2, float eps, float max_norm, float* norm_out, float* hyp_scratch,
                        int advance, void* stream);
 
+int mlvae_adam_step_fused(float* params, float* exp_avg, float* exp_avg_sq, const float* grads,
+                          size_t n, const double* partials, int nparts, const float* loss, int* step,
+                          int* nonfinite, const int* err, int* err_skips, float lr, float beta1,
+                          float beta2, float eps, float max_norm, float* norm_out, float* hyp_scratch,
+                          unsigned* ticket, void* stream);
+
 int mlvae_clip_scale(float* grads, size_t n, const double* partials, int nparts, float max_norm,
                      float* norm_out, void* stream);
 
diff --git a/ml-vae_amd/csrc/gemm_bf16.hip b/ml-vae_amd/csrc/gemm_bf16.hip
--- a/ml-vae_amd/csrc/gemm_bf16.hip
+++ b/ml-vae_amd/csrc/gemm_bf16.hip
@@ -423,17 +423,29 @@
                             ws_bytes, stream);
 }
 
-__global__ __launch_bounds__(256) void cast_bf16_kernel(size_t n, const float* __restrict__ x,
-                                                        unsigned short* __restrict__ y) {
+__device__ __forceinline__ void cast_bf16_block(size_t n, const float* __restrict__ x,
+                                                unsigned short* __restrict__ y, unsigned blk, unsigned nblk) {
   const size_t n4 = n / 4;
-  for (size_t i = (size_t)blockIdx.x * 256 + threadIdx.x; i < n4; i += (size_t)gridDim.x * 256) {
+  for (size_t i = (size_t)blk * 256 + threadIdx.x; i < n4; i += (size_t)nblk * 256) {
     const f32x4 v = reinterpret_cast<const f32x4*>(x)[i];
     u32x2 o = {(unsigned)bf_bits(v[0]) | ((unsigned)bf_bits(v[1]) << 16),
                (unsigned)bf_bits(v[2]) | ((unsigned)bf_bits(v[3]) << 16)};
     reinterpret_cast<u32x2*>(y)[i] = o;
   }
-  for (size_t i = n4 * 4 + (size_t)blockIdx.x * 256 + threadIdx.x; i < n; i += (size_t)gridDim.x * 256)
+  for (size_t i = n4 * 4 + (size_t)blk * 256 + threadIdx.x; i < n; i += (size_t)nblk * 256)
     y[i] = bf_bits(x[i]);
+}
+
+__global__ __launch_bounds__(256) void cast_bf16_kernel(size_t n, const float* __restrict__ x,
+                                                        unsigned short* __restrict__ y) {
+  cast_bf16_block(n, x, y, blockIdx.x, gridDim.x);
+}
+
+static unsigned cast_blocks(size_t n) {
+  size_t blocks = (n / 4 + 255) / 256;
+  if (blocks > 4096) blocks = 4096;
+  if (blocks < 1) blocks = 1;
+  return (unsigned)blocks;
 }
 
 extern "C" int mlvae_cast_bf16(size_t n, const float* x, void* y, void* stream) {
@@ -442,31 +454,32 @@
     mlvae_set_error("mlvae_cast_bf16: needs 16-byte aligned x, 8-byte aligned y");
     return 1;
   }
-  size_t blocks = (n / 4 + 255) / 256;
-  if (blocks > 4096) blocks = 4096;
-  if (blocks < 1) blocks = 1;
-  cast_bf16_kernel<<<(unsigned)blocks, 256, 0, (hipStream_t)stream>>>(n, x,
-                                                                       static_cast<unsigned short*>(y));
+  cast_bf16_kernel<<<cast_blocks(n), 256, 0, (hipStream_t)stream>>>(n, x, static_cast<unsigned short*>(y));
   MLVAE_CHECK_LAUNCH();
   return 0;
+}
+
+__device__ __forceinline__ void cast_bf16_t_tile(int rows, int cols, const float* __restrict__ x,
+                                                 unsigned short* __restrict__ y, float (*t)[33], int bx, int by) {
+  const int r0 = by * 32, c0 = bx * 32;
+  const int tx = threadIdx.x & 31, ty = threadIdx.x >> 5;
+#pragma unroll
+  for (int k = 0; k < 4; ++k) {
+    const int r = r0 + ty + 8 * k, c = c0 + tx;
+    t[ty + 8 * k][tx] = (r < rows && c < cols) ? x[(size_t)r * cols + c] : 0.f;
+  }
+  __syncthreads();
+#pragma unroll
+  for (int k = 0; k < 4; ++k) {
+    const int c = c0 + ty + 8 * k, r = r0 + tx;
+    if (c < cols && r < rows) y[(size_t)c * rows + r] = bf_bits(t[tx][ty + 8 * k]);
+  }
 }
 
 __global__ __launch_bounds__(256) void cast_bf16_t_kernel(int rows, int cols, const float* __restrict__ x,
                                                           unsigned short* __restrict__ y) {
   __shared__ float t[32][33];
-  const int r0 = blockIdx.y * 32, c0 = blockIdx.x * 32;
-  const int tx = threadIdx.x & 31, ty = threadIdx.x >> 5;
-#pragma unroll
-  for (int k = 0; k < 4; ++k) {
-    const int r = r0 + ty + 8 * k, c = c0 + tx;
-    t[ty + 8 * k][tx] = (r < rows && c < cols) ? x[(size_t)r * cols + c] : 0.f;
-  }
-  __syncthreads();
-#pragma unroll
-  for (int k = 0; k < 4; ++k) {
-    const int c = c0 + ty + 8 * k, r = r0 + tx;
-    if (c < cols && r < rows) y[(size_t)c * rows + r] = bf_bits(t[tx][ty + 8 * k]);
-  }
+  cast_bf16_t_tile(rows, cols, x, y, t, blockIdx.x, blockIdx.y);
 }
 
 extern "C" int mlvae_cast_bf16_t(int rows, int cols, const float* x, void* y, void* stream) {
@@ -477,3 +490,67 @@
   MLVAE_CHECK_LAUNCH();
   return 0;
 }
+
+constexpr int PREP_MAX = 8;
+struct PrepSeg {
+  const float* x; unsigned short* y;
+  size_t n;
+  int rows, cols;
+  unsigned blk0, nblk;
+  int tiles_x;
+};
+struct PrepArgs { PrepSeg s[PREP_MAX]; };
+
+__global__ __launch_bounds__(256) void weight_prep_kernel(PrepArgs a) {
+  __shared__ float t[32][33];
+  PrepSeg sg = a.s[0];
+#pragma unroll
+  for (int i = 1; i < PREP_MAX; ++i)
+    if (blockIdx.x >= a.s[i].blk0) sg = a.s[i];
+  const unsigned b = blockIdx.x - sg.blk0;
+  if (sg.cols == 0) cast_bf16_block(sg.n, sg.x, sg.y, b, sg.nblk);
+  else cast_bf16_t_tile(sg.rows, sg.cols, sg.x, sg.y, t, (int)(b % (unsigned)sg.tiles_x), (int)(b / (unsigned)sg.tiles_x));
+}
+
+extern "C" int mlvae_weight_prep(int nseg, const long long* desc, void* stream) {
+  if (nseg < 0 || nseg > PREP_MAX || (nseg > 0 && !desc)) {
+    mlvae_set_error("mlvae_weight_prep: 0 .. %d segments", PREP_MAX);
+    return 1;
+  }
+  PrepArgs a;
+  unsigned total = 0;
+  int used = 0;
+  for (int i = 0; i < nseg; ++i) {
+    const float* x = reinterpret_cast<const float*>((uintptr_t)desc[4 * i]);
+    unsigned short* y = reinterpret_cast<unsigned short*>((uintptr_t)desc[4 * i + 1]);
+    const long long rows = desc[4 * i + 2], cols = desc[4 * i + 3];
+    if (rows <= 0 || cols < 0) continue;
+    if (!x || !y || cols > 0x7fffffffLL || (cols > 0 && rows > 0x7fffffffLL) ||
+        (cols == 0 && (((uintptr_t)x % 16) || ((uintptr_t)y % 8)))) {
+      mlvae_set_error("mlvae_weight_prep: segment %d: null / misaligned pointer or size out of range", i);
+      return 1;
+    }
+    PrepSeg& sg = a.s[used++];
+    sg.x = x; sg.y = y; sg.blk0 = total;
+    if (cols == 0) {
+      sg.n = (size_t)rows; sg.rows = 0; sg.cols = 0; sg.tiles_x = 1;
+      sg.nblk = cast_blocks(sg.n);
+    } else {
+      sg.n = 0; sg.rows = (int)rows; sg.cols = (int)cols;
+      sg.tiles_x = (sg.cols + 31) / 32;
+      const unsigned long long nb = (unsigned long long)sg.tiles_x * ((sg.rows + 31) / 32);
+      if (nb > 0x3fffffffull) { mlvae_set_error("mlvae_weight_prep: segment %d too large", i); return 1; }
+      sg.nblk = (unsigned)nb;
+    }
+    if (total + sg.nblk < total || total + sg.nblk > 0x7fffffffu) {
+      mlvae_set_error("mlvae_weight_prep: too many blocks");
+      return 1;
+    }
+    total += sg.nblk;
+  }
+  if (!used) return 0;
+  for (int i = used; i < PREP_MAX; ++i) { a.s[i] = a.s[0]; a.s[i].blk0 = 0xffffffffu; }
+  weight_prep_kernel<<<total, 256, 0, (hipStream_t)stream>>>(a);
+  MLVAE_CHECK_LAUNCH();
+  return 0;
+}
diff --git a/ml-vae_amd/csrc/lstm.hip b/ml-vae_amd/csrc/lstm.hip
--- a/ml-vae_amd/csrc/lstm.hip
+++ b/ml-vae_amd/csrc/lstm.hip
@@ -937,10 +937,14 @@
   WideZ wz;
 };
 
+thread_local WideXNext g_xnext;
+
 int run(bool fwd, int prec, int B, int T, int H, const float* W0, const float* W1, float* G,
         float* Cs, float* Y, void* xbuf, size_t xbytes, int* err, hipStream_t st,
         unsigned short* yb = nullptr, unsigned short* dgb = nullptr, int gates_fp16 = 0,
         const WideExtra& ex = WideExtra(), int ndir = 2) {
+  const WideXNext xn = g_xnext;
+  g_xnext = WideXNext();
   if (B <= 0 || T <= 0) return 0;
   if (H <= 0 || H % 4 != 0) { mlvae_set_error("lstm: H=%d must be a positive multiple of 4", H); return 1; }
   if (prec != PREC_F32 && prec != PREC_BF16) { mlvae_set_error("lstm: bad prec %d", prec); return 1; }
@@ -958,7 +962,7 @@
     }
     if (ex.ydb && !(ex.p >= 0.f && ex.p < 1.f)) { mlvae_set_error("lstm: dropout p=%g", ex.p); return 1; }
     return lstm_wide_run(fwd, B, T, H, W0, W1, G, Cs, Y, xbuf, xbytes, err, st, yb, dgb, ex.dbias, ex.ydb,
-                         ex.seed, ex.off, ex.p, g_dbg, g_dbg_mode, ex.f8, ex.dyb, ex.wz);
+                         ex.seed, ex.off, ex.p, g_dbg, g_dbg_mode, ex.f8, ex.dyb, ex.wz, xn);
   }
   if (ex.dyb) { mlvae_set_error("lstm: bf16 dY only on the wide-batch path (fp16 gates)"); return 1; }
   if (ex.ydb || ex.dbias || !Y) {
@@ -1015,6 +1019,18 @@
 
 }
 
+extern "C" int mlvae_lstm_exchange_next(int xbuf_is_zero, void* clear, size_t clear_bytes) {
+  if (clear && (((uintptr_t)clear % 16) || (clear_bytes % 16))) {
+    mlvae_set_error("lstm_exchange_next: the region to clear must be 16-byte aligned and a multiple of 16 bytes");
+    return 1;
+  }
+  g_xnext.armed = true;
+  g_xnext.clean = xbuf_is_zero != 0;
+  g_xnext.clear = clear_bytes ? clear : nullptr;
+  g_xnext.bytes = clear ? clear_bytes : 0;
+  return 0;
+}
+
 extern "C" int mlvae_lstm_workspace_size(int B, int H, int prec, size_t* xbytes) {
   if (H <= 0 || H % 4 != 0) { mlvae_set_error("lstm: H=%d must be a positive multiple of 4", H); return 1; }
   const int bf = max_batch_per_launch(H, true, prec), bb = max_batch_per_launch(H, false, prec);
diff --git a/ml-vae_amd/csrc/lstm_common.h b/ml-vae_amd/csrc/lstm_common.h
--- a/ml-vae_amd/csrc/lstm_common.h
+++ b/ml-vae_amd/csrc/lstm_common.h
@@ -50,7 +50,16 @@
   const float* Wz1;
   const float* bz[4];
   int yb_prev;
-};
+  void* xclear;
+  unsigned xclear_n16;
+};
+
+__device__ __forceinline__ void clear_next_exchange(const LstmArgs& a) {
+  if (!a.xclear) return;
+  u32x4* c = reinterpret_cast<u32x4*>(a.xclear);
+  for (unsigned i = blockIdx.x * blockDim.x + threadIdx.x; i < a.xclear_n16; i += gridDim.x * blockDim.x)
+    c[i] = u32x4{0u, 0u, 0u, 0u};
+}
 
 __device__ __forceinline__ unsigned xcc_id() {
   return __builtin_amdgcn_s_getreg((3 << 11) | (0 << 6) | 20) & 0xf;
@@ -179,12 +188,19 @@
   const float* b[4] = {nullptr, nullptr, nullptr, nullptr};
   int yb_prev = 0;
 };
+struct WideXNext {
+  bool armed = false;
+  bool clean = false;
+  void* clear = nullptr;
+  size_t bytes = 0;
+};
 int lstm_wide_run(bool fwd, int B, int T, int H, const float* W0, const float* W1, float* G,
                   float* Cs, float* Y, void* xbuf, size_t xbytes, int* err, hipStream_t st,
                   unsigned short* yb, unsigned short* dgb, float* dbias, unsigned short* ydb,
                   unsigned long long dseed, unsigned long long doff, float dp,
                   unsigned long long* dbg, int dbg_mode, const WideFp8& f8 = WideFp8(),
-                  const unsigned short* dyb = nullptr, const WideZ& wz = WideZ());
+                  const unsigned short* dyb = nullptr, const WideZ& wz = WideZ(),
+                  const WideXNext& xn = WideXNext());
 size_t lstm_wide_xbytes(int B, int H, bool fwd);
 bool lstm_wide_t_ok(int T, int H);
 int lstm_wide_workgroups(int B, int H, bool fwd);
diff --git a/ml-vae_amd/csrc/lstm_wide.hip b/ml-vae_amd/csrc/lstm_wide.hip
--- a/ml-vae_amd/csrc/lstm_wide.hip
+++ b/ml-vae_amd/csrc/lstm_wide.hip
@@ -56,6 +56,7 @@
   unsigned* dbl = reinterpret_cast<unsigned*>(wlds + 8 * TPW * KLF * 64);
   __shared__ int abort_flag;
 
+  clear_next_exchange(a);
   const int ngroups = 2 * a.NB, gstride = (ngroups + 7) & ~7;
   const int gid = blockIdx.x % gstride, js = blockIdx.x / gstride;
   if (gid >= ngroups) return;
@@ -525,6 +526,7 @@
   char* cst = smem + 2 * AIMG + (size_t)8 * NTW * KLB * 64 * 16;
   __shared__ int abort_flag;
 
+  clear_next_exchange(a);
   const int ngroups = 2 * a.NB, gstride = (ngroups + 7) & ~7;
   const int gid = blockIdx.x % gstride, js = blockIdx.x / gstride;
   if (gid >= ngroups) return;
@@ -1031,7 +1033,7 @@
                   unsigned short* yb, unsigned short* dgb, float* dbias, unsigned short* ydb,
                   unsigned long long dseed, unsigned long long doff, float dp,
                   unsigned long long* dbg, int dbg_mode, const WideFp8& f8, const unsigned short* dyb,
-                  const WideZ& wz) {
+                  const WideZ& wz, const WideXNext& xn) {
   WidePlan p = wide_plan(B, H, fwd, dbg_mode);
   if (!p.ok) return -1;
   if (!lstm_wide_t_ok(T, H)) {
@@ -1072,7 +1074,19 @@
   }
   a.dscale = dp < 1.f ? 1.f / (1.f - dp) : 0.f;
   a.xtab = reinterpret_cast<unsigned*>(static_cast<char*>(xbuf) + p.xtab_off);
-  if (hipMemsetAsync(xbuf, 0, p.xbytes, st) != hipSuccess) {
+  if (xn.armed && xn.clear) {
+    const char* c0 = static_cast<const char*>(xn.clear);
+    const char* x0 = static_cast<const char*>(xbuf);
+    if (((uintptr_t)xn.clear % 16) || (xn.bytes % 16) || xn.bytes / 16 > 0x40000000ull ||
+        (c0 < x0 + p.xbytes && x0 < c0 + xn.bytes)) {
+      mlvae_set_error("lstm_wide: the region to clear must be 16-byte aligned, a multiple of 16 bytes and apart "
+                      "from the exchange in use");
+      return 1;
+    }
+    a.xclear = xn.clear;
+    a.xclear_n16 = (unsigned)(xn.bytes / 16);
+  }
+  if (!(xn.armed && xn.clean) && hipMemsetAsync(xbuf, 0, p.xbytes, st) != hipSuccess) {
     mlvae_set_error("lstm_wide: memset failed");
     return 2;
   }
diff --git a/ml-vae_amd/csrc/norm.hip b/ml-vae_amd/csrc/norm.hip
--- a/ml-vae_amd/csrc/norm.hip
+++ b/ml-vae_amd/csrc/norm.hip
@@ -94,6 +94,12 @@
   if (lb == 0 && f <= 2 * F) sums[f] = ((red[0][c] + red[1][c]) + red[2][c]) + red[3][c];
 }
 
+__device__ __forceinline__ float norm_blend(int mode, float g, float cur, float w1, float w) {
+#pragma clang fp contract(off)
+  const float a = w1 * g, b = w * cur;
+  return mode == 1 ? cur : a + b;
+}
+
 __global__ __launch_bounds__(NT) void norm_update_kernel(int F, const float* __restrict__ sums,
                                                          float* __restrict__ gmean, float* __restrict__ gstd,
                                                          int mode, float w1, float w) {
@@ -101,7 +107,7 @@
   for (int f = threadIdx.x; f < F; f += NT) {
     const float cm = sums[f] / cnt, cs = sums[F + f] / cnt;
     if (mode == 1) { gmean[f] = cm; gstd[f] = cs; }
-    else if (mode == 2) { gmean[f] = w1 * gmean[f] + w * cm; gstd[f] = w1 * gstd[f] + w * cs; }
+    else if (mode == 2) { gmean[f] = norm_blend(2, gmean[f], cm, w1, w); gstd[f] = norm_blend(2, gstd[f], cs, w1, w); }
   }
 }
 
@@ -117,6 +123,37 @@
   }
 }
 
+__global__ __launch_bounds__(NT) void norm_update_apply_kernel(size_t nq, int F, const f32x4* __restrict__ x,
+                                                               const float* __restrict__ sums,
+                                                               const float* __restrict__ gmean,
+                                                               const float* __restrict__ gstd,
+                                                               float* __restrict__ gmean_out,
+                                                               float* __restrict__ gstd_out, int mode, float w1,
+                                                               float w, f32x4* __restrict__ out) {
+  extern __shared__ f32x4 gl4[];
+  float* gl = reinterpret_cast<float*>(gl4);
+  if (mode == 0) {
+    for (int f = threadIdx.x; f < F; f += NT) { gl[f] = gmean[f]; gl[F + f] = gstd[f]; }
+  } else {
+    const float cnt = sums[2 * F] > 0.f ? sums[2 * F] : 1.f;
+    for (int f = threadIdx.x; f < F; f += NT) {
+      const float cm = sums[f] / cnt, cs = sums[F + f] / cnt;
+      const float m = norm_blend(mode, mode == 2 ? gmean[f] : 0.f, cm, w1, w);
+      const float sd = norm_blend(mode, mode == 2 ? gstd[f] : 0.f, cs, w1, w);
+      gl[f] = m; gl[F + f] = sd;
+      if (blockIdx.x == 0) { gmean_out[f] = m; gstd_out[f] = sd; }
+    }
+  }
+  __syncthreads();
+  const int FQ = F / 4;
+  for (size_t i = (size_t)blockIdx.x * NT + threadIdx.x; i < nq; i += (size_t)gridDim.x * NT) {
+    const int q = (int)(i % FQ);
+    const f32x4 m = gl4[q];
+    const f32x4 s = gl4[FQ + q];
+    out[i] = (x[i] - m) / s;
+  }
+}
+
 }
 
 extern "C" int mlvae_norm_supported(int F) { return F > 0 && F % 4 == 0 && F / 4 <= NT; }
@@ -135,6 +172,32 @@
   const int FQ = F / 4, RL = NT / FQ;
   norm_stats_kernel<<<B, NT, (size_t)RL * FQ * sizeof(f32x4), s>>>(T, F, x, rel_lens, utt_stats, eps);
   norm_sums_kernel<<<(2 * F + 1 + 63) / 64, NT, 0, s>>>(B, T, F, rel_lens, utt_stats, sums);
+  MLVAE_CHECK_LAUNCH();
+  return 0;
+}
+
+extern "C" int mlvae_norm_update_apply(size_t rows, int F, const float* x, const float* sums,
+                                       const float* glob_mean, const float* glob_std, float* glob_mean_out,
+                                       float* glob_std_out, int mode, float w_old, float w_new, float* out,
+                                       void* stream) {
+  if (!mlvae_norm_supported(F)) { mlvae_set_error("norm_update_apply: F=%d unsupported", F); return 1; }
+  if (mode < 0 || mode > 2) { mlvae_set_error("norm_update_apply: mode %d", mode); return 1; }
+  if (((uintptr_t)x | (uintptr_t)out) & 15) {
+    mlvae_set_error("norm_update_apply: buffers must be 16-byte aligned");
+    return 1;
+  }
+  if ((mode != 1 && (!glob_mean || !glob_std)) || (mode != 0 && (!sums || !glob_mean_out || !glob_std_out)) ||
+      (mode == 2 && (glob_mean_out == glob_mean || glob_std_out == glob_std))) {
+    mlvae_set_error("norm_update_apply: mode %d needs its statistics buffers (mode 2: out != in)", mode);
+    return 1;
+  }
+  const size_t nq = rows * (size_t)(F / 4);
+  size_t g = (nq + NT - 1) / NT;
+  if (g > 4096) g = 4096;
+  if (g < 1) g = 1;
+  norm_update_apply_kernel<<<(unsigned)g, NT, (size_t)2 * F * sizeof(float), (hipStream_t)stream>>>(
+      nq, F, reinterpret_cast<const f32x4*>(x), sums, glob_mean, glob_std, glob_mean_out, glob_std_out, mode,
+      w_old, w_new, reinterpret_cast<f32x4*>(out));
   MLVAE_CHECK_LAUNCH();
   return 0;
 }
diff --git a/ml-vae_amd/csrc/optim.hip b/ml-vae_amd/csrc/optim.hip
--- a/ml-vae_amd/csrc/optim.hip
+++ b/ml-vae_amd/csrc/optim.hip
@@ -27,11 +27,7 @@
   float b1, b2, eps;
 };
 
-__global__ __launch_bounds__(256) void adam_prologue(const double* partials, int nparts,
-                                                     const float* loss, const int* step, float lr,
-                                                     float b1, float b2, float max_norm,
-                                                     float* hyp, float* norm_out, const int* err) {
-  __shared__ double red[256];
+__device__ __forceinline__ double fold_partials(const double* partials, int nparts, double* red) {
   double a = 0.0;
   for (int i = threadIdx.x; i < nparts; i += 256) a += partials[i];
   red[threadIdx.x] = a;
@@ -40,24 +36,56 @@
     if ((int)threadIdx.x < o) red[threadIdx.x] += red[threadIdx.x + o];
     __syncthreads();
   }
-  if (threadIdx.x != 0) return;
-  const float total = (float)sqrt(red[0]);
+  return red[0];
+}
+
+__device__ __forceinline__ void adam_scalars(double sumsq, const float* loss, const int* step, float lr, float b1,
+                                             float b2, float max_norm, const int* err, float* h, float* total_out) {
+  const float total = (float)sqrt(sumsq);
   float coef = max_norm / (total + 1e-6f);
   coef = coef < 1.f ? coef : 1.f;
   if (!(total == total)) coef = total;
   const int t = *step + 1;
   const double bc1 = 1.0 - pow((double)b1, (double)t);
   const double bc2 = 1.0 - pow((double)b2, (double)t);
-  hyp[0] = coef;
-  hyp[1] = ((loss && !isfinite(*loss)) || (err && *err != 0)) ? 1.f : 0.f;
-  hyp[2] = (float)((double)lr / bc1);
-  hyp[3] = (float)sqrt(bc2);
+  h[0] = coef;
+  h[1] = ((loss && !isfinite(*loss)) || (err && *err != 0)) ? 1.f : 0.f;
+  h[2] = (float)((double)lr / bc1);
+  h[3] = (float)sqrt(bc2);
+  *total_out = total;
+}
+
+__global__ __launch_bounds__(256) void adam_prologue(const double* partials, int nparts,
+                                                     const float* loss, const int* step, float lr,
+                                                     float b1, float b2, float max_norm,
+                                                     float* hyp, float* norm_out, const int* err) {
+  __shared__ double red[256];
+  const double sumsq = fold_partials(partials, nparts, red);
+  if (threadIdx.x != 0) return;
+  float total;
+  adam_scalars(sumsq, loss, step, lr, b1, b2, max_norm, err, hyp, &total);
   if (norm_out) *norm_out = total;
 }
 
-__global__ __launch_bounds__(256) void adam_kernel(AdamArgs a) {
-  if (a.hyp[1] != 0.f) return;
-  const float coef = a.hyp[0], step_size = a.hyp[2], bc2s = a.hyp[3];
+template <bool FUSED>
+__device__ __forceinline__ float adam_elem(float g, float& m, float& v, float p, float coef, float w1, float w2,
+                                           float b2, float eps, float step_size, float bc2s) {
+#pragma clang fp contract(off)
+  const float gc = g * coef;
+  const float d = __builtin_fmaf(coef, g, -m);
+  const float t = gc * (w2 * gc);
+  if constexpr (FUSED) {
+    m = __builtin_fmaf(w1, d, m);
+    v = __builtin_fmaf(b2, v, t);
+  } else {
+    m = m + w1 * d;
+    v = v * b2 + t;
+  }
+  const float denom = sqrtf(v) / bc2s + eps;
+  return __builtin_fmaf(-step_size, m / denom, p);
+}
+
+__device__ __forceinline__ void adam_update(const AdamArgs& a, float coef, float step_size, float bc2s) {
   const float w1 = 1.f - a.b1, w2 = 1.f - a.b2;
   const size_t n4 = a.n / 4;
   f32x4* p4 = reinterpret_cast<f32x4*>(a.p);
@@ -65,34 +93,69 @@
   f32x4* v4 = reinterpret_cast<f32x4*>(a.v);
   const f32x4* g4 = reinterpret_cast<const f32x4*>(a.g);
   for (size_t i = (size_t)blockIdx.x * 256 + threadIdx.x; i < n4; i += (size_t)gridDim.x * 256) {
-    f32x4 g = g4[i] * coef, m = m4[i], v = v4[i], p = p4[i];
+    f32x4 g = g4[i], m = m4[i], v = v4[i], p = p4[i];
 #pragma unroll
     for (int e = 0; e < 4; ++e) {
-      m[e] = m[e] + w1 * (g[e] - m[e]);
-      v[e] = v[e] * a.b2 + w2 * g[e] * g[e];
-      const float denom = sqrtf(v[e]) / bc2s + a.eps;
-      p[e] = p[e] + (-step_size) * (m[e] / denom);
+      float me = m[e], ve = v[e];
+      p[e] = adam_elem<true>(g[e], me, ve, p[e], coef, w1, w2, a.b2, a.eps, step_size, bc2s);
+      m[e] = me; v[e] = ve;
     }
     p4[i] = p; m4[i] = m; v4[i] = v;
   }
   if (blockIdx.x == 0) {
     for (size_t i = n4 * 4 + threadIdx.x; i < a.n; i += 256) {
-      const float g = a.g[i] * coef;
       float m = a.m[i], v = a.v[i];
-      m = m + w1 * (g - m);
-      v = v * a.b2 + w2 * g * g;
-      a.p[i] = a.p[i] + (-step_size) * (m / (sqrtf(v) / bc2s + a.eps));
+      a.p[i] = adam_elem<false>(a.g[i], m, v, a.p[i], coef, w1, w2, a.b2, a.eps, step_size, bc2s);
       a.m[i] = m; a.v[i] = v;
     }
   }
+}
+
+__global__ __launch_bounds__(256) void adam_kernel(AdamArgs a) {
+  if (a.hyp[1] != 0.f) return;
+  adam_update(a, a.hyp[0], a.hyp[2], a.hyp[3]);
+}
+
+__device__ __forceinline__ void advance_counters(const float* loss, int* step, int* nonfinite, const int* err,
+                                                 int* err_skips) {
+  if (err && *err != 0) { if (err_skips) *err_skips += 1; }
+  else if (loss && !isfinite(*loss)) { if (nonfinite) *nonfinite += 1; }
+  else *step += 1;
+}
+
+struct AdamFusedArgs {
+  AdamArgs a;
+  const double* partials; int nparts;
+  const float* loss; int* step; int* nonfinite; const int* err; int* err_skips;
+  float lr, max_norm;
+  float* hyp; float* norm_out;
+  unsigned* ticket;
+};
+
+__global__ __launch_bounds__(256) void adam_fused_kernel(AdamFusedArgs f) {
+  __shared__ double red[256];
+  __shared__ float h[5];
+  const double sumsq = fold_partials(f.partials, f.nparts, red);
+  if (threadIdx.x == 0) {
+    adam_scalars(sumsq, f.loss, f.step, f.lr, f.a.b1, f.a.b2, f.max_norm, f.err, h, &h[4]);
+    if (blockIdx.x == 0) {
+      f.hyp[0] = h[0]; f.hyp[1] = h[1]; f.hyp[2] = h[2]; f.hyp[3] = h[3];
+      if (f.norm_out) *f.norm_out = h[4];
+    }
+  }
+  __syncthreads();
+  if (h[1] == 0.f) adam_update(f.a, h[0], h[2], h[3]);
+  if (threadIdx.x != 0) return;
+  const unsigned tk = __hip_atomic_fetch_add(f.ticket, 1u, __ATOMIC_RELAXED, __HIP_MEMORY_SCOPE_AGENT);
+  if (tk != gridDim.x - 1) return;
+  __hip_atomic_store(f.ticket, 0u, __ATOMIC_RELAXED, __HIP_MEMORY_SCOPE_AGENT);
+  advance_counters(f.loss, f.step, f.nonfinite, f.err, f.err_skips);
 }
 
 __global__ void step_counter_kernel(const float* loss, int* step, int* nonfinite, const int* err,
                                     int* err_skips) {
   if (threadIdx.x || blockIdx.x) return;
-  if (err && *err != 0) { if (err_skips) *err_skips += 1; }
-  else if (loss && !isfinite(*loss)) { if (nonfinite) *nonfinite += 1; }
-  else *step += 1;
+  advance_counters(loss, step, nonfinite, err, err_skips);
 }
 
 __global__ __launch_bounds__(256) void clip_scale_kernel(float* __restrict__ g, size_t n,
@@ -266,6 +329,27 @@
   return 0;
 }
 
+extern "C" int mlvae_adam_step_fused(float* params, float* exp_avg, float* exp_avg_sq, const float* grads,
+                                     size_t n, const double* partials, int nparts, const float* loss,
+                                     int* step, int* nonfinite, const int* err, int* err_skips, float lr,
+                                     float beta1, float beta2, float eps, float max_norm, float* norm_out,
+                                     float* hyp, unsigned* ticket, void* stream) {
+  if (!hyp || !ticket || !step || !partials ||
+      (((uintptr_t)params | (uintptr_t)exp_avg | (uintptr_t)exp_avg_sq | (uintptr_t)grads) & 15)) {
+    mlvae_set_error("adam_step_fused: needs hyp scratch, a ticket word, the step counter and 16-byte aligned buffers");
+    return 1;
+  }
+  AdamFusedArgs f;
+  f.a.p = params; f.a.m = exp_avg; f.a.v = exp_avg_sq; f.a.g = grads; f.a.n = n; f.a.hyp = hyp;
+  f.a.b1 = beta1; f.a.b2 = beta2; f.a.eps = eps;
+  f.partials = partials; f.nparts = nparts; f.loss = loss; f.step = step; f.nonfinite = nonfinite;
+  f.err = err; f.err_skips = err_skips; f.lr = lr; f.max_norm = max_norm; f.hyp = hyp; f.norm_out = norm_out;
+  f.ticket = ticket;
+  adam_fused_kernel<<<grid_for(n / 4 + 1, 2048), 256, 0, (hipStream_t)stream>>>(f);
+  MLVAE_CHECK_LAUNCH();
+  return 0;
+}
+
 extern "C" int mlvae_adam_step(float* params, float* exp_avg, float* exp_avg_sq, const float* grads,
                                size_t n, const double* partials, int nparts, const float* loss,
                                int* step, int* nonfinite, float lr, float beta1, float beta2,
diff --git a/ml-vae_amd/mlvae_hip/_lib.py b/ml-vae_amd/mlvae_hip/_lib.py
--- a/ml-vae_amd/mlvae_hip/_lib.py
+++ b/ml-vae_amd/mlvae_hip/_lib.py
@@ -22,6 +22,8 @@
                            F, P, SZ, P],
     "mlvae_cast_bf16": [SZ, P, P, P],
     "mlvae_cast_bf16_t": [I, I, P, P, P],
+    "mlvae_weight_prep": [I, P, P],
+    "mlvae_lstm_exchange_next": [I, P, SZ],
     "mlvae_gemm_bf16_workspace_size": [I, I, I, I],
     "mlvae_gemm_bf16_set_split_target": [I],
     "mlvae_gemm_bf16_set_variant": [I],
@@ -103,6 +105,7 @@
     "mlvae_grad_sumsq": [P, SZ, P, P],
     "mlvae_adam_step": [P, P, P, P, SZ, P, I, P, P, P, F, F, F, F, F, P, P, I, P],
     "mlvae_adam_step_ex": [P, P, P, P, SZ, P, I, P, P, P, P, P, F, F, F, F, F, P, P, I, P],
+    "mlvae_adam_step_fused": [P, P, P, P, SZ, P, I, P, P, P, P, P, F, F, F, F, F, P, P, P, P],
     "mlvae_colsum_workspace_size": [I, I],
     "mlvae_colsum": [I, I, P, I, P, P, F, P, SZ, P],
     "mlvae_colsum_ex": [I, I, P, I, I, P, P, F, P, SZ, P],
@@ -134,6 +137,7 @@
     "mlvae_norm_stats": [I, I, I, P, P, P, P, F, P],
     "mlvae_norm_update": [I, P, P, P, I, F, F, P],
     "mlvae_norm_apply": [SZ, I, P, P, P, P, P],
+    "mlvae_norm_update_apply": [SZ, I, P, P, P, P, P, P, I, F, F, P, P],
 }
 _RESTYPE = {
     "mlvae_last_error": C.c_char_p,
diff --git a/ml-vae_amd/mlvae_hip/engine.py b/ml-vae_amd/mlvae_hip/engine.py
--- a/ml-vae_amd/mlvae_hip/engine.py
+++ b/ml-vae_amd/mlvae_hip/engine.py
@@ -263,7 +263,9 @@
         self.gws_bytes = self.gws.numel() * 4
         xb = _lib.SZ()
         check(l.mlvae_lstm_workspace_size(B, H, PREC[cfg.prec], _lib.C.byref(xb)), "lstm_workspace_size")
-        self.xbuf = empty(max(xb.value, 16), dtype=torch.uint8)
+        xr = (max(xb.value, 16) + 15) // 16 * 16
+        self.xbufs = [empty(xr, dtype=torch.uint8), empty(xr, dtype=torch.uint8)]
+        self.x_cur, self.x_clean, self.x_stream = 0, False, None
         self.reset_step()
 
     def reset_step(self):
@@ -324,6 +326,7 @@
         self.nonfinite_ctr = torch.zeros(1, device=self.device, dtype=torch.int32)
         self.grad_norm = torch.zeros(1, **f)
         self.hyp = torch.zeros(4, **f)
+        self.adam_ticket = torch.zeros(1, device=self.device, dtype=torch.int32)
         self.err = torch.zeros(1, device=self.device, dtype=torch.int32)
         self.err_skips = torch.zeros(1, device=self.device, dtype=torch.int32)
         self._nonfinite_seen = 0
@@ -500,6 +503,16 @@
             return self.side_stream.cuda_stream
         return torch.cuda.current_stream(self.device).cuda_stream
 
+    def _exchange(self, w):
+        cur, other, s = w.xbufs[w.x_cur], w.xbufs[1 - w.x_cur], self._stream()
+        if not w.g16:
+            w.x_clean = False
+            return cur
+        clean = w.x_clean and w.x_stream == s
+        check(lib().mlvae_lstm_exchange_next(int(clean), _p(other), other.numel()), "lstm_exchange_next")
+        w.x_cur, w.x_clean, w.x_stream = 1 - w.x_cur, True, s
+        return cur
+
     def _ws(self, w):
         return w.gws_side if self._on_side else w.gws
 
@@ -630,10 +643,10 @@
     def _prep_weights(self, B, train):
         if self.flat_bf is None:
             return None
+        if self._full_chip(B):
+            self._weight_prep(train, flat=True)
+            return None
         check(lib().mlvae_cast_bf16(self.layout.total, _p(self.flat), _pb(self.flat_bf), self._stream()), "cast_bf16")
-        if self._full_chip(B):
-            self._weight_prep(train)
-            return None
         self._on_side = True
         self.side_stream.wait_event(self._mark())
         try:
@@ -644,15 +657,21 @@
         prep_ev.record(self.side_stream)
         return prep_ev
 
-    def _weight_prep(self, train):
+    def _weight_prep(self, train, flat=False):
         cfg, l, s = self.cfg, lib(), self._stream()
+        segs = []
+        if flat:
+            segs.append((_p(self.flat), _pb(self.flat_bf), self.layout.total, 0))
         if train and self.w1_t is not None:
-            check(l.mlvae_cast_bf16_t(2 * cfg.C, 2 * cfg.H, self._ptr("decoder.mean_fc.blocks.0.weight"),
-                                      _pb(self.w1_t), s), "cast_bf16_t")
+            segs.append((self._ptr("decoder.mean_fc.blocks.0.weight"), _pb(self.w1_t), 2 * cfg.C, 2 * cfg.H))
         if train:
             for li, dst in self.wih_t.items():
-                check(l.mlvae_cast_bf16_t(8 * cfg.H, cfg.Z if li == 0 else 2 * cfg.H,
-                                          self._ptr(f"decoder.rnn.weight_ih_l{li}"), _pb(dst), s), "cast_bf16_t")
+                segs.append((self._ptr(f"decoder.rnn.weight_ih_l{li}"), _pb(dst), 8 * cfg.H,
+                             cfg.Z if li == 0 else 2 * cfg.H))
+        for i in range(0, len(segs), 8):
+            part = segs[i:i + 8]
+            desc = (_lib.C.c_longlong * (4 * len(part)))(*[int(v) for sg in part for v in sg])
+            check(l.mlvae_weight_prep(len(part), desc, s), "weight_prep")
         n = 8 * cfg.H * 2 * cfg.H
         for li in self.w8:
             wih = self._ptr(f"decoder.rnn.weight_ih_l{li}")
@@ -758,6 +777,7 @@
         ydb_arg = None if skip_ydb else (_pb(w.Ydb[li]) if fuse_drop else None)
         yb_prev = bool(zproj and fuse_drop)
         w.yb_prev[li] = yb_prev
+        xbuf = self._exchange(w)
         with self._timed("lstm_fwd"):
             if zproj:
                 rp = lambda n: self._ptr(f"decoder.rnn.{n}")
@@ -768,17 +788,17 @@
                                           _p(w.Y[li]) if need_y else None, _pb(w.Yb[li]), int(yb_prev),
                                           ydb_arg, x8_ptr, x8_scale(cfg.dropout) if x8_fused else 0.0, seed,
                                           self._drop_off, cfg.dropout if fuse_drop else 0.0,
-                                          _p(w.xbuf), w.xbuf.numel(), _p(self.err), s), "lstm_fwd_z2")
+                                          _p(xbuf), xbuf.numel(), _p(self.err), s), "lstm_fwd_z2")
             elif x8_fused:
                 check(l.mlvae_lstm_fwd_fp8(B, T, H, W_hh, W_hh_r, _p(w.G[li]), _p(w.Cs[li]), _pb(w.Yb[li]),
                                            ydb_arg, x8_ptr, x8_scale(cfg.dropout), seed, self._drop_off, cfg.dropout,
-                                           _p(w.xbuf), w.xbuf.numel(), _p(self.err), s), "lstm_fwd_fp8")
+                                           _p(xbuf), xbuf.numel(), _p(self.err), s), "lstm_fwd_fp8")
             else:
                 check(l.mlvae_lstm_fwd_ex2(PREC[cfg.prec], B, T, H, W_hh, W_hh_r, _p(w.G[li]), int(w.g16),
                                            _p(w.Cs[li]), _p(w.Y[li]) if need_y else None, _pgb(w.Yb[li] if w.bf else None),
                                            _pb(w.Ydb[li]) if fuse_drop else None, seed, self._drop_off,
                                            cfg.dropout if fuse_drop else 0.0,
-                                           _p(w.xbuf), w.xbuf.numel(), _p(self.err), s), "lstm_fwd")
+                                           _p(xbuf), xbuf.numel(), _p(self.err), s), "lstm_fwd")
         if not drop:
             return w.Y[li], (w.Yb[li] if w.bf else None), 2 * H, 2 * H
         if fuse_drop:
@@ -999,6 +1019,7 @@
         W_hh, W_hh_r = self._ptr(f"decoder.rnn.weight_hh_l{li}"), self._ptr(f"decoder.rnn.weight_hh_l{li}_reverse")
         dGb = w.dGb[li] if w.bf else None
         dyb = w.dy_bf16[li]
+        xbuf = self._exchange(w)
         with self._timed("lstm_bwd"):
             rows = w.dbias_rows[li] if (w.g16 and not (li == 0 and w.enc_fused)) else None
             if f8:
@@ -1013,12 +1034,12 @@
                 check(l.mlvae_lstm_bwd_fp8_ex(B, T, H, W_hh, W_hh_r, _p(w.G[li]),
                                            _p(w.Cs[li]), _p(w.dY[li]), int(dyb), None if f8hh else _pb(dGb),
                                            _pg(rows), w.dG8[li].data_ptr() if f8_dgrad else None, _p(self.g8[li]),
-                                           am + 4 * par, _p(w.xbuf), w.xbuf.numel(), _p(self.err), s),
+                                           am + 4 * par, _p(xbuf), xbuf.numel(), _p(self.err), s),
                       "lstm_bwd_fp8")
             else:
                 check(l.mlvae_lstm_bwd_ex3(PREC[cfg.prec], B, T, H, W_hh, W_hh_r, _p(w.G[li]),
                                            int(w.g16), _p(w.Cs[li]), _p(w.dY[li]), int(dyb), _pgb(dGb), _pg(rows),
-                                           _p(w.xbuf), w.xbuf.numel(), _p(self.err), s), "lstm_bwd")
+                                           _p(xbuf), xbuf.numel(), _p(self.err), s), "lstm_bwd")
 
     def _lstm_wgrads(self, w, li, split_target, f8w, f8hh):
         prev = lib().mlvae_gemm_bf16_set_split_target(split_target)
@@ -1187,12 +1208,12 @@
             self._allreduce_grads(w)
         check(l.mlvae_grad_sumsq(_p(self.grad), self.layout.total, self.sq_parts.data_ptr(), s), "sumsq")
         b1, b2 = cfg.betas
-        check(l.mlvae_adam_step_ex(_p(self.flat), _p(self.exp_avg), _p(self.exp_avg_sq), _p(self.grad),
-                                   self.layout.total, self.sq_parts.data_ptr(), self.nparts,
-                                   _p(w.loss, 2), self.step_ctr.data_ptr(), self.nonfinite_ctr.data_ptr(),
-                                   self.err.data_ptr(), self.err_skips.data_ptr(),
-                                   cfg.lr, b1, b2, cfg.adam_eps, cfg.max_grad_norm,
-                                   _p(self.grad_norm), _p(self.hyp), 1, s), "adam")
+        check(l.mlvae_adam_step_fused(_p(self.flat), _p(self.exp_avg), _p(self.exp_avg_sq), _p(self.grad),
+                                      self.layout.total, self.sq_parts.data_ptr(), self.nparts,
+                                      _p(w.loss, 2), self.step_ctr.data_ptr(), self.nonfinite_ctr.data_ptr(),
+                                      self.err.data_ptr(), self.err_skips.data_ptr(),
+                                      cfg.lr, b1, b2, cfg.adam_eps, cfg.max_grad_norm,
+                                      _p(self.grad_norm), _p(self.hyp), self.adam_ticket.data_ptr(), s), "adam")
 
     def _start_suffix_allreduce(self):
         from . import dist as mdist
@@ -1245,7 +1266,6 @@
                     or gm.data_ptr() % 16 or gs.data_ptr() % 16:
                 gm = gm.to(self.device, torch.float32).contiguous().clone()
                 gs = gs.to(self.device, torch.float32).contiguous().clone()
-            norm.glob_mean, norm.glob_std = gm, gs
             mode, w_old, w_new = (1 if fresh else 0), 0.0, 0.0
             if norm.training:
                 if norm.count == 0:
@@ -1254,8 +1274,10 @@
                     wt = norm.avg_factor if norm.avg_factor is not None else 1.0 / (norm.count + 1)
                     mode, w_old, w_new = 2, 1 - wt, wt
                 norm.count += 1
-            check(l.mlvae_norm_update(F, _p(sums), _p(gm), _p(gs), mode, w_old, w_new, s), "norm_update")
-            check(l.mlvae_norm_apply(B * T, F, _p(x), _p(gm), _p(gs), _p(out), s), "norm_apply")
+            gm_new, gs_new = (torch.empty_like(gm), torch.empty_like(gs)) if mode == 2 else (gm, gs)
+            check(l.mlvae_norm_update_apply(B * T, F, _p(x), _p(sums), _p(gm), _p(gs), _p(gm_new), _p(gs_new),
+                                            mode, w_old, w_new, _p(out), s), "norm_update_apply")
+            norm.glob_mean, norm.glob_std = gm_new, gs_new
         return out
 
     def train_step(self, x, lens, eps=None, dropout_masks=None, normalizer=None, epoch=0):
@@ -1279,6 +1301,8 @@
 
     def check_errors(self):
         if int(self.err.item()) != 0:
+            for w in self._work.values():
+                w.x_clean = False
             raise RuntimeError("LSTM recurrence hand-off timed out (err word set): the outputs "
                                "of the affected steps are undefined; their optimizer updates were "
                                f"skipped ({int(self.err_skips.item())} steps)")
```

Result: no change. 13.80 million (-0.7%).
